# benfred/implicit

Hardware: AMD Instinct MI355X
Metric: ALS user+item updates/sec per iteration (factors=128); top-k recs/sec (higher is better)
Workload: dtype f32; 1 GPU; BASELINE configs[2]: last.fm-360K-shaped synthetic CSR, ALS CG cg_steps=3; users=358868, items=292385, nnz=17308340, factors=128, solver=cg, cg_steps=3

## Files before the change

implicit_amd/csrc/als_cg.hip:

```cpp
#include <type_traits>

#include "common.h"
#include "wave_ops.h"
#include "als_qtile.h"
#include "als_tile.h"

namespace imp {

template <int VPL, bool VEC, bool FIRST>
__device__ __forceinline__ void sparse_pass_simple(const int32_t *__restrict__ indices, const float *__restrict__ data,
                                                   const float *__restrict__ Y, int f, int lane, int begin, int end,
                                                   const float (&vec)[VPL], float (&acc)[VPL]) {
  constexpr int U = 4;
  for (int k0 = begin; k0 < end; k0 += 64) {
    int cnt = min(64, end - k0);
    int my_idx = 0;
    float my_c = 0.f;
    if (lane < cnt) {
      my_idx = indices[k0 + lane];
      my_c = data[k0 + lane];
    }
    for (int j = 0; j < cnt; j += U) {
      float y[U][VPL];
      float d[U];
// ... 387 lines not shown
        acc[v] = ((a8[0][v] + a8[1][v]) + (a8[2][v] + a8[3][v])) + ((a8[4][v] + a8[5][v]) + (a8[6][v] + a8[7][v]));
    }
    float x[VPL], dense[VPL];
    if (PHASE == 1 && xvec) load_row<VPL, VEC>(xvec + (size_t)li * LD, VEC ? LD : f, lane, x);
    else load_xrow<VPL, VEC>(xrow, f, lane, x);
#pragma unroll
    for (int v = 0; v < VPL; ++v) dense[v] = 0.f;
    if (PHASE == 0) {
      gram_matvec<VPL, VEC>(Amat, lda, lane, x, dense, 0, f);
      float r[VPL];
#pragma unroll
      for (int v = 0; v < VPL; ++v) r[v] = acc[v] - dense[v];
      float rsold = wave_allsum(dot_local<VPL>(r, r));
#pragma unroll
      for (int v = 0; v < VPL; ++v) {
        int e = elem<VPL, VEC>(lane, v);
        rvec[(size_t)li * LD + e] = r[v];
        pvec[(size_t)li * LD + e] = r[v];
        if (xvec) xvec[(size_t)li * LD + e] = x[v];
      }
      if (lane == 0) {
        scal[2 * li] = rsold;
        scal[2 * li + 1] = rsold < 1e-20f ? 1.f : 0.f;
      }
    } else {
      float p[VPL], r[VPL];
      load_row<VPL, VEC>(pvec + (size_t)li * LD, vld, lane, p);
      load_row<VPL, VEC>(rvec + (size_t)li * LD, vld, lane, r);
      gram_matvec<VPL, VEC>(Amat, lda, lane, p, dense, 0, f);
      float Ap[VPL];
#pragma unroll
      for (int v = 0; v < VPL; ++v) Ap[v] = dense[v] + acc[v];
      float rsold = scal[2 * li];
      float alpha = rsold / wave_allsum(dot_local<VPL>(p, Ap));
#pragma unroll
      for (int v = 0; v < VPL; ++v) {
        x[v] = fmaf(alpha, p[v], x[v]);
        r[v] = fmaf(-alpha, Ap[v], r[v]);
      }
      float rsnew = wave_allsum(dot_local<VPL>(r, r));
      float beta = rsnew / rsold;
#pragma unroll
      for (int v = 0; v < VPL; ++v) {
        int e = elem<VPL, VEC>(lane, v);
        if (e < f) store_x(xrow + e, x[v]);
        if (xvec) xvec[(size_t)li * LD + e] = x[v];
        rvec[(size_t)li * LD + e] = r[v];
        pvec[(size_t)li * LD + e] = fmaf(beta, p[v], r[v]);
      }
      if (lane == 0) {
        scal[2 * li] = rsnew;
        if (rsnew < 1e-20f) scal[2 * li + 1] = 1.f;
      }
    }
  }
}

template <typename T>
__global__ void zero_rows_kernel(const int32_t *__restrict__ order, int first, int count, T *__restrict__ X, int f) {
  size_t total = (size_t)count * f;
  for (size_t i = blockIdx.x * (size_t)blockDim.x + threadIdx.x; i < total; i += (size_t)gridDim.x * blockDim.x) {
    size_t r = i / f, c = i - r * f;
    store1(X + (size_t)order[first + r] * f + c, 0.f);
  }
}

template <typename T> static void zero_rows_t(const int32_t *order, int first, int count, T *X, int f) {
  if (count <= 0) return;
  IMP_PROF("zero_rows");
  size_t total = (size_t)count * f;
  int grid = (int)std::min<size_t>((total + 255) / 256, (size_t)ctx().num_cus * 8);
  zero_rows_kernel<T><<<grid, 256, 0, stream()>>>(order, first, count, X, f);
  IMP_CHECK_HIP(hipGetLastError());
}
void zero_rows(const int32_t *order, int first, int count, float *X, int f) { zero_rows_t<float>(order, first, count, X, f); }

template <int VPL, bool A_LDS>
static void launch_fused(const imp_csr *C, int first, int count, float *X, const float *Y, const float *A0, int f,
                         int cg_steps, const char *name) {
  if (count <= 0) return;
  constexpr int BLOCK = 512;
  constexpr int LD = 64 * VPL;
  size_t lds = (A_LDS ? (size_t)f * LD : 0) * sizeof(float);
  auto kern = als_cg_kernel<VPL, BLOCK, A_LDS>;
  allow_dynamic_lds(kern, std::max<size_t>(lds, 16));
  int blocks_per_cu = (int)std::max<size_t>(1, std::min<size_t>(2048 / BLOCK, (160 * 1024) / std::max<size_t>(lds, 1)));
  int grid = std::min((count + BLOCK / 64 - 1) / (BLOCK / 64), ctx().num_cus * blocks_per_cu * ctx().oversub);
  IMP_PROF(name);
  kern<<<grid, BLOCK, lds, stream()>>>(C->order.data(), first, count, C->indptr.data(), C->indices.data(), C->data.data(), X, Y,
                                       A0, f, cg_steps);
  IMP_CHECK_HIP(hipGetLastError());
}

template <int VPL, bool VEC, bool A_LDS, typename T>
static void launch_long(const imp_csr *C, const LongPlan &lp, T *X, const T *Y, const float *A0, int f, int cg_steps) {
  const int n_long = lp.n_long, n_seg = lp.n_seg;
  if (n_long <= 0) return;
  constexpr int BLOCK = 512;
  constexpr int LD = 64 * VPL;
  constexpr bool kHalf = !std::is_same<T, float>::value;
  size_t need = ((size_t)n_seg + (kHalf ? 3 : 2) * (size_t)n_long) * LD + 2 * (size_t)n_long;
  float *partial = ctx().long_ws.reserve(need);
  float *rvec = partial + (size_t)n_seg * LD;
  float *pvec = rvec + (size_t)n_long * LD;
  float *scal = pvec + (size_t)n_long * LD;
  float *xvec = kHalf ? scal + 2 * (size_t)n_long : nullptr;
  LongPlanDev plan = lp.dev(C->order.data());

  const bool rowblock = n_long <= ctx().num_cus * 2;
  size_t lds = ((A_LDS ? (size_t)f * LD : 0) + (rowblock ? (size_t)(BLOCK / 64) * LD : 0)) * sizeof(float);
  auto comb0 = rowblock ? cg_long_combine_kernel<VPL, VEC, BLOCK, A_LDS, 0, true, T> : cg_long_combine_kernel<VPL, VEC, BLOCK, A_LDS, 0, false, T>;
  auto comb1 = rowblock ? cg_long_combine_kernel<VPL, VEC, BLOCK, A_LDS, 1, true, T> : cg_long_combine_kernel<VPL, VEC, BLOCK, A_LDS, 1, false, T>;
  allow_dynamic_lds(comb0, std::max<size_t>(lds, 16));
  allow_dynamic_lds(comb1, std::max<size_t>(lds, 16));
  int grid_part = std::min(((n_seg + 3) / 4 + 7) / 8 * 8, ctx().num_cus * 8);
  int grid_comb = rowblock ? n_long : std::min((n_long + BLOCK / 64 - 1) / (BLOCK / 64), ctx().num_cus * 2);
  {
    IMP_PROF("als_cg_long_partial");
    if constexpr (VEC && (VPL == 1 || VPL == 2))
      cg_long_partial_q_kernel<64 * VPL, true, T>
          <<<grid_part, 256, 0, stream()>>>(plan, C->indices.data(), C->data.data(), X, Y, partial, pvec, scal);
    else if constexpr (std::is_same<T, float>::value)
      cg_long_partial_kernel<VPL, VEC, true>
          <<<grid_part, 256, 0, stream()>>>(plan, C->indices.data(), C->data.data(), X, Y, f, partial, pvec, scal);
    IMP_CHECK_HIP(hipGetLastError());
  }
  {
    IMP_PROF("als_cg_long_combine");
    comb0<<<grid_comb, BLOCK, lds, stream()>>>(plan, X, A0, f, partial, rvec, pvec, scal, xvec);
    IMP_CHECK_HIP(hipGetLastError());
  }
  for (int it = 0; it < cg_steps; ++it) {
    {
      IMP_PROF("als_cg_long_partial");
      if constexpr (VEC && (VPL == 1 || VPL == 2))
        cg_long_partial_q_kernel<64 * VPL, false, T>
            <<<grid_part, 256, 0, stream()>>>(plan, C->indices.data(), C->data.data(), X, Y, partial, pvec, scal);
      else if constexpr (std::is_same<T, float>::value)
        cg_long_partial_kernel<VPL, VEC, false>
            <<<grid_part, 256, 0, stream()>>>(plan, C->indices.data(), C->data.data(), X, Y, f, partial, pvec, scal);
      IMP_CHECK_HIP(hipGetLastError());
    }
    {
      IMP_PROF("als_cg_long_combine");
      comb1<<<grid_comb, BLOCK, lds, stream()>>>(plan, X, A0, f, partial, rvec, pvec, scal, xvec);
      IMP_CHECK_HIP(hipGetLastError());
    }
  }
}

template <int VPL, typename T>
static void cg_f64_f128(const imp_csr *C, T *X, const T *Y, size_t y_rows, const float *A0, int cg_steps) {
  constexpr int f = 64 * VPL;
  if (solver_switches().nm) least_squares_cg_nm<T>(C, X, Y, y_rows, A0, f, cg_steps);
  else launch_long<VPL, true, true, T>(C, C->plan_all, X, Y, A0, f, cg_steps);
  least_squares_cg_q<T>(C, X, Y, A0, f, cg_steps);
  zero_rows_t<T>(C->order.data(), C->first_empty(), C->n_empty(), X, f);
}

static void cg_f256(const imp_csr *C, float *X, const float *Y, const float *A0, int cg_steps) {
  constexpr int f = 256;
  const int32_t *b = C->bin_start;
  launch_long<4, true, false, float>(C, C->plan_all, X, Y, A0, f, cg_steps);
  if (solver_switches().w256) {
    launch_f256(C, b[1], b[2] - b[1], X, Y, A0, cg_steps, "als_cg_mid_rows");
    least_squares_cg_w256(C, X, Y, A0, cg_steps);
  } else {
    launch_f256(C, b[1], b[7] - b[1], X, Y, A0, cg_steps, "als_cg_mid_rows");
  }
  zero_rows_t<float>(C->order.data(), C->first_empty(), C->n_empty(), X, f);
}

template <int VPL, bool A_LDS>
static void cg_generic(const imp_csr *C, float *X, const float *Y, const float *A0, int f, int cg_steps) {
  const int32_t *b = C->bin_start;
  launch_long<VPL, false, A_LDS, float>(C, C->plan_all, X, Y, A0, f, cg_steps);
  launch_fused<VPL, A_LDS>(C, b[1], b[7] - b[1], X, Y, A0, f, cg_steps, "als_cg_mid_rows");
  zero_rows_t<float>(C->order.data(), C->first_empty(), C->n_empty(), X, f);
}

bool cg_native_half(int f) { return f == 64 || f == 128; }

static void least_squares_cg_padded(const imp_csr *C, imp_matrix *X, const imp_matrix *YtY, const imp_matrix *Y, int cg_steps, int F) {
  const size_t rx = (size_t)C->rows;
  const PaddedViews p = pad_in(X, Y, YtY, rx, F, true);
  if (F == 64) cg_f64_f128<1, float>(C, p.X.f32(), p.Y.f32(), p.Y.rows, p.YtY.f32(), cg_steps);
  else if (F == 128) cg_f64_f128<2, float>(C, p.X.f32(), p.Y.f32(), p.Y.rows, p.YtY.f32(), cg_steps);
  else cg_f256(C, p.X.f32(), p.Y.f32(), p.YtY.f32(), cg_steps);
  pad_out(X, rx, F);
}

void least_squares_cg(const imp_csr *C, imp_matrix *X, const imp_matrix *YtY, const imp_matrix *Y, int cg_steps) {
  note_device_write(X->data, (size_t)C->rows * X->cols * X->itemsize);
  IMP_PROF("als_cg_half_sweep");
  const int f = (int)X->cols;
  const float *a0 = YtY->f32();
  if (X->itemsize == 2) {
    if (!cg_native_half(f)) throw std::invalid_argument("least_squares: fp16 factors with this factor count are converted by the caller");
    __half *x = reinterpret_cast<__half *>(X->data);
    const __half *y = reinterpret_cast<const __half *>(Y->data);
    if (f == 64) cg_f64_f128<1, __half>(C, x, y, Y->rows, a0, cg_steps);
    else cg_f64_f128<2, __half>(C, x, y, Y->rows, a0, cg_steps);
    return;
  }
  float *x = X->f32();
  const float *y = Y->f32();
  if (solver_switches().cg_pad && f < 256 && f != 64 && f != 128 && f >= 1) {
    least_squares_cg_padded(C, X, YtY, Y, cg_steps, f < 64 ? 64 : (f < 128 ? 128 : 256));
    return;
  }
  if (f == 64) cg_f64_f128<1, float>(C, x, y, Y->rows, a0, cg_steps);
  else if (f == 128) cg_f64_f128<2, float>(C, x, y, Y->rows, a0, cg_steps);
  else if (f == 256) cg_f256(C, x, y, a0, cg_steps);
  else if (f < 64) cg_generic<1, true>(C, x, y, a0, f, cg_steps);
  else if (f < 128) cg_generic<2, true>(C, x, y, a0, f, cg_steps);
  else if (f < 192) cg_generic<3, true>(C, x, y, a0, f, cg_steps);
  else if (f < 256) cg_generic<4, false>(C, x, y, a0, f, cg_steps);
  else if (f <= 384) cg_generic<6, false>(C, x, y, a0, f, cg_steps);
  else if (f <= 512) cg_generic<8, false>(C, x, y, a0, f, cg_steps);
  else if (f <= 768) cg_generic<12, false>(C, x, y, a0, f, cg_steps);
  else if (f <= 1024) cg_generic<16, false>(C, x, y, a0, f, cg_steps);
  else throw std::invalid_argument("least_squares: factors must be <= 1024 (as the reference, implicit/gpu/als.cu:177-182)");
}

}
```

implicit_amd/csrc/als_cg_fixup.hip:

```cpp
#include <type_traits>

#include "als_qtile.h"
#include "common.h"

namespace imp {

template <int F, typename ST>
__global__ __launch_bounds__(256) void als_cg_fault_fixup_kernel(const unsigned *__restrict__ fault_count,
                                                                 const unsigned *__restrict__ fault_rows, int capacity,
                                                                 const int32_t *__restrict__ indptr,
                                                                 const int32_t *__restrict__ indices,
                                                                 const float *__restrict__ data, ST *__restrict__ X,
                                                                 const ST *__restrict__ Y, const float *__restrict__ A0, int cg_steps,
                                                                 unsigned long long *total) {
  constexpr int FC = F / 64, WAVES = 4, U = 4;
  __shared__ float vecs[WAVES][F];
  const int n = min((int)fault_count[0], capacity);
  if (n == 0) return;
  if (blockIdx.x == 0 && threadIdx.x == 0) __hip_atomic_fetch_add(total, (unsigned long long)n, __ATOMIC_RELAXED, __HIP_MEMORY_SCOPE_SYSTEM);
  const int lane = threadIdx.x & 63, wave = threadIdx.x >> 6;
  float *vec = vecs[wave];
  auto load_vec = [&](const ST *row, float (&v)[FC]) {
#pragma unroll
    for (int c = 0; c < FC; ++c) v[c] = load1(row + FC * lane + c);
  };
  auto apply = [&](bool first, int rb, int re, const float (&v)[FC], float (&acc)[FC]) {
#pragma unroll
    for (int c = 0; c < FC; ++c) vec[FC * lane + c] = v[c];
#pragma unroll
    for (int c = 0; c < FC; ++c) acc[c] = 0.f;
    for (int j = 0; j < F; ++j) {
      const float vj = vec[j];
#pragma unroll
      for (int c = 0; c < FC; ++c) acc[c] = fmaf(A0[(size_t)j * F + FC * lane + c], vj, acc[c]);
    }
    if (first) {
#pragma unroll
      for (int c = 0; c < FC; ++c) acc[c] = -acc[c];
    }
    for (int k0 = rb; k0 < re; k0 += U) {
      float conf[U], y[U][FC];
#pragma unroll
      for (int q = 0; q < U; ++q) {
        const int k = min(k0 + q, re - 1);
        conf[q] = data[k];
        load_vec(Y + (size_t)indices[k] * F, y[q]);
      }
#pragma unroll
      for (int q = 0; q < U; ++q) {
        if (k0 + q < re) {
          const float d = wave_allsum(dot_local<FC>(y[q], v));
          const float cm1 = fabsf(conf[q]) - 1.f;
          const float w = first ? fmaxf(conf[q], 0.f) - cm1 * d : cm1 * d;
#pragma unroll
          for (int c = 0; c < FC; ++c) acc[c] = fmaf(w, y[q][c], acc[c]);
        }
      }
    }
  };
  for (int i = blockIdx.x * WAVES + wave; i < n; i += gridDim.x * WAVES) {
    const int u = (int)fault_rows[i];
    const int rb = indptr[u], re = indptr[u + 1];
    ST *xrow = X + (size_t)u * F;
    float x[FC], r[FC], p[FC], Ap[FC];
    load_vec(xrow, x);
    apply(true, rb, re, x, r);
#pragma unroll
    for (int c = 0; c < FC; ++c) p[c] = r[c];
    float rsold = wave_allsum(dot_local<FC>(r, r));
    if (rsold < 1e-20f) continue;
    for (int it = 0; it < cg_steps; ++it) {
      apply(false, rb, re, p, Ap);
      const float alpha = rsold / wave_allsum(dot_local<FC>(p, Ap));
#pragma unroll
      for (int c = 0; c < FC; ++c) {
        x[c] = fmaf(alpha, p[c], x[c]);
        r[c] = fmaf(-alpha, Ap[c], r[c]);
      }
      const float rsnew = wave_allsum(dot_local<FC>(r, r));
      if (rsnew < 1e-20f) break;
      const float beta = rsnew / rsold;
#pragma unroll
      for (int c = 0; c < FC; ++c) p[c] = fmaf(beta, p[c], r[c]);
      rsold = rsnew;
    }
#pragma unroll
    for (int c = 0; c < FC; ++c) store1(xrow + FC * lane + c, x[c]);
  }
}

unsigned long long *fixup_total() {
  auto &c = ctx();
  if (!c.fixup_total) {
    IMP_CHECK_HIP(hipHostMalloc(reinterpret_cast<void **>(&c.fixup_total), sizeof(unsigned long long), hipHostMallocMapped));
    *c.fixup_total = 0ull;
  }
  return c.fixup_total;
}

template <int F, typename T>
void launch_cg_fixup(const unsigned *count, const unsigned *rows, int capacity, const imp_csr *C, T *X, const T *Y, const float *A0,
                     int cg_steps) {
  if (capacity <= 0) return;
  IMP_PROF("als_cg_fixup");
  als_cg_fault_fixup_kernel<F, T><<<std::min((capacity + 3) / 4, ctx().num_cus * 2), 256, 0, stream()>>>(
      count, rows, capacity, C->indptr.data(), C->indices.data(), C->data.data(), X, Y, A0, cg_steps, fixup_total());
  IMP_CHECK_HIP(hipGetLastError());
}
template void launch_cg_fixup<64, float>(const unsigned *, const unsigned *, int, const imp_csr *, float *, const float *, const float *, int);
template void launch_cg_fixup<128, float>(const unsigned *, const unsigned *, int, const imp_csr *, float *, const float *, const float *, int);
template void launch_cg_fixup<64, __half>(const unsigned *, const unsigned *, int, const imp_csr *, __half *, const __half *, const float *, int);
template void launch_cg_fixup<128, __half>(const unsigned *, const unsigned *, int, const imp_csr *, __half *, const __half *, const float *, int);


}
```

implicit_amd/csrc/als_cg_nm.hip:

```cpp
#include "als_qf_common.h"
#include "common.h"
#include "wave_ops.h"

namespace imp {

namespace {

typedef _Float16 half8 __attribute__((ext_vector_type(8)));
typedef _Float16 half2v __attribute__((ext_vector_type(2)));
typedef float f32x16 __attribute__((ext_vector_type(16)));
typedef float f32x4v __attribute__((ext_vector_type(4)));
typedef unsigned u32x4 __attribute__((ext_vector_type(4)));

template <int F> struct NmShape;
template <> struct NmShape<128> {
  static constexpr int M = 32, KG = 2, NACC = 16;
  using acc_t = f32x16;
  __device__ static __forceinline__ acc_t mfma(half8 a, half8 b, acc_t c) { return __builtin_amdgcn_mfma_f32_32x32x16_f16(a, b, c, 0, 0, 0); }
  __device__ static __forceinline__ int row(int lane, int e) { return (e & 3) + 8 * (e >> 2) + 4 * (lane >> 5); }
  __device__ static __forceinline__ int col(int lane) { return lane & 31; }
};
template <> struct NmShape<64> {
  static constexpr int M = 16, KG = 4, NACC = 4;
  using acc_t = f32x4v;
  __device__ static __forceinline__ acc_t mfma(half8 a, half8 b, acc_t c) { return __builtin_amdgcn_mfma_f32_16x16x32_f16(a, b, c, 0, 0, 0); }
  __device__ static __forceinline__ int row(int lane, int e) { return 4 * (lane >> 4) + e; }
  __device__ static __forceinline__ int col(int lane) { return lane & 15; }
};

template <int F> struct NmLayout {
  static constexpr int M = F / 4;
  static constexpr int TS = M + 1;
  static constexpr int IMG = 16 * M * TS;
  static constexpr int KCH = 8 * NmShape<F>::KG;
  static constexpr int ROUND = 4 * KCH;
  static constexpr int kTiles = 10;
  static constexpr int kSlots = 3;
  static constexpr int QUAD = 64 * 4;
  static constexpr int OPS = 4 * 16 * QUAD;
  static constexpr int NP = 256 / F;
  static constexpr int kVec = IMG > OPS ? IMG : OPS;
  static constexpr size_t lds_floats = (size_t)kVec + 2 * F + NP * F + 64 + 4 * F;
  __host__ __device__ static constexpr int at(int I, int J, int m, int n) { return ((I * 4 + J) * M + m) * TS + n; }
};
__device__ constexpr int nm_tile_i(int t) { return t < 1 ? 0 : t < 3 ? 1 : t < 6 ? 2 : 3; }
__device__ constexpr int nm_tile_j(int t) { return t - (nm_tile_i(t) * (nm_tile_i(t) + 1)) / 2; }

__device__ __forceinline__ void split_pair(float x0, float x1, unsigned &hi, unsigned &lo) {
  const f32x2 v = {x0, x1};
  const half2v h = __builtin_convertvector(v, half2v);
  const f32x2 r = v - __builtin_convertvector(h, f32x2);
  const half2v l = __builtin_convertvector(r, half2v);
  hi = __builtin_bit_cast(unsigned, h);
  lo = __builtin_bit_cast(unsigned, l);
}
__device__ __forceinline__ unsigned pack_pair(float x0, float x1) {
  const f32x2 v = {x0, x1};
  return __builtin_bit_cast(unsigned, __builtin_convertvector(v, half2v));
}
__device__ __forceinline__ float comp(const float4 &v, int c) { return c == 0 ? v.x : c == 1 ? v.y : c == 2 ? v.z : v.w; }

template <int F> __global__ void nm_gram_image_kernel(const float *__restrict__ A0, float *__restrict__ img, int *__restrict__ ctl,
                                                      float y_rows, int forced_k, float reg = 0.f) {
  using L = NmLayout<F>;
  if (blockIdx.x == 0 && threadIdx.x < 64) {
    float d = 0.f;
    for (int j = threadIdx.x; j < F; j += 64) d = fmaxf(d, A0[(size_t)j * F + j]);
    d = wave_allmax(d);
    if (threadIdx.x == 0) {
      int k = 0;
      const float rms = sqrtf((d + reg) / fmaxf(y_rows, 1.f));
      if (rms > 0.f && rms < 8.f) k = min((int)floorf(log2f(8.f / rms)), 16);
      ctl[0] = 0;
      ctl[1] = forced_k >= 0 ? forced_k : k;
      ctl[2] = 0;
      ctl[3] = 0;
    }
  }
  for (int e = blockIdx.x * blockDim.x + threadIdx.x; e < L::IMG; e += gridDim.x * blockDim.x) {
    const int n = e % L::TS, m = (e / L::TS) % L::M, t = e / (L::TS * L::M);
    img[e] = n < L::M ? A0[(size_t)(4 * m + t / 4) * F + 4 * n + t % 4] + ((m == n && t / 4 == t % 4) ? reg : 0.f) : 0.f;
  }
}

__device__ __forceinline__ void lds_barrier() { asm volatile("s_waitcnt lgkmcnt(0)\n\ts_barrier" ::: "memory"); }

template <int F, typename T, bool TRIM = false>
__device__ __forceinline__ void nm_build(const int32_t *__restrict__ indices, const float *__restrict__ data, const T *__restrict__ Y,
                                         const float *__restrict__ gram_img, bool whole, int begin, int end, float *smem, float *bvec,
                                         int tid, int ko, int scale_k) {
  using S = NmShape<F>;
  using L = NmLayout<F>;
  constexpr bool kHalf = !std::is_same<T, float>::value;
  const int lane = tid & 63, wave = __builtin_amdgcn_readfirstlane(tid >> 6);
  const int a = lane % S::M, g = lane / S::M;
  const int first = wave < 2 ? 3 * wave : 2 * wave + 2;
  const int n_slots = wave < 2 ? 3 : 2;
  int tI[L::kSlots], tJ[L::kSlots];
#pragma unroll
  for (int k = 0; k < L::kSlots; ++k) {
    const int t = min(first + k, L::kTiles - 1);
    tI[k] = t < 1 ? 0 : t < 3 ? 1 : t < 6 ? 2 : 3;
    tJ[k] = t - tI[k] * (tI[k] + 1) / 2;
  }
  typename S::acc_t acc[L::kSlots];
#pragma unroll
  for (int k = 0; k < L::kSlots; ++k)
#pragma unroll
    for (int e = 0; e < S::NACC; ++e) acc[k][e] = 0.f;
  float b4[4] = {0.f, 0.f, 0.f, 0.f};
  const float scale2 = __uint_as_float((unsigned)(127 + 2 * scale_k) << 23), unscale2 = __uint_as_float((unsigned)(127 - 2 * scale_k) << 23);

  const int n_rounds = (ko & 1) ? 0 : (end - begin + L::ROUND - 1) / L::ROUND;
  struct Entry {
    int col;
    float c;
  };
  auto load_entry = [&](int r) {
    Entry en;
    const int k = begin + r * L::ROUND + wave * L::KCH + (lane % L::KCH);
    const int kk = min(k, end - 1);
    en.col = indices[kk];
    const float c = data[kk];
    en.c = k < end ? c : -1.f;
    return en;
  };
  float4 yb[8];
  auto gather = [&](const Entry &en, float4 (&y)[8]) {
#pragma unroll
    for (int q = 0; q < 8; ++q) {
      const int col = __shfl(en.col, 8 * g + q, 64);
      y[q] = load4(Y + (size_t)col * F + 4 * a);
    }
  };
  float *ops = smem;
  int *negflag = reinterpret_cast<int *>(bvec + 2 * F + L::NP * F + 32);
  Entry e0{0, -1.f}, e1 = e0, e2 = e0;
  if (n_rounds > 0) {
    e0 = load_entry(0), e1 = load_entry(1);
    gather(e0, yb);
  }
  struct Pair {
    half8 h, l;
  };
  const float *lane_ops = ops + 4 * lane;
  int negbits = 0;
  auto ld_u = [&](int st, int I) {
    Pair p;
    const int ku = (negbits >> st) & 1 ? 0 : 2;
    p.h = __builtin_bit_cast(half8, *reinterpret_cast<const u32x4 *>(lane_ops + (st * 16 + ku * 4 + I) * L::QUAD));
    p.l = __builtin_bit_cast(half8, *reinterpret_cast<const u32x4 *>(lane_ops + (st * 16 + (ku + 1) * 4 + I) * L::QUAD));
    return p;
  };
  auto ld_y = [&](int st, int J) {
    Pair p;
    p.h = __builtin_bit_cast(half8, *reinterpret_cast<const u32x4 *>(lane_ops + (st * 16 + 2 * 4 + J) * L::QUAD));
    if constexpr (!kHalf) p.l = __builtin_bit_cast(half8, *reinterpret_cast<const u32x4 *>(lane_ops + (st * 16 + 3 * 4 + J) * L::QUAD));
    else p.l = p.h;
    return p;
  };
  auto products = [&](auto k, const Pair &u, const Pair &y) {
    acc[k.value] = S::mfma(u.h, y.h, acc[k.value]);
    acc[k.value] = S::mfma(u.l, y.h, acc[k.value]);
    if constexpr (!kHalf) acc[k.value] = S::mfma(u.h, y.l, acc[k.value]);
  };
  auto consume = [&](int s0, int s1) {
    negbits = __builtin_amdgcn_readfirstlane(negflag[0] | (negflag[1] << 1) | (negflag[2] << 2) | (negflag[3] << 3));
    if (wave == 0) {
      Pair u0 = ld_u(s0, 0), y0 = ld_y(s0, 0);
#pragma unroll 1
      for (int st = s0; st < s1; ++st) {
        const Pair u1 = ld_u(st, 1);
        products(idx_t<0>{}, u0, y0);
        const Pair y1 = ld_y(st, 1);
        products(idx_t<1>{}, u1, y0);
        u0 = ld_u(min(st + 1, s1 - 1), 0), y0 = ld_y(min(st + 1, s1 - 1), 0);
        products(idx_t<2>{}, u1, y1);
      }
    } else if (wave == 1) {
      Pair u2 = ld_u(s0, 2), y0 = ld_y(s0, 0);
#pragma unroll 1
      for (int st = s0; st < s1; ++st) {
        const Pair y1 = ld_y(st, 1);
        products(idx_t<0>{}, u2, y0);
        const Pair y2 = ld_y(st, 2);
        products(idx_t<1>{}, u2, y1);
        const Pair un = ld_u(min(st + 1, s1 - 1), 2);
        y0 = ld_y(min(st + 1, s1 - 1), 0);
        products(idx_t<2>{}, u2, y2);
        u2 = un;
      }
    } else {
      const int J0 = wave == 2 ? 0 : 2;
      Pair u3 = ld_u(s0, 3), ya = ld_y(s0, J0);
#pragma unroll 1
      for (int st = s0; st < s1; ++st) {
        const Pair yb2 = ld_y(st, J0 + 1);
        products(idx_t<0>{}, u3, ya);
        const Pair un = ld_u(min(st + 1, s1 - 1), 3);
        ya = ld_y(min(st + 1, s1 - 1), J0);
        products(idx_t<1>{}, u3, yb2);
        u3 = un;
      }
    }
  };
  auto produce = [&](int r, float4 (&y)[8]) {
    if (r > 0) e0 = e1, e1 = e2;
    e2 = load_entry(r + 2);
    {
      const float w_mine = (fabsf(e0.c) - 1.f) * scale2;
      const float cp_mine = e0.c > 0.f ? e0.c : 0.f;
      float *mine = ops + (size_t)wave * 16 * L::QUAD + 4 * lane;
      if constexpr (!kHalf) {
        const float sq_mine = __builtin_amdgcn_sqrtf(fabsf(w_mine));
        const unsigned ng_mine = w_mine < 0.f ? 0x8000u : 0u;
        const bool any_neg = __builtin_amdgcn_ballot_w64(ng_mine != 0u) != 0ull;
        if (lane == 0) negflag[wave] = any_neg ? 1 : 0;
        float sq[8];
        unsigned ng[8];
#pragma unroll
        for (int q = 0; q < 8; ++q) {
          sq[q] = __shfl(sq_mine, 8 * g + q, 64);
          ng[q] = (unsigned)__shfl((int)ng_mine, 8 * g + q, 64);
          const float cp = __shfl(cp_mine, 8 * g + q, 64);
          b4[0] = fmaf(cp, y[q].x, b4[0]);
          b4[1] = fmaf(cp, y[q].y, b4[1]);
          b4[2] = fmaf(cp, y[q].z, b4[2]);
          b4[3] = fmaf(cp, y[q].w, b4[3]);
        }
#pragma unroll
        for (int c = 0; c < 4; ++c) {
          u32x4 zh, zl;
#pragma unroll
          for (int q = 0; q < 8; q += 2) {
            unsigned h, l;
            split_pair(sq[q] * comp(y[q], c), sq[q + 1] * comp(y[q + 1], c), h, l);
            zh[q / 2] = h, zl[q / 2] = l;
          }
          *reinterpret_cast<u32x4 *>(mine + (2 * 4 + c) * L::QUAD) = zh;
          *reinterpret_cast<u32x4 *>(mine + (3 * 4 + c) * L::QUAD) = zl;
          if (any_neg) {
            u32x4 uh, ul;
#pragma unroll
            for (int q = 0; q < 8; q += 2) {
              const unsigned m = ng[q] | (ng[q + 1] << 16);
              uh[q / 2] = zh[q / 2] ^ m, ul[q / 2] = zl[q / 2] ^ m;
            }
            *reinterpret_cast<u32x4 *>(mine + (0 * 4 + c) * L::QUAD) = uh;
            *reinterpret_cast<u32x4 *>(mine + (1 * 4 + c) * L::QUAD) = ul;
          }
          __builtin_amdgcn_sched_barrier(0);
        }
      } else {
        unsigned hb = (((__float_as_uint(w_mine) & 0x7f800000u) + (127u << 23)) >> 1) & 0x7f800000u;
        hb = min(max(hb, (127u - 12u) << 23), (127u + 24u) << 23);
        const float sb_mine = __uint_as_float(hb), wa_mine = w_mine * __uint_as_float((254u << 23) - hb);
        if (lane == 0) negflag[wave] = 1;
        float wa[8], sb[8];
#pragma unroll
        for (int q = 0; q < 8; ++q) {
          wa[q] = __shfl(wa_mine, 8 * g + q, 64);
          sb[q] = __shfl(sb_mine, 8 * g + q, 64);
          const float cp = __shfl(cp_mine, 8 * g + q, 64);
          b4[0] = fmaf(cp, y[q].x, b4[0]);
          b4[1] = fmaf(cp, y[q].y, b4[1]);
          b4[2] = fmaf(cp, y[q].z, b4[2]);
          b4[3] = fmaf(cp, y[q].w, b4[3]);
        }
#pragma unroll
        for (int c = 0; c < 4; ++c) {
          u32x4 uh, ul, yh;
#pragma unroll
          for (int q = 0; q < 8; q += 2) {
            const float y0 = comp(y[q], c), y1 = comp(y[q + 1], c);
            unsigned h, l;
            yh[q / 2] = pack_pair(sb[q] * y0, sb[q + 1] * y1);
            split_pair(wa[q] * y0, wa[q + 1] * y1, h, l);
            uh[q / 2] = h, ul[q / 2] = l;
          }
          *reinterpret_cast<u32x4 *>(mine + (0 * 4 + c) * L::QUAD) = uh;
          *reinterpret_cast<u32x4 *>(mine + (1 * 4 + c) * L::QUAD) = ul;
          *reinterpret_cast<u32x4 *>(mine + (2 * 4 + c) * L::QUAD) = yh;
          __builtin_amdgcn_sched_barrier(0);
        }
      }
    }
    gather(e1, y);
  };
#pragma unroll 1
  for (int r = 0; r < n_rounds; ++r) {
    produce(r, yb);
    lds_barrier();
    if constexpr (TRIM) consume(0, min(4, (end - begin - r * L::ROUND + L::KCH - 1) / L::KCH));
    else consume(0, 4);
    lds_barrier();
  }
  if (!(ko & 2)) {
    float *bstage = bvec + 2 * F + L::NP * F + 64;
#pragma unroll
    for (int c = 0; c < 4; ++c) {
      float v = b4[c];
      if constexpr (S::KG == 4) v += __shfl_xor(v, 16, 64);
      v += __shfl_xor(v, 32, 64);
      if (g == 0) bstage[wave * F + c * L::M + a] = v;
    }
    float *img = smem;
    const int n = S::col(lane);
#pragma unroll
    for (int k = 0; k < L::kSlots; ++k) {
      if (k < n_slots) {
        const int I = tI[k], J = tJ[k];
        float gv[S::NACC];
#pragma unroll
        for (int e = 0; e < S::NACC; ++e) gv[e] = 0.f;
        if (whole) {
#pragma unroll
          for (int e = 0; e < S::NACC; ++e) gv[e] = gram_img[L::at(I, J, S::row(lane, e), n)];
        }
#pragma unroll
        for (int e = 0; e < S::NACC; ++e) {
          const int m = S::row(lane, e);
          const float v = fmaf(acc[k][e], unscale2, gv[e]);
          img[L::at(I, J, m, n)] = v;
          if (I != J) img[L::at(J, I, n, m)] = v;
        }
      }
    }
  }
  __syncthreads();
}

template <int F, typename T>
__device__ __forceinline__ bool nm_cg(const float *img, const float *bvec, float *pv, float *parts, float *red, T *xrow, int cg_steps, int tid) {
  using L = NmLayout<F>;
  constexpr int M = L::M, NP = L::NP, JPG = 4 / NP;
  const int r = tid % F, grp = tid / F, lane = tid & 63, wave = tid >> 6;
  const int I = r / M, m = r % M;
  int slot = 0;
  auto matvec = [&]() {
    float s[4] = {0.f, 0.f, 0.f, 0.f};
#pragma unroll
    for (int jj = 0; jj < JPG; ++jj) {
      const int J = grp * JPG + jj;
      const float *row = img + L::at(I, J, m, 0);
#pragma unroll
      for (int n = 0; n < M; n += 4) {
        const float4 p4 = *reinterpret_cast<const float4 *>(pv + J * M + n);
        s[0] = fmaf(row[n], p4.x, s[0]), s[1] = fmaf(row[n + 1], p4.y, s[1]);
        s[2] = fmaf(row[n + 2], p4.z, s[2]), s[3] = fmaf(row[n + 3], p4.w, s[3]);
      }
    }
    parts[grp * F + r] = (s[0] + s[1]) + (s[2] + s[3]);
    __syncthreads();
    float q = parts[r];
#pragma unroll
    for (int gq = 1; gq < NP; ++gq) q += parts[gq * F + r];
    return q;
  };
  auto block_sum = [&](float v) {
    v = wave_allsum(grp == 0 ? v : 0.f);
    if (lane == 0) red[4 * slot + wave] = v;
    __syncthreads();
    const float s = (red[4 * slot] + red[4 * slot + 1]) + (red[4 * slot + 2] + red[4 * slot + 3]);
    slot = (slot + 1) & 7;
    return s;
  };
  auto finite = [](float v) { return fabsf(v) <= 3.0e38f; };
  float x = load1(xrow + 4 * m + I);
  if (grp == 0) pv[r] = x;
  __syncthreads();
  float res = bvec[r] - matvec();
  float p = res;
  float rsold = block_sum(res * res);
  if (!finite(rsold)) return true;
  if (rsold < 1e-20f) return false;
  for (int it = 0; it < cg_steps; ++it) {
    if (grp == 0) pv[r] = p;
    __syncthreads();
    const float Ap = matvec();
    const float pAp = block_sum(p * Ap);
    const float alpha = rsold / pAp;
    x = fmaf(alpha, p, x);
    res = fmaf(-alpha, Ap, res);
    const float rsnew = block_sum(res * res);
    if (!finite(pAp) || !finite(rsnew) || !finite(alpha)) return true;
    if (rsnew < 1e-20f) break;
    p = fmaf(rsnew / rsold, p, res);
    rsold = rsnew;
  }
  if (grp == 0) store1(xrow + 4 * m + I, x);
  return false;
}

#ifdef CHOL_NM_STATS
__device__ unsigned long long g_chol_nm_stats[8];
#define CHOL_TICK(slot)                                                          \
  do {                                                                           \
    __builtin_amdgcn_sched_barrier(0);                                           \
    const unsigned long long now_ = __builtin_amdgcn_s_memtime();                \
    if (threadIdx.x == 0) atomicAdd(&g_chol_nm_stats[slot], now_ - chol_t_last); \
    chol_t_last = now_;                                                          \
    __builtin_amdgcn_sched_barrier(0);                                           \
  } while (0)
__device__ unsigned long long chol_t_last_dummy;
#else
#define CHOL_TICK(slot) ((void)0)
#endif
struct NoGram {
  __device__ __forceinline__ float operator()(int, int, int, int) const { return 0.f; }
};
template <int F, typename GB>
__device__ __forceinline__ bool nm_chol(float *img, float *bvec, float *scr, float *xrow, int tid, const GB &gblocks) {
  static_assert(F == 128, "block ownership and the LDS budget are laid out for f = 128");
#ifdef CHOL_NM_STATS
  unsigned long long chol_t_last = __builtin_amdgcn_s_memtime();
#endif
  using L = NmLayout<F>;
  constexpr int NB = F / 4, NBLK = NB * (NB + 1) / 2, LDL = F + 4, SL = (NBLK + 255) / 256;
  static_assert(F * LDL <= L::kVec, "the row-major factor re-uses the image's space");
  float *pan = scr;
  float *dblk = scr + 2 * F * 4;
  int bm[SL], bn[SL];
  float B[SL][4][4];
#pragma unroll
  for (int s = 0; s < SL; ++s) {
    const int bid = tid + 256 * s;
    bm[s] = bn[s] = -1;
    if (bid < NBLK) {
      int t = (int)((sqrtf(8.f * (float)bid + 1.f) - 1.f) * 0.5f);
      while (t * (t + 1) / 2 > bid) --t;
      while ((t + 1) * (t + 2) / 2 <= bid) ++t;
      bn[s] = NB - 1 - t, bm[s] = bn[s] + (bid - t * (t + 1) / 2);
#pragma unroll
      for (int a = 0; a < 4; ++a)
#pragma unroll
        for (int c = 0; c < 4; ++c) B[s][a][c] = img[L::at(a, c, bm[s], bn[s])] + gblocks(a, c, bm[s], bn[s]);
    }
  }
  float rb[4] = {0.f, 0.f, 0.f, 0.f};
  if (tid < NB) {
#pragma unroll
    for (int c = 0; c < 4; ++c) rb[c] = bvec[c * L::M + tid];
  }
  __syncthreads();
  CHOL_TICK(1);
#pragma unroll
  for (int s = 0; s < SL; ++s) {
    if (bm[s] == 0 && bn[s] == 0) {
#pragma unroll
      for (int a = 0; a < 4; ++a) *reinterpret_cast<float4 *>(dblk + 4 * a) = make_float4(B[s][a][0], B[s][a][1], B[s][a][2], B[s][a][3]);
    }
  }
  __syncthreads();
  bool fail = false;
#pragma unroll 1
  for (int kb = 0; kb < NB; ++kb) {
    const float *D = dblk + (kb & 1) * 16;
    float *P = pan + (size_t)(kb & 1) * F * 4;
    const float4 d0 = *reinterpret_cast<const float4 *>(D), d1 = *reinterpret_cast<const float4 *>(D + 4),
                 d2 = *reinterpret_cast<const float4 *>(D + 8), d3 = *reinterpret_cast<const float4 *>(D + 12);
    auto rsq = [](float d) {
      const float r = __builtin_amdgcn_rsqf(d);
      return r * fmaf(-0.5f * d * r, r, 1.5f);
    };
    const float p0 = d0.x, r0 = rsq(p0);
    const float l10 = d1.x * r0, l20 = d2.x * r0, l30 = d3.x * r0;
    const float p1 = fmaf(-l10, l10, d1.y), r1 = rsq(p1);
    const float l21 = fmaf(-l20, l10, d2.y) * r1, l31 = fmaf(-l30, l10, d3.y) * r1;
    const float p2 = fmaf(-l21, l21, fmaf(-l20, l20, d2.z)), r2 = rsq(p2);
    const float l32 = fmaf(-l31, l21, fmaf(-l30, l20, d3.z)) * r2;
    const float p3 = fmaf(-l32, l32, fmaf(-l31, l31, fmaf(-l30, l30, d3.w))), r3 = rsq(p3);
    if (!(p0 > 0.f && p1 > 0.f && p2 > 0.f && p3 > 0.f && p3 < 3.0e38f)) {
      fail = true;
      break;
    }
    auto solve_row = [&](float (&v)[4]) {
      const float x0 = v[0] * r0;
      const float x1 = fmaf(-x0, l10, v[1]) * r1;
      const float x2 = fmaf(-x1, l21, fmaf(-x0, l20, v[2])) * r2;
      const float x3 = fmaf(-x2, l32, fmaf(-x1, l31, fmaf(-x0, l30, v[3]))) * r3;
      v[0] = x0, v[1] = x1, v[2] = x2, v[3] = x3;
    };
#pragma unroll
    for (int s = 0; s < SL; ++s) {
      if (bn[s] == kb) {
        if (bm[s] > kb) {
#pragma unroll
          for (int a = 0; a < 4; ++a) {
            solve_row(B[s][a]);
            *reinterpret_cast<float4 *>(P + (size_t)(4 * bm[s] + a) * 4) = make_float4(B[s][a][0], B[s][a][1], B[s][a][2], B[s][a][3]);
          }
        } else {
          B[s][0][0] = r0, B[s][1][0] = l10, B[s][1][1] = r1, B[s][2][0] = l20, B[s][2][1] = l21, B[s][2][2] = r2;
          B[s][3][0] = l30, B[s][3][1] = l31, B[s][3][2] = l32, B[s][3][3] = r3;
        }
      }
    }
    if (tid == kb) {
      solve_row(rb);
      *reinterpret_cast<float4 *>(bvec + 4 * kb) = make_float4(rb[0], rb[1], rb[2], rb[3]);
    }
    __syncthreads();
    float *Dn = dblk + ((kb + 1) & 1) * 16;
#pragma unroll
    for (int s = 0; s < SL; ++s) {
      if (bn[s] > kb) {
        float4 pm[4], pn[4];
#pragma unroll
        for (int a = 0; a < 4; ++a) {
          pm[a] = *reinterpret_cast<const float4 *>(P + (size_t)(4 * bm[s] + a) * 4);
          pn[a] = *reinterpret_cast<const float4 *>(P + (size_t)(4 * bn[s] + a) * 4);
        }
#pragma unroll
        for (int a = 0; a < 4; ++a)
#pragma unroll
          for (int c = 0; c < 4; ++c)
            B[s][a][c] = fmaf(-pm[a].w, pn[c].w, fmaf(-pm[a].z, pn[c].z, fmaf(-pm[a].y, pn[c].y, fmaf(-pm[a].x, pn[c].x, B[s][a][c]))));
        if (bn[s] == kb + 1 && bm[s] == kb + 1) {
#pragma unroll
          for (int a = 0; a < 4; ++a) *reinterpret_cast<float4 *>(Dn + 4 * a) = make_float4(B[s][a][0], B[s][a][1], B[s][a][2], B[s][a][3]);
        }
      }
    }
    if (tid < NB && tid > kb) {
      const float4 z4 = *reinterpret_cast<const float4 *>(bvec + 4 * kb);
#pragma unroll
      for (int c = 0; c < 4; ++c) {
        const float4 pc = *reinterpret_cast<const float4 *>(P + (size_t)(4 * tid + c) * 4);
        rb[c] = fmaf(-z4.w, pc.w, fmaf(-z4.z, pc.z, fmaf(-z4.y, pc.y, fmaf(-z4.x, pc.x, rb[c]))));
      }
    }
    __syncthreads();
  }
  CHOL_TICK(2);
  if (fail) return true;
#pragma unroll
  for (int s = 0; s < SL; ++s) {
    if (bm[s] >= 0) {
#pragma unroll
      for (int a = 0; a < 4; ++a)
        *reinterpret_cast<float4 *>(img + (size_t)(4 * bm[s] + a) * LDL + 4 * bn[s]) = make_float4(B[s][a][0], B[s][a][1], B[s][a][2], B[s][a][3]);
    }
  }
  __syncthreads();
// ... 10 lines not shown
    const float x1 = fmaf(-q3.y, x3, fmaf(-q2.y, x2, z.y)) * q1.y;
    const float x0 = fmaf(-q3.x, x3, fmaf(-q2.x, x2, fmaf(-q1.x, x1, z.x))) * q0.x;
    if (tid < 4 * kb) {
      const float *col = img + (size_t)(4 * kb) * LDL + tid;
      bvec[tid] = fmaf(-col[3 * LDL], x3, fmaf(-col[2 * LDL], x2, fmaf(-col[LDL], x1, fmaf(-col[0], x0, bvec[tid]))));
    }
    if (tid == 0) *reinterpret_cast<float4 *>(xs + 4 * kb) = make_float4(x0, x1, x2, x3);
    __syncthreads();
  }
  CHOL_TICK(4);
  if (tid < F) xrow[tid] = xs[tid];
  return false;
}

template <int F, typename T, bool CHOL = false>
__global__ __launch_bounds__(256, 2) void als_cg_nm_kernel(const LongPlanDev plan, const int32_t *__restrict__ indices,
                                                           const float *__restrict__ data, T *__restrict__ X, const T *__restrict__ Y,
                                                           const float *__restrict__ gram_img, int cg_steps, float *__restrict__ partial,
                                                           int *__restrict__ ticket,
                                                           unsigned *__restrict__ fix_rows,
                                                           int ko) {
  using L = NmLayout<F>;
  extern __shared__ __attribute__((aligned(16))) float smem[];
  __shared__ int next_item;
  float *img = smem, *bvec = img + L::kVec, *pv = bvec + F, *parts = pv + F, *red = parts + L::NP * F;
  const int tid = threadIdx.x;
  const int scale_k = __builtin_amdgcn_readfirstlane(ticket[1]);
  for (int s = blockIdx.x; s < plan.n_seg;) {
    const int li = plan.seg_row[s];
    const int begin = plan.seg_begin[s], end = plan.seg_end[s];
    const bool whole = plan.row_seg[li + 1] - plan.row_seg[li] == 1;
    __syncthreads();
    nm_build<F, T>(indices, data, Y, gram_img, whole, begin, end, smem, bvec, tid, ko, scale_k);
    if (tid < F) {
      const float *bstage = bvec + 2 * F + L::NP * F + 64;
      bvec[tid] = (bstage[tid] + bstage[F + tid]) + (bstage[2 * F + tid] + bstage[3 * F + tid]);
    }
    __syncthreads();
    int drawn = 0;
    if (tid == 0) drawn = (int)gridDim.x + atomicAdd(ticket, 1);
    if (!(ko & 4)) {
      if (whole) {
        bool bad = false;
        if constexpr (CHOL) bad = nm_chol<F>(img, bvec, pv, X + (size_t)plan.rows[li] * F, tid, NoGram{});
        else bad = nm_cg<F, T>(img, bvec, pv, parts, red, X + (size_t)plan.rows[li] * F, cg_steps, tid);
        if (bad && tid == 0) fix_rows[atomicAdd(ticket + 2, 1)] = (unsigned)plan.rows[li];
      } else {
        float *out = partial + (size_t)s * (L::IMG + F);
        for (int e = tid; e < L::IMG / 4; e += 256) reinterpret_cast<float4 *>(out)[e] = reinterpret_cast<const float4 *>(img)[e];
        if (tid < F) out[L::IMG + tid] = bvec[tid];
      }
    }
    if (tid == 0) next_item = drawn;
    __syncthreads();
    s = next_item;
  }
}

template <int F>
__global__ __launch_bounds__(256) void als_cg_nm_reduce_kernel(const LongPlanDev plan, int n_multi, const float *__restrict__ gram_img,
                                                               float *__restrict__ partial) {
  using L = NmLayout<F>;
  constexpr int CH = 16, PER = L::IMG / CH / 4;
  static_assert(L::IMG % (CH * 4) == 0, "chunks of whole float4 pieces");
  for (int item = blockIdx.x; item < n_multi * CH; item += gridDim.x) {
    const int li = item / CH, chunk = item % CH;
    const int s0 = plan.row_seg[li], s1 = plan.row_seg[li + 1];
    const size_t stride = (size_t)(L::IMG + F) / 4;
    for (int e = threadIdx.x; e < PER + (chunk == 0 ? F / 4 : 0); e += 256) {
      const size_t off = e < PER ? (size_t)chunk * PER + e : (size_t)L::IMG / 4 + (e - PER);
      float4 *base = reinterpret_cast<float4 *>(partial) + off;
      float4 sum = e < PER ? reinterpret_cast<const float4 *>(gram_img)[off] : make_float4(0.f, 0.f, 0.f, 0.f);
      int s = s0;
      for (; s + 8 <= s1; s += 8) {
        float4 v[8];
#pragma unroll
        for (int q = 0; q < 8; ++q) v[q] = base[(size_t)(s + q) * stride];
#pragma unroll
        for (int q = 0; q < 8; ++q) sum.x += v[q].x, sum.y += v[q].y, sum.z += v[q].z, sum.w += v[q].w;
      }
      for (; s < s1; ++s) {
        const float4 v = base[(size_t)s * stride];
        sum.x += v.x, sum.y += v.y, sum.z += v.z, sum.w += v.w;
      }
      base[(size_t)s0 * stride] = sum;
    }
  }
}

template <int F, typename T, bool CHOL = false>
__global__ __launch_bounds__(256) void als_cg_nm_finish_kernel(const LongPlanDev plan, int n_multi, T *__restrict__ X, int cg_steps,
                                                               const float *__restrict__ partial, int *__restrict__ ctl,
                                                               unsigned *__restrict__ fix_rows) {
  using L = NmLayout<F>;
  extern __shared__ __attribute__((aligned(16))) float smem[];
  float *img = smem, *bvec = img + L::kVec, *pv = bvec + F, *parts = pv + F, *red = parts + L::NP * F;
  const int tid = threadIdx.x;
  for (int li = blockIdx.x; li < n_multi; li += gridDim.x) {
    const float *in = partial + (size_t)plan.row_seg[li] * (L::IMG + F);
    __syncthreads();
    for (int e = tid; e < L::IMG / 4; e += 256) reinterpret_cast<float4 *>(img)[e] = reinterpret_cast<const float4 *>(in)[e];
    if (tid < F) bvec[tid] = in[L::IMG + tid];
    __syncthreads();
    bool bad = false;
    if constexpr (CHOL) bad = nm_chol<F>(img, bvec, pv, X + (size_t)plan.rows[li] * F, tid, NoGram{});
    else bad = nm_cg<F, T>(img, bvec, pv, parts, red, X + (size_t)plan.rows[li] * F, cg_steps, tid);
    if (bad && tid == 0) fix_rows[atomicAdd(ctl + 2, 1)] = (unsigned)plan.rows[li];
  }
}

template <int F>
__global__ __launch_bounds__(256, 2) void als_chol_nm_rows_kernel(const int32_t *__restrict__ order, int first, int count,
                                                                  const int32_t *__restrict__ indptr, const int32_t *__restrict__ indices,
                                                                  const float *__restrict__ data, float *__restrict__ X,
                                                                  const float *__restrict__ Y, const float *__restrict__ gram_img,
                                                                  int *__restrict__ ctl, unsigned *__restrict__ fix_rows) {
  using L = NmLayout<F>;
  extern __shared__ __attribute__((aligned(16))) float smem[];
  __shared__ int next_item;
  float *img = smem, *bvec = img + L::kVec, *pv = bvec + F;
  const int tid = threadIdx.x;
  const int scale_k = __builtin_amdgcn_readfirstlane(ctl[1]);
  struct GramBlocks {
    const float *img;
    __device__ __forceinline__ float operator()(int a, int c, int m, int n) const { return img[L::at(a, c, m, n)]; }
  } gb{gram_img};
  for (int i = blockIdx.x; i < count;) {
    const int u = order[first + i];
    const int begin = indptr[u], end = indptr[u + 1];
    __syncthreads();
#ifdef CHOL_NM_STATS
    unsigned long long chol_t_last = __builtin_amdgcn_s_memtime();
#endif
    nm_build<F, float, true>(indices, data, Y, gram_img, false, begin, end, smem, bvec, tid, 0, scale_k);
    if (tid < F) {
      const float *bstage = bvec + 2 * F + L::NP * F + 64;
      bvec[tid] = (bstage[tid] + bstage[F + tid]) + (bstage[2 * F + tid] + bstage[3 * F + tid]);
    }
    __syncthreads();
    CHOL_TICK(0);
#ifdef CHOL_NM_STATS
    if (tid == 0) atomicAdd(&g_chol_nm_stats[5], 1ull);
#endif
    int drawn = 0;
    if (tid == 0) drawn = (int)gridDim.x + atomicAdd(ctl + 3, 1);
    const bool bad = nm_chol<F>(img, bvec, pv, X + (size_t)u * F, tid, gb);
    if (bad && tid == 0) fix_rows[atomicAdd(ctl + 2, 1)] = (unsigned)u;
    if (tid == 0) next_item = drawn;
    __syncthreads();
    i = next_item;
  }
}

template <int F, typename T> void launch_nm(const imp_csr *C, T *X, const T *Y, size_t y_rows, const float *A0, int cg_steps) {
  const LongPlan &lp = C->plan_nm;
  if (lp.n_seg <= 0) return;
  using L = NmLayout<F>;
  static_assert(L::IMG % 4 == 0, "the image is copied in 16-byte pieces");
  const size_t lds = L::lds_floats * sizeof(float);
  const int n_multi = C->nm_multi_rows, n_multi_seg = C->nm_multi_segs;
  const size_t need = (size_t)L::IMG + (size_t)n_multi_seg * (L::IMG + F);
  float *gram_img = ctx().long_ws.reserve(need), *partial = gram_img + L::IMG;
  auto &tk = ctx().nm_ticket;
  tk.reserve(4, true);
  auto &fix = ctx().nm_fix_rows;
  fix.reserve((size_t)lp.n_long);
  LongPlanDev plan = lp.dev(C->order.data());
  auto kern = als_cg_nm_kernel<F, T>;
  auto fin = als_cg_nm_finish_kernel<F, T>;
  allow_dynamic_lds(kern, lds);
  allow_dynamic_lds(fin, lds);
  {
    IMP_PROF("als_cg_nm_rows");
    constexpr int forced_k = -1;
    nm_gram_image_kernel<F><<<(L::IMG + 255) / 256, 256, 0, stream()>>>(A0, gram_img, tk.data(), (float)y_rows, std::min(forced_k, 16));
    const int grid = std::min(lp.n_seg, ctx().num_cus * 2);
    constexpr int ko = 0;
    kern<<<grid, 256, lds, stream()>>>(plan, C->indices.data(), C->data.data(), X, Y, gram_img, cg_steps, partial, tk.data(), fix.data(), ko);
    IMP_CHECK_HIP(hipGetLastError());
  }
  if (n_multi > 0) {
    IMP_PROF("als_cg_nm_finish");
    als_cg_nm_reduce_kernel<F><<<std::min(n_multi * 16, ctx().num_cus * 16), 256, 0, stream()>>>(plan, n_multi, gram_img, partial);
    fin<<<std::min(n_multi, ctx().num_cus * 2), 256, lds, stream()>>>(plan, n_multi, X, cg_steps, partial, tk.data(), fix.data());
    IMP_CHECK_HIP(hipGetLastError());
  }
  launch_cg_fixup<F, T>(reinterpret_cast<const unsigned *>(tk.data() + 2), fix.data(), lp.n_long, C, X, Y, A0, cg_steps);
}

}

CholNmList least_squares_cholesky_nm(const imp_csr *C, float *X, const float *Y, size_t y_rows, const float *YtY, float reg) {
  constexpr int F = 128;
  using L = NmLayout<F>;
  const LongPlan &lp = C->plan_nm;
  const int32_t *b = C->bin_start;
  const size_t lds = (L::lds_floats + 128) * sizeof(float);
  const int n_multi = C->nm_multi_rows, n_multi_seg = C->nm_multi_segs;
  const size_t need = (size_t)L::IMG + (size_t)n_multi_seg * (L::IMG + F);
  float *gram_img = ctx().long_ws.reserve(need), *partial = gram_img + L::IMG;
  auto &tk = ctx().nm_ticket;
  tk.reserve(4, true);
  auto &fix = ctx().nm_fix_rows;
  const int capacity = C->nonempty();
  fix.reserve((size_t)std::max(capacity, 1));
  constexpr int forced_k = -1;
  {
    IMP_PROF("als_cholesky_nm_long");
    nm_gram_image_kernel<F><<<(L::IMG + 255) / 256, 256, 0, stream()>>>(YtY, gram_img, tk.data(), (float)y_rows, std::min(forced_k, 16), reg);
    if (lp.n_seg > 0) {
      LongPlanDev plan = lp.dev(C->order.data());
      auto kern = als_cg_nm_kernel<F, float, true>;
      auto fin = als_cg_nm_finish_kernel<F, float, true>;
      allow_dynamic_lds(kern, lds);
      allow_dynamic_lds(fin, lds);
      kern<<<std::min(lp.n_seg, ctx().num_cus * 2), 256, lds, stream()>>>(plan, C->indices.data(), C->data.data(), X, Y, gram_img, -1, partial,
                                                                          tk.data(), fix.data(), 0);
      if (n_multi > 0) {
        als_cg_nm_reduce_kernel<F><<<std::min(n_multi * 16, ctx().num_cus * 16), 256, 0, stream()>>>(plan, n_multi, gram_img, partial);
        fin<<<std::min(n_multi, ctx().num_cus * 2), 256, lds, stream()>>>(plan, n_multi, X, -1, partial, tk.data(), fix.data());
      }
    }
    IMP_CHECK_HIP(hipGetLastError());
  }
  const int count = b[7] - b[1];
  if (count > 0) {
    IMP_PROF("als_cholesky_nm_rows");
    auto rk = als_chol_nm_rows_kernel<F>;
    allow_dynamic_lds(rk, lds);
    rk<<<std::min(count, ctx().num_cus * 2), 256, lds, stream()>>>(C->order.data(), b[1], count, C->indptr.data(), C->indices.data(),
                                                                    C->data.data(), X, Y, gram_img, tk.data(), fix.data());
    IMP_CHECK_HIP(hipGetLastError());
#ifdef CHOL_NM_STATS
    {
      unsigned long long h[8], z[8] = {0, 0, 0, 0, 0, 0, 0, 0};
      IMP_CHECK_HIP(hipStreamSynchronize(stream()));
      IMP_CHECK_HIP(hipMemcpyFromSymbol(h, HIP_SYMBOL(g_chol_nm_stats), sizeof(h)));
      IMP_CHECK_HIP(hipMemcpyToSymbol(HIP_SYMBOL(g_chol_nm_stats), z, sizeof(z)));
      const double n = (double)std::max<unsigned long long>(1, h[5]);
      fprintf(stderr, "[chol-nm-stats] rows=%llu cycles per row: build %.0f  block load %.0f  factorisation %.0f  L store %.0f  back substitution %.0f\n",
              h[5], h[0] / n, h[1] / n, h[2] / n, h[3] / n, h[4] / n);
    }
#endif
  }
  return CholNmList{reinterpret_cast<const unsigned *>(tk.data() + 2), fix.data(), capacity};
}

template <typename T> void least_squares_cg_nm(const imp_csr *C, T *X, const T *Y, size_t y_rows, const float *A0, int f, int cg_steps) {
  if (f == 128) launch_nm<128, T>(C, X, Y, y_rows, A0, cg_steps);
  else if (f == 64) launch_nm<64, T>(C, X, Y, y_rows, A0, cg_steps);
  else throw std::invalid_argument("least_squares_cg_nm: f must be 64 or 128");
}
template void least_squares_cg_nm<float>(const imp_csr *, float *, const float *, size_t, const float *, int, int);
template void least_squares_cg_nm<__half>(const imp_csr *, __half *, const __half *, size_t, const float *, int, int);

}
```

implicit_amd/csrc/als_cg_q.hip:

```cpp
#include <type_traits>

#include "als_qtile.h"
#include "common.h"

namespace imp {

template <typename T>
void launch_team_fused(const imp_csr *C, int f, int width, int first, int count, T *X, const T *Y, const float *A0, int cg_steps,
                       const char *name);
template <typename T>
void launch_group_fused(const imp_csr *C, int f, int first, int count, T *X, const T *Y, const float *A0, int cg_steps, const char *name);
template <typename ST>
void launch_team_tile64(const imp_csr *C, int f, int width, int first, int count, ST *X, const ST *Y, const float *A0, int cg_steps,
                        const char *name);

template <typename T>
void launch_team_chain(const imp_csr *C, int f, const int (&first)[3], const int (&count)[3], T *X, const T *Y, const float *A0, int cg_steps,
                       const char *name);
template <typename T>
void launch_wide_chain(const imp_csr *C, int f, const int (&first)[2], const int (&count)[2], T *X, const T *Y, const float *A0, int cg_steps,
                       const char *name);

template <int F, typename T> static void run_classes_q(const imp_csr *C, T *X, const T *Y, const float *A0, int cg_steps) {
  const int32_t *b = C->bin_start;
  constexpr bool kHalf = std::is_same<T, __half>::value;
  auto team = [&](int width32, int lo, int hi, const char *name) {
    if constexpr (kHalf) launch_team_tile64<T>(C, F, width32 / 2, lo, hi - lo, X, Y, A0, cg_steps, name);
    else launch_team_fused<T>(C, F, width32, lo, hi - lo, X, Y, A0, cg_steps, name);
  };
  if (F == 128 && !kHalf && !prof_unfiltered()) {
    const int first[3] = {b[2], b[3], b[4]}, count[3] = {b[3] - b[2], b[4] - b[3], b[5] - b[4]};
    launch_team_chain<T>(C, F, first, count, X, Y, A0, cg_steps, "als_cg_team_chain_rows");
    const int wide_first[2] = {b[1], b[5]}, wide_count[2] = {b[2] - b[1], b[7] - b[5]};
    launch_wide_chain<T>(C, F, wide_first, wide_count, X, Y, A0, cg_steps, "als_cg_wide_chain_rows");
    return;
  }
  team(16, b[1], b[2], "als_cg_team16_rows");
  team(8, b[2], b[3], "als_cg_team8_rows");
  team(4, b[3], b[4], "als_cg_team4_rows");
  team(2, b[4], b[5], "als_cg_team2_rows");
  if constexpr (F == 64) launch_team_fused<T>(C, F, 1, b[5], b[7] - b[5], X, Y, A0, cg_steps, "als_cg_short_rows");
  else launch_group_fused<T>(C, F, b[5], b[7] - b[5], X, Y, A0, cg_steps, "als_cg_short_rows");
}

template <typename T> void least_squares_cg_q(const imp_csr *C, T *X, const T *Y, const float *A0, int f, int cg_steps) {
  if (f == 128) run_classes_q<128, T>(C, X, Y, A0, cg_steps);
  else if (f == 64) run_classes_q<64, T>(C, X, Y, A0, cg_steps);
  else throw std::invalid_argument("least_squares_cg_q: f must be 64 or 128");
}
template void least_squares_cg_q<float>(const imp_csr *, float *, const float *, const float *, int, int);
template void least_squares_cg_q<__half>(const imp_csr *, __half *, const __half *, const float *, int, int);

}
```

implicit_amd/csrc/als_cg_qf.hip:

```cpp
#include <type_traits>

#include <algorithm>

#include "als_qf_common.h"
#include "common.h"

namespace imp {

template <typename ST> struct Tile32 {
  typedef f32x2 elem;
  static constexpr int T = 32;
  static constexpr bool ROLL = std::is_same<ST, float>::value;
  static __device__ __forceinline__ void fetch(const int32_t *indices, const float *data, int lane, int k0, int end, int &col, float &c) {
    fetch_entries(indices, data, lane, k0, end, col, c);
  }
  template <int H> static __device__ __forceinline__ void gather(elem (&yq)[H], const ST *p) {
#pragma unroll
    for (int h = 0; h < H; h += 2) {
      const float4 v = load4(p + 32 * h);
      yq[h] = f32x2{v.x, v.y}, yq[h + 1] = f32x2{v.z, v.w};
    }
  }
  template <int H> static __device__ __forceinline__ float dot(const elem (&yq)[H], const f32x2 (&ve)[H]) {
    f32x2 s = yq[0] * ve[0];
#pragma unroll
    for (int h = 1; h < H; ++h) s = __builtin_elementwise_fma(yq[h], ve[h], s);
    return s.x + s.y;
  }
  template <int H> static __device__ __forceinline__ void axpy(const elem (&yq)[H], float w, f32x2 (&ae)[H]) {
    const f32x2 w2 = {w, w};
#pragma unroll
    for (int h = 0; h < H; ++h) ae[h] = __builtin_elementwise_fma(w2, yq[h], ae[h]);
  }
};

template <int F, int WPR, int BLOCK, typename ST>
__global__ __launch_bounds__(BLOCK, F == 64 ? 8 : 4) void als_cg_qfteam_kernel(const int32_t *__restrict__ order, int first, int count,
                                                                 const int32_t *__restrict__ indptr,
                                                                 const int32_t *__restrict__ indices,
                                                                 const float *__restrict__ data, ST *__restrict__ X,
                                                                 const ST *__restrict__ Y, const float *__restrict__ A0,
                                                                 int cg_steps) {
  team_rows<Tile32<ST>, F, WPR, BLOCK>(order, first, count, indptr, indices, data, X, Y, A0, cg_steps);
}

template <int F, int WPR, int BLOCK, typename T>
static void launch_qfteam(const imp_csr *C, int first, int count, T *X, const T *Y, const float *A0, int cg_steps,
                          const char *name) {
  if (count <= 0) return;
  constexpr int WAVES = BLOCK / 64, TEAMS = WAVES / WPR;
  size_t lds = team_lds_bytes<F, WPR, BLOCK, Tile32<T>::T>();
  auto kern = als_cg_qfteam_kernel<F, WPR, BLOCK, T>;
  allow_dynamic_lds(kern, lds);
  int per_cu = (int)std::max<size_t>(1, std::min<size_t>(2048 / BLOCK, (160 * 1024) / lds));
  constexpr int kBaseOversub = WPR <= 4 ? 4 : (WPR == 8 ? 2 : (F == 64 ? 2 : 1));
  int grid = std::min((count + TEAMS - 1) / TEAMS, ctx().num_cus * per_cu * std::max(kBaseOversub, ctx().oversub));
  IMP_PROF(name);
  kern<<<grid, BLOCK, lds, stream()>>>(C->order.data(), first, count, C->indptr.data(), C->indices.data(), C->data.data(), X, Y,
                                      A0, cg_steps);
  IMP_CHECK_HIP(hipGetLastError());
}

struct ChainClassArgs {
  int first[ChainTickets::kClasses], count[ChainTickets::kClasses];
  unsigned base[ChainTickets::kClasses][ChainTickets::kQueues];
};
static_assert(ChainTickets::kQueues == kTicketQueues, "queues of a ticketed class");
template <int F> constexpr size_t chain_lds_bytes() {
  return std::max(team_lds_bytes<F, 8, 512, 32>(), std::max(team_lds_bytes<F, 4, 512, 32>(), team_lds_bytes<F, 2, 512, 32>()));
}
template <int F, typename ST>
__global__ __launch_bounds__(512, F == 64 ? 8 : 4) void als_cg_qfteam_chain_kernel(const int32_t *__restrict__ order, ChainClassArgs cls,
                                                                                  unsigned *__restrict__ counters,
                                                                                  const int32_t *__restrict__ indptr,
                                                                                  const int32_t *__restrict__ indices,
                                                                                  const float *__restrict__ data, ST *__restrict__ X,
                                                                                  const ST *__restrict__ Y, const float *__restrict__ A0,
                                                                                  int cg_steps) {
  static_assert(Tile32<ST>::T == 32, "chain_lds_bytes");
  team_stage_gramian<F, 512>(A0);
  bool entered = false;
  static_for<ChainTickets::kClasses>([&](auto Cc) {
    constexpr int C = decltype(Cc)::value, WPR = 8 >> C;
    if (cls.count[C] > 0) {
      if (entered) __syncthreads();
      entered = true;
      team_rows<Tile32<ST>, F, WPR, 512, true, false>(order, cls.first[C], cls.count[C], indptr, indices, data, X, Y, A0, cg_steps,
                                                      counters + (C * kTicketQueues + blockIdx.x % kTicketQueues) * ChainTickets::kCounterStride,
                                                      cls.base[C][blockIdx.x % kTicketQueues]);
    }
  });
}

static int team512_per_cu(size_t lds) { return (int)std::max<size_t>(1, std::min<size_t>(2048 / 512, (160 * 1024) / lds)); }

template <typename T>
void launch_team_chain(const imp_csr *C, int f, const int (&first)[3], const int (&count)[3], T *X, const T *Y, const float *A0, int cg_steps,
                       const char *name) {
  if constexpr (std::is_same<T, float>::value) {
    auto run = [&](auto Fc) {
      constexpr int F = decltype(Fc)::value;
      if (count[0] <= 0 && count[1] <= 0 && count[2] <= 0) return;
      const size_t lds = chain_lds_bytes<F>();
      auto kern = als_cg_qfteam_chain_kernel<F, T>;
      allow_dynamic_lds(kern, lds);
      const int grid = std::max(ctx().num_cus * team512_per_cu(lds), ChainTickets::kQueues);
      ChainClassArgs cls;
      const int teams[3] = {1, 2, 4};
      for (int c = 0; c < 3; ++c) {
        if (count[c] >= ChainTickets::kMaxCount) throw std::invalid_argument("launch_team_chain: too many rows in a class");
        cls.first[c] = first[c], cls.count[c] = std::max(count[c], 0);
      }
      Context &cx = ctx();
      cx.chain_counters.reserve((size_t)ChainTickets::kClasses * ChainTickets::kQueues * ChainTickets::kCounterStride, true);
      ChainTickets after = cx.chain_tickets;
      after.launch(cls.count, grid, teams, cls.base);
      IMP_PROF(name);
      kern<<<grid, 512, lds, stream()>>>(C->order.data(), cls, cx.chain_counters.data(), C->indptr.data(), C->indices.data(),
                                        C->data.data(), X, Y, A0, cg_steps);
      IMP_CHECK_HIP(hipGetLastError());
      cx.chain_tickets = after;
    };
    if (f == 128) run(idx_t<128>{});
    else throw std::invalid_argument("launch_team_chain: f must be 128");
  } else {
    throw std::invalid_argument("launch_team_chain: fp32 storage only (float16 storage runs its classes on the packed tiles)");
  }
}
template void launch_team_chain<float>(const imp_csr *, int, const int (&)[3], const int (&)[3], float *, const float *, const float *, int,
                                       const char *);
template void launch_team_chain<__half>(const imp_csr *, int, const int (&)[3], const int (&)[3], __half *, const __half *, const float *,
                                        int, const char *);

typedef float f32x4 __attribute__((ext_vector_type(4)));
template <int F> struct QFGroupCfg {
  static constexpr int LD = F + 8;
  static constexpr int LDB = F + 8;
  static constexpr int NT = F / 16;
  static constexpr int KH = 16 / NT;
  static constexpr int KB = (F / 16) / KH;
  static constexpr size_t lds_bytes = (size_t)3 * F * LDB * 2 + (size_t)3 * 16 * LDB * 2 +
                                      ((size_t)16 * LD + (size_t)KH * 16 * LD + 16 * 64) * sizeof(float);
};
typedef __bf16 bf16x8 __attribute__((ext_vector_type(8)));
typedef __bf16 bf16x2 __attribute__((ext_vector_type(2)));
__device__ __forceinline__ void split_bf16(float x, __bf16 &hi, __bf16 &mid, __bf16 &lo) {
  hi = (__bf16)x;
  const float r1 = x - (float)hi;
  mid = (__bf16)r1;
  lo = (__bf16)(r1 - (float)mid);
}

template <int F, bool FIRST, bool LAST, bool ROLL, typename ST>
__device__ __forceinline__ float tile_pass(f32x2 (&y)[8][F / 32], float *cw, int cnt, const float *vrow, float (&acc)[F / 64], int lane,
                                          int cnt_nx, int &col_nx, float &c_nx, const ST *__restrict__ Y) {
  using Tile = Tile32<ST>;
  constexpr int FE = F / 16, H = FE / 2;
  static_assert(!(FIRST && LAST) && (LAST || !ROLL), "pass form");
  if constexpr (ROLL) {
    col_nx = opaque(col_nx);
    c_nx = __int_as_float(opaque(__float_as_int(c_nx)));
  }
  f32x2 ve[H], ae[H];
  const float *cwg;
  {
    const int ln = opaque(lane);
    const int g = ln >> 4, m = ln & 15;
#pragma unroll
    for (int e = 0; e < FE; e += 4) {
      const float4 t = *reinterpret_cast<const float4 *>(vrow + 16 * e + 4 * m);
      ve[e / 2] = f32x2{t.x, t.y}, ve[e / 2 + 1] = f32x2{t.z, t.w};
    }
    cwg = cw + g;
    if constexpr (LAST) cwg += 4 * (m >> 3);
  }
#pragma unroll
  for (int h = 0; h < H; ++h) ae[h] = f32x2{0.f, 0.f};
  float s8 = 0.f;
  auto partial = [&](int q) { return Tile::template dot<H>(y[q], ve); };
  auto axpy = [&](int q, float w) { Tile::template axpy<H>(y[q], w, ae); };
  static_for<4>([&](auto Pc) {
    constexpr int P = decltype(Pc)::value;
    if (8 * P < cnt) {
      const float cm1_0 = cwg[8 * P];
      float cm1_1 = 0.f, cp_0 = 0.f, cp_1 = 0.f;
      if constexpr (!LAST) cm1_1 = cwg[8 * P + 4];
      if constexpr (FIRST) cp_0 = cwg[32 + 8 * P], cp_1 = cwg[32 + 8 * P + 4];
      const float u = reduce_pair(partial(2 * P), partial(2 * P + 1));
      if constexpr (LAST) {
        s8 = fmaf(cm1_0 * u, u, s8);
      } else {
        const float w0 = FIRST ? fmaf(-cm1_0, row_bcast_from<0>(u), cp_0) : cm1_0 * row_bcast_from<0>(u);
        const float w1 = FIRST ? fmaf(-cm1_1, row_bcast_from<8>(u), cp_1) : cm1_1 * row_bcast_from<8>(u);
        axpy(2 * P, w0);
        axpy(2 * P + 1, w1);
      }
    }
    if constexpr (ROLL) {
      if (8 * P < cnt_nx) gather_pair<Tile, F, P>(y, cw, col_nx, c_nx, cnt_nx, Y, lane);
    }
  });
  if constexpr (LAST) {
    return 0.125f * s8;
  } else {
    float aes[FE];
#pragma unroll
    for (int h = 0; h < H; ++h) aes[2 * h] = ae[h].x, aes[2 * h + 1] = ae[h].y;
    reduce_expanded<F>(aes, acc);
    return 0.f;
  }
}

template <int F> __device__ __forceinline__ void group_stage_gramian(const float *__restrict__ A0) {
  extern __shared__ __attribute__((aligned(16))) float smem[];
  constexpr int LDB = QFGroupCfg<F>::LDB;
  __bf16 *A0b = reinterpret_cast<__bf16 *>(smem);
  for (int e = threadIdx.x; e < F * F; e += 1024) {
    int r = e / F, c = e - r * F;
    __bf16 h, m, l;
    split_bf16(A0[e], h, m, l);
    A0b[r * LDB + c] = h, A0b[(size_t)F * LDB + r * LDB + c] = m, A0b[(size_t)2 * F * LDB + r * LDB + c] = l;
  }
  __syncthreads();
}

template <int F, typename ST, bool TICKETS = false>
__device__ __forceinline__ void group_rows(const int32_t *__restrict__ order, int first, int count, const int32_t *__restrict__ indptr,
                                           const int32_t *__restrict__ indices, const float *__restrict__ data, ST *__restrict__ X,
                                           const ST *__restrict__ Y, int cg_steps, unsigned *counter = nullptr, unsigned base = 0u) {
  using Cfg = QFGroupCfg<F>;
  constexpr int FC = F / 64, FE = F / 16, LD = Cfg::LD;
  constexpr bool ROLL = Tile32<ST>::ROLL;
  extern __shared__ __attribute__((aligned(16))) float smem[];
  constexpr int LDB = Cfg::LDB;
  __bf16 *A0b = reinterpret_cast<__bf16 *>(smem);
  __bf16 *Pb = A0b + (size_t)3 * F * LDB;
  float *Ps = reinterpret_cast<float *>(Pb + (size_t)3 * 16 * LDB);
  float *Outs = Ps + 16 * LD;
  float *cws = Outs + (size_t)Cfg::KH * 16 * LD;
  const int lane = threadIdx.x & 63;
  const int wave = __builtin_amdgcn_readfirstlane(threadIdx.x >> 6);
  float *prow = Ps + (size_t)wave * LD;
  float *cw = cws + (size_t)wave * 64;
  const unsigned cf = (unsigned)QL<F>::cfactor(lane, 0);

  auto publish = [&](const float (&vec)[FC], bool valid) {
    if constexpr (FC == 2) *reinterpret_cast<float2 *>(prow + cf) = valid ? make_float2(vec[0], vec[1]) : make_float2(0.f, 0.f);
    else prow[cf] = valid ? vec[0] : 0.f;
    bf16x2 t[3];
#pragma unroll
    for (int c = 0; c < 2; ++c) {
      __bf16 h, m, l;
      split_bf16(valid ? vec[c] : 0.f, h, m, l);
      t[0][c] = h, t[1][c] = m, t[2][c] = l;
    }
#pragma unroll
    for (int k = 0; k < 3; ++k) *reinterpret_cast<bf16x2 *>(Pb + (size_t)k * 16 * LDB + (size_t)wave * LDB + cf) = t[k];
    __syncthreads();
  };
  auto product = [&]() {
    const int ti = wave % Cfg::NT, kh = wave / Cfg::NT;
    const int ln = opaque(lane);
    const int i = ln & 15, kq = ln >> 4;
    f32x4 acc = {0.f, 0.f, 0.f, 0.f};
    static_assert(Cfg::KB * 16 == 64, "three-term product: 64 k per wave");
#pragma unroll
    for (int b = 0; b < 2; ++b) {
      const int k0 = kh * 64 + 32 * b + 8 * kq;
      const __bf16 *ar = A0b + (size_t)(16 * ti + i) * LDB + k0, *pr = Pb + (size_t)i * LDB + k0;
      const bf16x8 ah = *reinterpret_cast<const bf16x8 *>(ar), am = *reinterpret_cast<const bf16x8 *>(ar + (size_t)F * LDB),
                   al = *reinterpret_cast<const bf16x8 *>(ar + (size_t)2 * F * LDB);
      const bf16x8 ph = *reinterpret_cast<const bf16x8 *>(pr), pm = *reinterpret_cast<const bf16x8 *>(pr + (size_t)16 * LDB),
                   pl = *reinterpret_cast<const bf16x8 *>(pr + (size_t)2 * 16 * LDB);
      acc = __builtin_amdgcn_mfma_f32_16x16x32_bf16(al, ph, acc, 0, 0, 0);
      acc = __builtin_amdgcn_mfma_f32_16x16x32_bf16(ah, pl, acc, 0, 0, 0);
      acc = __builtin_amdgcn_mfma_f32_16x16x32_bf16(am, pm, acc, 0, 0, 0);
      acc = __builtin_amdgcn_mfma_f32_16x16x32_bf16(am, ph, acc, 0, 0, 0);
      acc = __builtin_amdgcn_mfma_f32_16x16x32_bf16(ah, pm, acc, 0, 0, 0);
      acc = __builtin_amdgcn_mfma_f32_16x16x32_bf16(ah, ph, acc, 0, 0, 0);
    }
    *reinterpret_cast<float4 *>(Outs + (kh * 16 + i) * LD + 16 * ti + 4 * kq) = make_float4(acc[0], acc[1], acc[2], acc[3]);
  };
  auto collect = [&](float (&out)[FC]) {
#pragma unroll
    for (int c = 0; c < FC; ++c) out[c] = 0.f;
// ... 31 lines not shown
  };
  int id0 = row_id(g_first), id1 = row_id(t1), id2 = row_id(t2), id3 = row_id(t3);
  int b0 = indptr[id0], e0 = indptr[id0 + 1], b1 = indptr[id1], e1 = indptr[id1 + 1], b2 = indptr[id2], e2 = indptr[id2 + 1];
  int ent_col, ent_cnt = row_valid(g_first) ? e0 - b0 : 0;
  float ent_c;
  fetch_entries(indices, data, opaque(lane), b0, max(e0, b0 + 1), ent_col, ent_c);
  bool tile_ready = false;
  int cnt = 0;
  f32x2 y[8][FE / 2];
  float x[FC];
  auto kill = [](float (&v)[FC]) {
#pragma unroll
    for (int cc = 0; cc < FC; ++cc) v[cc] = 0.f;
  };
  kill(x);
  for (int g = g_first; g < groups;) {
    const bool valid = row_valid(g);
    int t_new = t3 + g_step;
    ST *xrow = X + (size_t)id0 * F;
    if (!tile_ready) {
      cnt = ent_cnt;
      ent_col = opaque(ent_col);
      ent_c = __int_as_float(opaque(__float_as_int(ent_c)));
      static_for<4>([&](auto Pc) {
        constexpr int P = decltype(Pc)::value;
        if (8 * P < cnt) gather_pair<Tile32<ST>, F, P>(y, cw, ent_col, ent_c, cnt, Y, lane);
      });
      ent_cnt = row_valid(t1) ? e1 - b1 : 0;
      fetch_entries(indices, data, opaque(lane), b1, max(e1, b1 + 1), ent_col, ent_c);
      load_compact<F>(xrow, opaque(lane), x);
    }
    float xc[FC], r[FC], p[FC], Ap[FC], sp[FC];
#pragma unroll
    for (int cc = 0; cc < FC; ++cc) xc[cc] = x[cc];
    publish(xc, valid);
    const bool drawing = TICKETS && t3 < groups;
    if constexpr (TICKETS) {
      if (drawing && wave == 0) draw();
    }
    if (!product_first) tile_pass<F, true, false, false, ST>(y, cw, cnt, prow, sp, lane, 0, ent_col, ent_c, Y);
    product();
    if (product_first) tile_pass<F, true, false, false, ST>(y, cw, cnt, prow, sp, lane, 0, ent_col, ent_c, Y);
    if constexpr (TICKETS) {
      if (drawing && wave == 0) take_draw();
    }
    __syncthreads();
    if constexpr (TICKETS) {
      t_new = drawing ? (int)__builtin_amdgcn_readfirstlane(*reinterpret_cast<volatile unsigned *>(ticket_word)) : groups;
    }
    collect(Ap);
#pragma unroll
    for (int cc = 0; cc < FC; ++cc) p[cc] = r[cc] = sp[cc] - Ap[cc];
    float rsold = dot_compact<F>(r, r);
    bool active = valid && rsold >= 1e-20f;
    const bool store = active;
    for (int it = 0; it + 1 < cg_steps; ++it) {
      publish(p, active);
      if (active && !product_first) tile_pass<F, false, false, false, ST>(y, cw, cnt, prow, sp, lane, 0, ent_col, ent_c, Y);
      product();
      if (active && product_first) tile_pass<F, false, false, false, ST>(y, cw, cnt, prow, sp, lane, 0, ent_col, ent_c, Y);
      __syncthreads();
      collect(Ap);
      if (active) {
#pragma unroll
        for (int cc = 0; cc < FC; ++cc) Ap[cc] += sp[cc];
        const float alpha = rsold * __builtin_amdgcn_rcpf(dot_compact<F>(p, Ap));
#pragma unroll
        for (int cc = 0; cc < FC; ++cc) {
          xc[cc] = fmaf(alpha, p[cc], xc[cc]);
          r[cc] = fmaf(-alpha, Ap[cc], r[cc]);
        }
        const float rsnew = dot_compact<F>(r, r);
        if (rsnew < 1e-20f) {
          active = false;
        } else {
          const float beta = rsnew * __builtin_amdgcn_rcpf(rsold);
#pragma unroll
          for (int cc = 0; cc < FC; ++cc) p[cc] = fmaf(beta, p[cc], r[cc]);
          rsold = rsnew;
        }
      }
    }
    bool rolled = false;
    if (cg_steps > 0) {
      publish(p, active);
      float tile_pAp = 0.f;
      auto last_tiles = [&]() {
        if constexpr (ROLL) tile_pAp = tile_pass<F, false, true, true, ST>(y, cw, cnt, prow, sp, lane, ent_cnt, ent_col, ent_c, Y);
        else tile_pAp = tile_pass<F, false, true, false, ST>(y, cw, cnt, prow, sp, lane, 0, ent_col, ent_c, Y);
      };
      if (active && !product_first) last_tiles();
      product();
      if (active && product_first) last_tiles();
      __syncthreads();
      collect(Ap);
      if (active) {
        if constexpr (ROLL) {
          cnt = ent_cnt;
          ent_cnt = row_valid(t2) ? e2 - b2 : 0;
          fetch_entries(indices, data, opaque(lane), b2, max(e2, b2 + 1), ent_col, ent_c);
          load_compact<F>(X + (size_t)id1 * F, opaque(lane), x);
          rolled = true;
        } else {
          kill(x);
        }
        const float alpha = rsold * __builtin_amdgcn_rcpf(wave_allsum(dot_local<FC>(p, Ap) + tile_pAp));
#pragma unroll
        for (int cc = 0; cc < FC; ++cc) xc[cc] = fmaf(alpha, p[cc], xc[cc]);
      } else {
        kill(x);
      }
    } else {
      kill(x);
    }
    if (store) store_compact<F>(xrow, opaque(lane), xc);
    tile_ready = rolled;
    g = t1, t1 = t2, t2 = t3, t3 = t_new;
    id0 = id1, id1 = id2, id2 = id3, id3 = row_id(t3);
    b0 = b1, e0 = e1, b1 = b2, e1 = e2, b2 = indptr[id2], e2 = indptr[id2 + 1];
  }
}

template <int F, typename ST>
__global__ __launch_bounds__(1024) void als_cg_qfgroup_kernel(const int32_t *__restrict__ order, int first, int count,
                                                              const int32_t *__restrict__ indptr,
                                                              const int32_t *__restrict__ indices,
                                                              const float *__restrict__ data, ST *__restrict__ X,
                                                              const ST *__restrict__ Y, const float *__restrict__ A0, int cg_steps) {
  group_stage_gramian<F>(A0);
  group_rows<F, ST>(order, first, count, indptr, indices, data, X, Y, cg_steps);
}

template <typename T>
static void launch_qfgroup(const imp_csr *C, int first, int count, T *X, const T *Y, const float *A0, int cg_steps, const char *name) {
  if (count <= 0) return;
  constexpr int F = 128;
  const size_t lds = QFGroupCfg<F>::lds_bytes;
  auto kern = als_cg_qfgroup_kernel<F, T>;
  allow_dynamic_lds(kern, lds);
  int grid = std::min((count + 15) / 16, ctx().num_cus * std::max(2, ctx().oversub));
  IMP_PROF(name);
  kern<<<grid, 1024, lds, stream()>>>(C->order.data(), first, count, C->indptr.data(), C->indices.data(), C->data.data(), X, Y, A0,
                                      cg_steps);
  IMP_CHECK_HIP(hipGetLastError());
}

#ifndef IMP_WIDE_FORM
#define IMP_WIDE_FORM 0
#endif
struct WideClassArgs {
  int first[WideTickets::kClasses], count[WideTickets::kClasses];
  unsigned base[WideTickets::kClasses][WideTickets::kQueues];
};
static_assert(WideTickets::kQueues == kTicketQueues && WideTickets::kGroupRows == 16, "queues and groups of the ticketed classes");
template <int F> constexpr size_t wide_chain_lds_bytes() {
  return std::max(team_lds_bytes<F, 16, 1024, 32>(), QFGroupCfg<F>::lds_bytes + 16);
}
template <int F, typename ST, bool SHORT_TICKETS>
__global__ __launch_bounds__(1024) void als_cg_qfwide_chain_kernel(const int32_t *__restrict__ order, WideClassArgs cls,
                                                                   unsigned *__restrict__ counters,
                                                                   const int32_t *__restrict__ indptr,
                                                                   const int32_t *__restrict__ indices,
                                                                   const float *__restrict__ data, ST *__restrict__ X,
                                                                   const ST *__restrict__ Y, const float *__restrict__ A0,
                                                                   int cg_steps) {
  const unsigned queue = blockIdx.x % kTicketQueues;
  if (cls.count[0] > 0)
    team_rows<Tile32<ST>, F, 16, 1024, true, true>(order, cls.first[0], cls.count[0], indptr, indices, data, X, Y, A0, cg_steps,
                                                   counters + queue * WideTickets::kCounterStride, cls.base[0][queue]);
  if (cls.count[1] > 0) {
    if (cls.count[0] > 0) __syncthreads();
    group_stage_gramian<F>(A0);
    group_rows<F, ST, SHORT_TICKETS>(order, cls.first[1], cls.count[1], indptr, indices, data, X, Y, cg_steps,
                                     counters + (kTicketQueues + queue) * WideTickets::kCounterStride, cls.base[1][queue]);
  }
}

template <typename T>
void launch_wide_chain(const imp_csr *C, int f, const int (&first)[2], const int (&count)[2], T *X, const T *Y, const float *A0, int cg_steps,
                       const char *name) {
  if constexpr (std::is_same<T, float>::value) {
    if (f != 128) throw std::invalid_argument("launch_wide_chain: f must be 128");
    constexpr int F = 128;
    constexpr bool kShortTickets = IMP_WIDE_FORM != 1;
    if (count[0] <= 0 && count[1] <= 0) return;
    const size_t lds = wide_chain_lds_bytes<F>();
    auto kern = als_cg_qfwide_chain_kernel<F, T, kShortTickets>;
    static const int per_cu = [&] {
      int n = 0;
      allow_dynamic_lds(kern, lds);
      IMP_CHECK_HIP(hipOccupancyMaxActiveBlocksPerMultiprocessor(&n, reinterpret_cast<const void *>(kern), 1024, lds));
      if (n < 1) throw std::runtime_error("launch_wide_chain: the kernel does not fit a compute unit");
      return n;
    }();
    allow_dynamic_lds(kern, lds);
    const int grid = std::max(ctx().num_cus * per_cu, WideTickets::kQueues);
    for (int c = 0; c < 2; ++c)
      if (count[c] >= WideTickets::kMaxCount) throw std::invalid_argument("launch_wide_chain: too many rows in a class");
    Context &cx = ctx();
    cx.wide_counters.reserve((size_t)WideTickets::kClasses * WideTickets::kQueues * WideTickets::kCounterStride, true);
    auto run = [&](bool on0, bool on1) {
      WideClassArgs cls;
      const int32_t rows[2] = {on0 ? std::max(count[0], 0) : 0, on1 ? std::max(count[1], 0) : 0};
      if (rows[0] == 0 && rows[1] == 0) return;
      for (int c = 0; c < 2; ++c) cls.first[c] = first[c], cls.count[c] = rows[c];
      WideTickets after = cx.wide_tickets;
      const int32_t ticketed[2] = {rows[0], kShortTickets ? rows[1] : 0};
      after.launch_rows(ticketed, grid, cls.base);
      kern<<<grid, 1024, lds, stream()>>>(C->order.data(), cls, cx.wide_counters.data(), C->indptr.data(), C->indices.data(),
                                         C->data.data(), X, Y, A0, cg_steps);
      IMP_CHECK_HIP(hipGetLastError());
      cx.wide_tickets = after;
    };
    IMP_PROF(name);
    if (IMP_WIDE_FORM == 2) run(true, false), run(false, true);
    else run(true, true);
  } else {
    throw std::invalid_argument("launch_wide_chain: fp32 storage only");
  }
}
template void launch_wide_chain<float>(const imp_csr *, int, const int (&)[2], const int (&)[2], float *, const float *, const float *, int,
                                       const char *);
template void launch_wide_chain<__half>(const imp_csr *, int, const int (&)[2], const int (&)[2], __half *, const __half *, const float *,
                                        int, const char *);

template <typename T>
void launch_group_fused(const imp_csr *C, int f, int first, int count, T *X, const T *Y, const float *A0, int cg_steps, const char *name) {
  if (f == 128) launch_qfgroup<T>(C, first, count, X, Y, A0, cg_steps, name);
  else throw std::invalid_argument("launch_group_fused: f must be 128 (f = 64 short rows run on independent wavefronts)");
}
template void launch_group_fused<float>(const imp_csr *, int, int, int, float *, const float *, const float *, int, const char *);
template void launch_group_fused<__half>(const imp_csr *, int, int, int, __half *, const __half *, const float *, int, const char *);

template <typename T>
void launch_team_fused(const imp_csr *C, int f, int width, int first, int count, T *X, const T *Y, const float *A0, int cg_steps,
                       const char *name) {
  if constexpr (std::is_same<T, __half>::value) {
    if (f != 64 || width != 1) throw std::invalid_argument("launch_team_fused: float16 storage takes the f = 64 short rows only");
    launch_qfteam<64, 1, 512, T>(C, first, count, X, Y, A0, cg_steps, name);
  } else {
    auto run = [&](auto Fc) {
      constexpr int F = decltype(Fc)::value;
      switch (width) {
        case 16: launch_qfteam<F, 16, 1024, T>(C, first, count, X, Y, A0, cg_steps, name); break;
        case 8: launch_qfteam<F, 8, 512, T>(C, first, count, X, Y, A0, cg_steps, name); break;
        case 4: launch_qfteam<F, 4, 512, T>(C, first, count, X, Y, A0, cg_steps, name); break;
        case 2: launch_qfteam<F, 2, 512, T>(C, first, count, X, Y, A0, cg_steps, name); break;
        case 1:
          if constexpr (F == 64) launch_qfteam<F, 1, 512, T>(C, first, count, X, Y, A0, cg_steps, name);
          else throw std::invalid_argument("launch_team_fused: one wave per row needs f = 64");
          break;
        default: throw std::invalid_argument("launch_team_fused: team width");
      }
    };
    if (f == 128) run(idx_t<128>{});
    else if (f == 64) run(idx_t<64>{});
    else throw std::invalid_argument("launch_team_fused: f must be 64 or 128");
  }
}
template void launch_team_fused<float>(const imp_csr *, int, int, int, int, float *, const float *, const float *, int, const char *);
template void launch_team_fused<__half>(const imp_csr *, int, int, int, int, __half *, const __half *, const float *, int,
                                        const char *);

}
```

implicit_amd/csrc/common.h:

```cpp
#ifndef IMPLICIT_AMD_CSRC_COMMON_H_
#define IMPLICIT_AMD_CSRC_COMMON_H_

#include <hip/hip_runtime.h>

#include <climits>
#include <cstdint>
#include <cstdio>
#include <memory>
#include <mutex>
#include <optional>
#include <stdexcept>
#include <string>
#include <vector>

#include "../../include/implicit_hip.h"
#include "csr_schedule.h"
#include "team_tickets.h"

namespace imp {

struct out_of_range_error : std::runtime_error {
  using std::runtime_error::runtime_error;
};

// ... 139 lines not shown
  bool deferred = false;
  hipStream_t occupy_stream = nullptr;
  std::recursive_mutex mutex;
  std::mutex small_mutex;
  std::vector<void *> small_free[24];
  void *pin_stage = nullptr;
  size_t pin_stage_bytes = 0;
  hipEvent_t pin_stage_ev = nullptr;
  DeviceArray<float> gram_ws;
  DeviceArray<float> long_ws;
  PaddedSystem pad;
  DeviceArray<double> loss_buf;
  DeviceArray<unsigned long long> fail_word;
  DeviceArray<float> barrier_word;
  unsigned long long *fixup_total = nullptr;
  DeviceArray<float> w256_ws;
  DeviceArray<unsigned> nm_fix_rows;
  DeviceArray<unsigned> chain_counters;
  ChainTickets chain_tickets;
  DeviceArray<unsigned> wide_counters;
  WideTickets wide_tickets;
  DeviceArray<int> nm_ticket;
  DeviceArray<unsigned long long> pair_stats;
  DeviceArray<float> lmf_ws;
  DeviceArray<double> knn_acc;
  DeviceArray<int32_t> knn_touched;
  int knn_cols = -1;
  DeviceArray<float> subspace_pred;
  DeviceArray<float> subspace_ws;
};
inline hipStream_t stream() { return ctx().stream; }

template <typename K> void allow_dynamic_lds(K *kernel, size_t bytes) {
  IMP_CHECK_HIP(hipFuncSetAttribute(reinterpret_cast<const void *>(kernel), hipFuncAttributeMaxDynamicSharedMemorySize, (int)bytes));
}
template <auto Kernel> void allow_dynamic_lds_once(size_t bytes) {
  static bool done[64] = {};
  const int dev = ctx().device;
  if (dev >= 0 && dev < 64 && done[dev]) return;
  allow_dynamic_lds(Kernel, bytes);
  if (dev >= 0 && dev < 64) done[dev] = true;
}

constexpr unsigned long long kNoFailure = ~0ULL;
unsigned long long *reset_fail_word();
int64_t read_fail_word(const unsigned long long *w);

imp_matrix *new_matrix(size_t rows, size_t cols, size_t itemsize, bool zero);
std::unique_ptr<imp_matrix> astype(const imp_matrix *src, size_t itemsize);
template <typename T> void pad_rows(int grid, const T *src, float *dst, size_t rows, int f, int F, const int *skip = nullptr);
void zero_rows(const int32_t *order, int first, int count, float *X, int f);
void note_device_write(const void *dst, size_t bytes);
struct DerivedCache {
  const void *src = nullptr;
  size_t bytes = 0;
};
void register_derived_cache(DerivedCache *c);
void unregister_derived_cache(DerivedCache *c);

}

struct imp_matrix {
  size_t rows = 0, cols = 0, itemsize = 4;
  void *data = nullptr;
  std::shared_ptr<imp::Storage> storage;
  size_t bytes() const { return rows * cols * itemsize; }
  float *f32() const {
    if (itemsize != 4) throw std::runtime_error("can't cast Matrix to float*");
    return reinterpret_cast<float *>(data);
  }
};

struct imp_intvector {
  imp::DeviceArray<int32_t> v;
  size_t size = 0;
};

struct LongPlanDev {
  int n_long, n_seg;
  const int32_t *rows;
  const int32_t *row_seg;
  const int32_t *seg_row;
  const int32_t *seg_begin;
  const int32_t *seg_end;
  const int32_t *seg_exec;
  int xcd_start[9];
};

struct LongPlan {
  int32_t n_long = 0, n_seg = 0;
  imp::DeviceArray<int32_t> row_seg, seg_row, seg_begin, seg_end, seg_exec;
  int32_t xcd_start[9] = {0, 0, 0, 0, 0, 0, 0, 0, 0};
  void upload(const imp::HostPlan &p) {
    n_long = p.n_long, n_seg = p.n_seg;
    seg_exec.upload(p.seg_exec.data(), p.seg_exec.size());
    row_seg.upload(p.row_seg.data(), p.row_seg.size());
    seg_row.upload(p.seg_row.data(), p.seg_row.size());
    seg_begin.upload(p.seg_begin.data(), p.seg_begin.size());
    seg_end.upload(p.seg_end.data(), p.seg_end.size());
    for (int x = 0; x < 9; ++x) xcd_start[x] = p.xcd_start[x];
  }
  LongPlanDev dev(const int32_t *rows) const {
    LongPlanDev d{n_long, n_seg, rows, row_seg.data(), seg_row.data(), seg_begin.data(), seg_end.data(), seg_exec.data(), {0}};
    for (int x = 0; x < 9; ++x) d.xcd_start[x] = xcd_start[x];
    return d;
  }
};

struct imp_csr : imp::CsrClasses {
  int32_t rows = 0, cols = 0;
  int64_t nnz = 0;
  imp::DeviceArray<int32_t> indptr, indices;
  imp::DeviceArray<float> data;
  imp::DeviceArray<int32_t> order;
  int32_t bin_start[kBins + 1] = {0, 0, 0, 0, 0, 0, 0, 0, 0};
  LongPlan plan_all;
  LongPlan plan_chol;
  int32_t n_chol_long = 0;
  LongPlan plan_nm;
  int32_t nm_segment = 2048, nm_multi_rows = 0, nm_multi_segs = 0;
  std::vector<std::unique_ptr<imp_csr>> parts;
  std::vector<int32_t> part_row0;
  int32_t nonempty() const { return bin_start[kBins - 1]; }
  int32_t first_empty() const { return bin_start[kBins - 1]; }
  int32_t n_empty() const { return bin_start[kBins] - bin_start[kBins - 1]; }
};

struct imp_coo {
  int32_t rows = 0, cols = 0;
  int64_t nnz = 0;
  imp::DeviceArray<int32_t> row, col;
  imp::DeviceArray<float> data;
};

namespace imp {
struct PaddedViews {
  imp_matrix X, Y, YtY;
};
PaddedViews pad_in(const imp_matrix *X, const imp_matrix *Y, const imp_matrix *YtY, size_t rows_of_X, int F, bool reuse_y);
void pad_out(imp_matrix *X, size_t rows_of_X, int F);
struct CholNmList {
  const unsigned *count, *rows;
  int capacity;
};
CholNmList least_squares_cholesky_nm(const imp_csr *C, float *X, const float *Y, size_t y_rows, const float *YtY, float reg);
template <int F, typename T>
void launch_cg_fixup(const unsigned *count, const unsigned *rows, int capacity, const imp_csr *C, T *X, const T *Y, const float *A0,
                     int cg_steps);

void gramian(const float *Y, long n_rows, int f, float reg, float *out);
void gramian_half(const void *Y, long n_rows, int f, float reg, float *out);
bool cg_native_half(int f);
void least_squares_cg(const imp_csr *C, imp_matrix *X, const imp_matrix *YtY, const imp_matrix *Y, int cg_steps);
template <typename T> void least_squares_cg_q(const imp_csr *C, T *X, const T *Y, const float *A0, int f, int cg_steps);
void least_squares_cg_w256(const imp_csr *C, float *X, const float *Y, const float *A0, int cg_steps);
template <typename T>
void least_squares_cg_nm(const imp_csr *C, T *X, const T *Y, size_t y_rows, const float *A0, int f, int cg_steps);
int64_t least_squares_cholesky(const imp_csr *C, imp_matrix *X, const imp_matrix *YtY, const imp_matrix *Y, double reg);
int64_t least_squares_subspace(const imp_csr *C, imp_matrix *X, const imp_matrix *YtY, const imp_matrix *Y, double reg, int block_size,
                               int sweeps);
size_t knn_temp_budget(const imp_knn *k);
}

#endif
```

implicit_amd/csrc/containers.hip:

```cpp
#include <hip/hip_fp16.h>

#include <algorithm>
#include <cstring>
#include <map>
#include <mutex>
#include <thread>

#include "common.h"

namespace imp {

static thread_local std::string g_last_error;
void set_last_error(const std::string &msg) { g_last_error = msg; }

static std::mutex g_ctx_mutex;
static auto &g_contexts = *new std::map<int, std::unique_ptr<Context>>;

Context &ctx() {
  int dev = 0;
  IMP_CHECK_HIP(hipGetDevice(&dev));
  std::lock_guard<std::mutex> lock(g_ctx_mutex);
  auto it = g_contexts.find(dev);
  if (it == g_contexts.end()) {
    auto c = std::make_unique<Context>();
    c->device = dev;
    IMP_CHECK_HIP(hipStreamCreateWithFlags(&c->stream, hipStreamNonBlocking));
    hipDeviceProp_t prop;
    IMP_CHECK_HIP(hipGetDeviceProperties(&prop, dev));
    c->num_cus = prop.multiProcessorCount;
    if (const char *e = getenv("IMP_OVERSUB")) c->oversub = std::max(1, atoi(e));
    it = g_contexts.emplace(dev, std::move(c)).first;
  }
  return *it->second;
}

static auto &g_derived = *new std::vector<DerivedCache *>;
void register_derived_cache(DerivedCache *c) {
  std::lock_guard<std::mutex> lock(g_ctx_mutex);
  g_derived.push_back(c);
}
void unregister_derived_cache(DerivedCache *c) {
  std::lock_guard<std::mutex> lock(g_ctx_mutex);
  g_derived.erase(std::remove(g_derived.begin(), g_derived.end(), c), g_derived.end());
}

void note_device_write(const void *dst, size_t bytes) {
  const char *a = static_cast<const char *>(dst);
  std::lock_guard<std::mutex> lock(g_ctx_mutex);
  for (DerivedCache *d : g_derived) {
    const char *b = static_cast<const char *>(d->src);
    if (b && a < b + d->bytes && b < a + bytes) d->src = nullptr;
  }
  for (auto &kv : g_contexts) {
    PaddedSystem &pad = kv.second->pad;
    if (pad.y_made_from(dst, bytes)) pad.forget_y();
  }
}

std::unique_lock<std::recursive_mutex> lock_device() {
  try {
    return std::unique_lock<std::recursive_mutex>(ctx().mutex);
  } catch (...) {
    return std::unique_lock<std::recursive_mutex>();
  }
}

static bool env_unless_zero(const char *name) {
  const char *e = getenv(name);
  return !(e && atoi(e) == 0);
}
const SolverSwitches &solver_switches() {
  static const SolverSwitches s = [] {
    SolverSwitches v;
    v.nm = env_unless_zero("IMP_NM");
    v.w256 = getenv("IMP_F256_OLD") == nullptr;
    v.cg_pad = getenv("IMP_NO_PAD") == nullptr;
    v.chol_nm = env_unless_zero("IMP_CHOL_NM");
    v.chol_pad = v.chol_nm && env_unless_zero("IMP_CHOL_PAD");
    return v;
  }();
  return s;
}

void sync() { IMP_CHECK_HIP(hipStreamSynchronize(stream())); }
void sync_call() {
  if (!ctx().deferred) sync();
}

unsigned long long *reset_fail_word() {
  unsigned long long *w = ctx().fail_word.reserve(1);
  IMP_CHECK_HIP(hipMemsetAsync(w, 0xFF, sizeof(unsigned long long), stream()));
  return w;
}
int64_t read_fail_word(const unsigned long long *w) {
  unsigned long long failed = 0;
  IMP_CHECK_HIP(hipMemcpyAsync(&failed, w, sizeof(failed), hipMemcpyDeviceToHost, stream()));
  sync();
  return failed == kNoFailure ? -1 : (int64_t)failed;
}

struct ProfEntry {
  double total_ms = 0;
  int64_t launches = 0;
};
struct ProfPending {
  const char *name;
  hipEvent_t start, stop;
};
static std::recursive_mutex g_prof_mutex;
static bool g_prof_on = false;
static std::string g_prof_filter;
static std::map<std::string, ProfEntry> g_prof;
static std::vector<ProfPending> g_prof_pending;
static std::vector<hipEvent_t> g_event_pool;

bool prof_enabled() { return g_prof_on; }
bool prof_unfiltered() {
  std::lock_guard<std::recursive_mutex> plock(g_prof_mutex);
  return g_prof_on && g_prof_filter.empty();
}

static hipEvent_t get_event() {
  if (!g_event_pool.empty()) {
    hipEvent_t e = g_event_pool.back();
    g_event_pool.pop_back();
    return e;
  }
  hipEvent_t e;
  IMP_CHECK_HIP(hipEventCreate(&e));
  return e;
}

static void prof_account(const ProfPending &p) {
  float ms = 0;
  if (hipEventElapsedTime(&ms, p.start, p.stop) == hipSuccess) {
    auto &e = g_prof[p.name];
    e.total_ms += ms;
    e.launches += 1;
  }
  g_event_pool.push_back(p.start);
  g_event_pool.push_back(p.stop);
}

static void prof_collect_finished() {
  size_t done = 0;
  while (done < g_prof_pending.size() && hipEventQuery(g_prof_pending[done].stop) == hipSuccess) prof_account(g_prof_pending[done++]);
  if (done) g_prof_pending.erase(g_prof_pending.begin(), g_prof_pending.begin() + (long)done);
}

ProfScope::ProfScope(const char *n) : name(n) {
  if (!g_prof_on) return;
  std::lock_guard<std::recursive_mutex> plock(g_prof_mutex);
  if (!g_prof_filter.empty() && !strstr(n, g_prof_filter.c_str())) return;
  if (g_event_pool.size() < 2 && g_prof_pending.size() >= 32) prof_collect_finished();
  start = get_event();
  stop = get_event();
  IMP_CHECK_HIP(hipEventRecord(start, stream()));
}

ProfScope::~ProfScope() {
  if (!start) return;
// ... 313 lines not shown
    if (indptr[0] != 0 || indptr[rows] != nnz) throw std::invalid_argument("host_csr_transpose: indptr does not span the nonzeros");
    int T = std::max(1, std::min(threads > 0 ? threads : (int)std::thread::hardware_concurrency() / 2, 32));
    while (T > 1 && (size_t)T * (size_t)cols > ((size_t)64 << 20)) --T;
    if (nnz < (1 << 16)) T = 1;
    std::vector<int32_t> cut(T + 1, rows);
    cut[0] = 0;
    for (int t = 1; t < T; ++t) {
      const int64_t target = nnz * t / T;
      cut[t] = (int32_t)(std::lower_bound(indptr, indptr + rows + 1, (int32_t)target) - indptr);
      cut[t] = std::min(rows, std::max(cut[t], cut[t - 1]));
    }
    for (int32_t r = 0; r < rows; ++r)
      if (indptr[r + 1] < indptr[r]) throw std::invalid_argument("host_csr_transpose: indptr must be non-decreasing (row " + std::to_string(r) + ")");
    std::vector<std::vector<int32_t>> hist(T);
    for (auto &h : hist) h.assign((size_t)cols, 0);
    std::string error;
    std::mutex error_mutex;
    auto parallel = [&](auto &&fn) {
      auto fenced = [&](int t) {
        try {
          fn(t);
        } catch (const std::exception &e) {
          std::lock_guard<std::mutex> g(error_mutex);
          if (error.empty()) error = std::string("host_csr_transpose: ") + e.what();
        } catch (...) {
          std::lock_guard<std::mutex> g(error_mutex);
          if (error.empty()) error = "host_csr_transpose: unknown failure in a worker thread";
        }
      };
      std::vector<std::thread> pool;
      pool.reserve((size_t)T);
      int started = 1;
      try {
        for (; started < T; ++started) pool.emplace_back(fenced, started);
      } catch (...) {
      }
      fenced(0);
      for (int t = started; t < T; ++t) fenced(t);
      for (auto &th : pool) th.join();
      if (!error.empty()) throw std::invalid_argument(error);
    };
    parallel([&](int t) {
      auto &h = hist[t];
      for (int64_t k = indptr[cut[t]]; k < indptr[cut[t + 1]]; ++k) {
        const int32_t c = indices[k];
        if (c < 0 || c >= cols) throw std::invalid_argument("column index out of range");
        ++h[c];
      }
    });
    parallel([&](int t) {
      const int32_t c0 = (int32_t)((int64_t)cols * t / T), c1 = (int32_t)((int64_t)cols * (t + 1) / T);
      for (int32_t c = c0; c < c1; ++c) {
        int32_t sum = 0;
        for (int u = 0; u < T; ++u) sum += hist[u][c];
        t_indptr[c + 1] = sum;
      }
    });
    t_indptr[0] = 0;
    for (int32_t c = 0; c < cols; ++c) t_indptr[c + 1] += t_indptr[c];
    parallel([&](int t) {
      const int32_t c0 = (int32_t)((int64_t)cols * t / T), c1 = (int32_t)((int64_t)cols * (t + 1) / T);
      for (int32_t c = c0; c < c1; ++c) {
        int32_t at = t_indptr[c];
        for (int u = 0; u < T; ++u) {
          const int32_t n = hist[u][c];
          hist[u][c] = at;
          at += n;
        }
      }
    });
    parallel([&](int t) {
      auto &pos = hist[t];
      for (int32_t r = cut[t]; r < cut[t + 1]; ++r)
        for (int32_t k = indptr[r]; k < indptr[r + 1]; ++k) {
          const int32_t at = pos[indices[k]]++;
          t_indices[at] = r;
          t_data[at] = data[k];
        }
    });
  });
}

int imp_host_csr_plan(int32_t rows, int32_t cols, const int32_t *indptr, const int32_t *indices, int32_t segment, int32_t stripe,
                      int32_t nm_segment, int32_t num_cus, int which, int32_t *order, int32_t *bin_start, int32_t *row_seg,
                      int64_t seg_capacity, int32_t *seg_row, int32_t *seg_begin, int32_t *seg_end, int32_t *seg_exec,
                      int32_t *xcd_start, int32_t *info) {
  return guarded_host([&] {
    if (which < 0 || which > 2) throw std::invalid_argument("host_csr_plan: which must be 0 (all), 1 (chol) or 2 (nm)");
    if (nm_segment < 0) throw std::invalid_argument("host_csr_plan: nm_segment must be positive, or 0 for the automatic length");
    if (rows < 0) throw std::invalid_argument("negative dimension for CSRMatrix");
    validate_csr(rows, cols, rows ? (int64_t)indptr[rows] : 0, indptr, indices);
    PlanKnobs knobs;
    knobs.segment = segment, knobs.stripe = stripe, knobs.nm_segment = nm_segment, knobs.num_cus = num_cus;
    const HostSchedule s = plan_csr(rows, cols, indptr, indices, knobs);
    const HostPlan &p = which == 0 ? s.plan_all : which == 1 ? s.plan_chol : s.plan_nm;
    if (p.n_seg > seg_capacity) throw std::invalid_argument("host_csr_plan: the plan has more segments than seg_capacity");
    std::copy(s.order.begin(), s.order.end(), order);
    std::copy(s.bin_start, s.bin_start + imp_csr::kBins + 1, bin_start);
    std::copy(p.row_seg.begin(), p.row_seg.end(), row_seg);
    std::copy(p.seg_row.begin(), p.seg_row.end(), seg_row);
    std::copy(p.seg_begin.begin(), p.seg_begin.end(), seg_begin);
    std::copy(p.seg_end.begin(), p.seg_end.end(), seg_end);
    std::copy(p.seg_exec.begin(), p.seg_exec.end(), seg_exec);
    std::copy(p.xcd_start, p.xcd_start + 9, xcd_start);
    const int32_t fields[8] = {p.n_long, p.n_seg, p.striped, s.n_chol_long, s.nm_segment, s.nm_multi_rows, s.nm_multi_segs, 0};
    std::copy(fields, fields + 8, info);
  });
}

int imp_host_chain_tickets(uint32_t *next, const int32_t *count, int32_t workgroups, const int32_t *teams_per_workgroup, uint32_t *base,
                           uint32_t *draws) {
  return guarded_host([&] {
    constexpr int NC = ChainTickets::kClasses, NQ = ChainTickets::kQueues;
    ChainTickets t;
    int32_t c[NC], n[NC];
    uint32_t b[NC][NQ];
    if (workgroups <= 0) throw std::invalid_argument("host_chain_tickets: the grid holds at least one workgroup");
    for (int k = 0; k < NC; ++k) {
      if (count[k] < 0 || count[k] >= ChainTickets::kMaxCount || teams_per_workgroup[k] <= 0)
        throw std::invalid_argument("host_chain_tickets: a class holds 0 .. 2^30 - 1 rows and a workgroup at least one team");
      c[k] = count[k], n[k] = teams_per_workgroup[k];
      for (int q = 0; q < NQ; ++q) t.next[k][q] = next[k * NQ + q];
    }
    t.launch(c, workgroups, n, b);
    for (int k = 0; k < NC; ++k)
      for (int q = 0; q < NQ; ++q) {
        draws[k * NQ + q] = t.next[k][q] - next[k * NQ + q];
        next[k * NQ + q] = t.next[k][q], base[k * NQ + q] = b[k][q];
      }
  });
}

int imp_host_wide_tickets(uint32_t *next, const int32_t *rows, int32_t workgroups, uint32_t *base, uint32_t *draws) {
  return guarded_host([&] {
    constexpr int NC = WideTickets::kClasses, NQ = WideTickets::kQueues;
    WideTickets t;
    uint32_t b[NC][NQ];
    if (workgroups <= 0) throw std::invalid_argument("host_wide_tickets: the grid holds at least one workgroup");
    for (int k = 0; k < NC; ++k) {
      if (rows[k] < 0 || rows[k] >= WideTickets::kMaxCount)
        throw std::invalid_argument("host_wide_tickets: a class holds 0 .. 2^30 - 1 rows");
      for (int q = 0; q < NQ; ++q) t.next[k][q] = next[k * NQ + q];
    }
    const int32_t r[NC] = {rows[0], rows[1]};
    t.launch_rows(r, workgroups, b);
    for (int k = 0; k < NC; ++k)
      for (int q = 0; q < NQ; ++q) {
        draws[k * NQ + q] = t.next[k][q] - next[k * NQ + q];
        next[k * NQ + q] = t.next[k][q], base[k * NQ + q] = b[k][q];
      }
  });
}

int imp_matrix_create(size_t rows, size_t cols, const void *host_data, size_t itemsize, imp_matrix **out) {
  return guarded([&] {
    imp_matrix *m = new_matrix(rows, cols, itemsize, host_data == nullptr);
    std::unique_ptr<imp_matrix> guard(m);
    if (host_data && m->bytes()) {
      IMP_CHECK_HIP(hipMemcpyAsync(m->data, host_data, m->bytes(), hipMemcpyHostToDevice, stream()));
    }
    sync();
    *out = guard.release();
  });
}

int imp_matrix_wrap_device(size_t rows, size_t cols, void *device_ptr, size_t itemsize, imp_matrix **out) {
  return guarded([&] {
    if (itemsize != 4 && itemsize != 2) throw std::invalid_argument("invalid itemsize for Matrix (must be 2 or 4)");
    auto m = std::make_unique<imp_matrix>();
    m->rows = rows;
    m->cols = cols;
    m->itemsize = itemsize;
    m->storage = std::make_shared<Storage>(device_ptr);
    m->data = device_ptr;
    *out = m.release();
  });
}

int imp_matrix_row(const imp_matrix *src, size_t rowid, imp_matrix **out) {
  return guarded([&] {
    if (rowid >= src->rows) throw std::invalid_argument("row index out of bounds for matrix");
    auto m = std::make_unique<imp_matrix>(*src);
    m->rows = 1;
    m->data = reinterpret_cast<char *>(src->data) + rowid * src->cols * src->itemsize;
    *out = m.release();
  });
}

int imp_matrix_slice(const imp_matrix *src, size_t start, size_t end, imp_matrix **out) {
  return guarded([&] {
    if (end < start) throw std::invalid_argument("end_rowid < start_rowid for matrix slice");
    if (end > src->rows) throw std::invalid_argument("row index out of bounds for matrix");
    auto m = std::make_unique<imp_matrix>(*src);
    m->rows = end - start;
    m->data = reinterpret_cast<char *>(src->data) + start * src->cols * src->itemsize;
    *out = m.release();
  });
}

int imp_matrix_gather(const imp_matrix *src, const imp_intvector *rowids, imp_matrix **out) {
  return guarded([&] {
    std::unique_ptr<imp_matrix> m(new_matrix(rowids->size, src->cols, src->itemsize, false));
    size_t total = m->rows * m->cols;
    if (total) {
      IMP_PROF("gather_rows");
      if (src->itemsize == 4)
        gather_rows_kernel<float><<<grid_for(total), 256, 0, stream()>>>(
            (const float *)src->data, rowids->v.data(), (float *)m->data, m->rows, m->cols);
      else
        gather_rows_kernel<__half><<<grid_for(total), 256, 0, stream()>>>(
            (const __half *)src->data, rowids->v.data(), (__half *)m->data, m->rows, m->cols);
      IMP_CHECK_HIP(hipGetLastError());
    }
    sync();
    *out = m.release();
  });
}

int imp_matrix_resize(imp_matrix *m, size_t rows, size_t cols) {
  return guarded([&] {
    if (cols != m->cols) throw std::logic_error("changing number of columns in Matrix::resize is not implemented yet");
    if (rows < m->rows) throw std::logic_error("reducing number of rows in Matrix::resize is not implemented yet");
    auto storage = std::make_shared<Storage>(rows * cols * m->itemsize, true);
    if (m->bytes()) IMP_CHECK_HIP(hipMemcpyAsync(storage->ptr, m->data, m->bytes(), hipMemcpyDeviceToDevice, stream()));
    sync();
    m->storage = storage;
    m->data = storage->ptr;
    m->rows = rows;
  });
}

int imp_matrix_assign_rows(imp_matrix *m, const imp_intvector *rowids, const imp_matrix *other) {
  return guarded([&] {
    if (other->cols != m->cols) throw std::invalid_argument("column dimension mismatch for Matrix::assign_rows");
    if (other->rows != rowids->size) throw std::invalid_argument("row dimension mismatch for Matrix::assign_rows");
    if (other->itemsize != m->itemsize) throw std::invalid_argument("dtype mismatch for Matrix::assign_rows");
    size_t total = other->rows * other->cols;
    note_device_write(m->data, m->bytes());
    if (total) {
      IMP_PROF("scatter_rows");
      if (m->itemsize == 4)
        scatter_rows_kernel<float><<<grid_for(total), 256, 0, stream()>>>(m->f32(), rowids->v.data(), other->f32(), other->rows,
                                                                          other->cols);
      else
        scatter_rows_kernel<__half><<<grid_for(total), 256, 0, stream()>>>((__half *)m->data, rowids->v.data(),
                                                                           (const __half *)other->data, other->rows, other->cols);
      IMP_CHECK_HIP(hipGetLastError());
    }
    sync();
  });
}

int imp_matrix_astype(const imp_matrix *src, size_t itemsize, imp_matrix **out) {
  return guarded([&] { *out = astype(src, itemsize).release(); });
}

int imp_matrix_calculate_norms(const imp_matrix *src, imp_matrix **out) {
  return guarded([&] {
    std::unique_ptr<imp_matrix> m(new_matrix(1, src->rows, 4, false));
    if (src->rows) {
      IMP_PROF("row_norms");
      int grid = grid_for(src->rows * 64);
      if (src->itemsize == 4)
        row_norms_kernel<float><<<grid, 256, 0, stream()>>>((const float *)src->data, (float *)m->data, src->rows, src->cols);
      else
        row_norms_kernel<__half><<<grid, 256, 0, stream()>>>((const __half *)src->data, (float *)m->data, src->rows, src->cols);
      IMP_CHECK_HIP(hipGetLastError());
    }
    sync();
    *out = m.release();
  });
}

int imp_matrix_to_host(const imp_matrix *m, void *host_out) {
  return guarded([&] {
    if (m->bytes()) IMP_CHECK_HIP(hipMemcpyAsync(host_out, m->data, m->bytes(), hipMemcpyDeviceToHost, stream()));
    sync();
  });
}

int imp_matrix_from_host(imp_matrix *m, const void *host_in) {
  return guarded([&] {
    note_device_write(m->data, m->bytes());
    if (m->bytes()) IMP_CHECK_HIP(hipMemcpyAsync(m->data, host_in, m->bytes(), hipMemcpyHostToDevice, stream()));
    sync();
  });
}

int imp_matrix_copy_rows(imp_matrix *dst, size_t dst_row, const imp_matrix *src, size_t src_row, size_t rows) {
  return guarded([&] {
    if (dst->cols != src->cols || dst->itemsize != src->itemsize)
      throw std::invalid_argument("copy_rows: the two matrices must have rows of the same width and itemsize");
    if (dst_row + rows > dst->rows || src_row + rows > src->rows) throw imp::out_of_range_error("copy_rows: row range out of bounds");
    const size_t row_bytes = dst->cols * dst->itemsize;
    note_device_write(static_cast<char *>(dst->data) + dst_row * row_bytes, rows * row_bytes);
    if (rows && row_bytes)
      IMP_CHECK_HIP(hipMemcpyAsync(static_cast<char *>(dst->data) + dst_row * row_bytes,
                                   static_cast<const char *>(src->data) + src_row * row_bytes, rows * row_bytes,
                                   hipMemcpyDeviceToDevice, stream()));
    sync_call();
  });
}

int imp_matrix_shape(const imp_matrix *m, size_t *rows, size_t *cols, size_t *itemsize) {
  return guarded([&] {
    if (rows) *rows = m->rows;
// ... 237 lines not shown
```

implicit_amd/gpu/_hip.py:

```python
import ctypes
import os

_HERE = os.path.dirname(os.path.abspath(__file__))
from .. import _libpath

LIB_PATH = _libpath.OVERRIDE or os.path.join(os.path.dirname(_HERE), "libimplicit_hip.so")

c_void_pp = ctypes.POINTER(ctypes.c_void_p)
c_i32_p = ctypes.POINTER(ctypes.c_int32)
c_f32_p = ctypes.POINTER(ctypes.c_float)

IMP_OK, IMP_INVALID_ARGUMENT, IMP_OUT_OF_RANGE, IMP_RUNTIME_ERROR = 0, 1, 2, 3

_SIGNATURES = {
    "imp_get_device_count": [ctypes.POINTER(ctypes.c_int)],
    "imp_set_device": [ctypes.c_int],
    "imp_get_device": [ctypes.POINTER(ctypes.c_int)],
    "imp_set_oversubscribe": [ctypes.c_int],
    "imp_get_oversubscribe": [ctypes.POINTER(ctypes.c_int)],
    "imp_set_deferred_sync": [ctypes.c_int],
    "imp_debug_occupy": [ctypes.c_int, ctypes.c_int],
    "imp_debug_core_clock": [ctypes.c_int, ctypes.POINTER(ctypes.c_double)],
    "imp_device_synchronize": [],
    "imp_solver_fixup_rows": [ctypes.POINTER(ctypes.c_ulonglong), ctypes.c_int],
    "imp_mem_get_info": [ctypes.POINTER(ctypes.c_size_t), ctypes.POINTER(ctypes.c_size_t)],
    "imp_release_workspaces": [],
    "imp_host_csr_transpose": [ctypes.c_int32, ctypes.c_int32, ctypes.c_int64, ctypes.c_void_p, ctypes.c_void_p, ctypes.c_void_p,
                               ctypes.c_void_p, ctypes.c_void_p, ctypes.c_void_p, ctypes.c_int],
    "imp_host_csr_plan": [ctypes.c_int32, ctypes.c_int32, ctypes.c_void_p, ctypes.c_void_p, ctypes.c_int32, ctypes.c_int32,
                          ctypes.c_int32, ctypes.c_int32, ctypes.c_int, ctypes.c_void_p, ctypes.c_void_p, ctypes.c_void_p,
                          ctypes.c_int64, ctypes.c_void_p, ctypes.c_void_p, ctypes.c_void_p, ctypes.c_void_p, ctypes.c_void_p,
                          ctypes.c_void_p],
    "imp_host_chain_tickets": [ctypes.c_void_p, ctypes.c_void_p, ctypes.c_int32, ctypes.c_void_p, ctypes.c_void_p, ctypes.c_void_p],
    "imp_host_wide_tickets": [ctypes.c_void_p, ctypes.c_void_p, ctypes.c_int32, ctypes.c_void_p, ctypes.c_void_p],
    "imp_matrix_create": [ctypes.c_size_t, ctypes.c_size_t, ctypes.c_void_p, ctypes.c_size_t, c_void_pp],
    "imp_matrix_wrap_device": [ctypes.c_size_t, ctypes.c_size_t, ctypes.c_void_p, ctypes.c_size_t, c_void_pp],
    "imp_matrix_row": [ctypes.c_void_p, ctypes.c_size_t, c_void_pp],
    "imp_matrix_slice": [ctypes.c_void_p, ctypes.c_size_t, ctypes.c_size_t, c_void_pp],
    "imp_matrix_gather": [ctypes.c_void_p, ctypes.c_void_p, c_void_pp],
    "imp_matrix_resize": [ctypes.c_void_p, ctypes.c_size_t, ctypes.c_size_t],
    "imp_matrix_assign_rows": [ctypes.c_void_p, ctypes.c_void_p, ctypes.c_void_p],
    "imp_matrix_astype": [ctypes.c_void_p, ctypes.c_size_t, c_void_pp],
    "imp_matrix_calculate_norms": [ctypes.c_void_p, c_void_pp],
    "imp_matrix_to_host": [ctypes.c_void_p, ctypes.c_void_p],
    "imp_matrix_from_host": [ctypes.c_void_p, ctypes.c_void_p],
    "imp_matrix_copy_rows": [ctypes.c_void_p, ctypes.c_size_t, ctypes.c_void_p, ctypes.c_size_t, ctypes.c_size_t],
    "imp_matrix_shape": [ctypes.c_void_p, ctypes.POINTER(ctypes.c_size_t), ctypes.POINTER(ctypes.c_size_t),
                         ctypes.POINTER(ctypes.c_size_t)],
    "imp_matrix_device_ptr": [ctypes.c_void_p, c_void_pp],
    "imp_matrix_destroy": [ctypes.c_void_p],
    "imp_intvector_create": [ctypes.c_void_p, ctypes.c_size_t, c_void_pp],
    "imp_intvector_destroy": [ctypes.c_void_p],
    "imp_csr_create": [ctypes.c_int32, ctypes.c_int32, ctypes.c_int64, ctypes.c_void_p, ctypes.c_void_p,
                       ctypes.c_void_p, c_void_pp],
    "imp_csr_create64": [ctypes.c_int32, ctypes.c_int32, ctypes.c_int64, ctypes.c_void_p, ctypes.c_void_p,
                         ctypes.c_void_p, c_void_pp],
    "imp_csr_shape": [ctypes.c_void_p, c_i32_p, c_i32_p, ctypes.POINTER(ctypes.c_int64)],
    "imp_csr_destroy": [ctypes.c_void_p],
    "imp_coo_create": [ctypes.c_int32, ctypes.c_int32, ctypes.c_int64, ctypes.c_void_p, ctypes.c_void_p,
                       ctypes.c_void_p, c_void_pp],
    "imp_coo_create_from_csr_pattern": [ctypes.c_int32, ctypes.c_int32, ctypes.c_void_p, ctypes.c_int, ctypes.c_void_p,
                                        ctypes.POINTER(ctypes.c_void_p)],
    "imp_coo_destroy": [ctypes.c_void_p],
    "imp_solver_create": [c_void_pp],
    "imp_solver_destroy": [ctypes.c_void_p],
    "imp_solver_calculate_yty": [ctypes.c_void_p, ctypes.c_void_p, ctypes.c_void_p, ctypes.c_float],
    "imp_solver_least_squares": [ctypes.c_void_p, ctypes.c_void_p, ctypes.c_void_p, ctypes.c_void_p,
                                 ctypes.c_void_p, ctypes.c_int],
    "imp_solver_least_squares_cholesky": [ctypes.c_void_p, ctypes.c_void_p, ctypes.c_void_p, ctypes.c_void_p,
                                          ctypes.c_void_p, ctypes.c_double, ctypes.POINTER(ctypes.c_int64)],
    "imp_solver_least_squares_subspace": [ctypes.c_void_p, ctypes.c_void_p, ctypes.c_void_p, ctypes.c_void_p,
                                          ctypes.c_void_p, ctypes.c_double, ctypes.c_int, ctypes.c_int,
                                          ctypes.POINTER(ctypes.c_int64)],
    "imp_solver_calculate_loss": [ctypes.c_void_p, ctypes.c_void_p, ctypes.c_void_p, ctypes.c_void_p,
                                  ctypes.c_float, c_f32_p],
    "imp_solver_explain_factor": [ctypes.c_void_p, ctypes.c_void_p, ctypes.c_void_p, ctypes.c_void_p, ctypes.c_double,
                                  ctypes.c_void_p, ctypes.POINTER(ctypes.c_int64)],
    "imp_solver_explain": [ctypes.c_void_p, ctypes.c_void_p, ctypes.c_void_p, ctypes.c_void_p, ctypes.c_void_p, ctypes.c_int,
                           ctypes.c_int, ctypes.c_void_p, ctypes.c_void_p, ctypes.c_void_p],
    "imp_knn_create": [ctypes.c_size_t, c_void_pp],
    "imp_knn_destroy": [ctypes.c_void_p],
    "imp_knn_topk": [ctypes.c_void_p, ctypes.c_void_p, ctypes.c_void_p, ctypes.c_int, ctypes.c_void_p,
                     ctypes.c_void_p, ctypes.c_void_p, ctypes.c_void_p, ctypes.c_void_p],
    "imp_knn_rank": [ctypes.c_void_p, ctypes.c_void_p, ctypes.c_void_p, ctypes.c_void_p, ctypes.c_void_p, ctypes.c_int,
                     ctypes.c_void_p, ctypes.c_void_p, ctypes.c_void_p, ctypes.c_void_p],
    "imp_random_create": [ctypes.c_int64, c_void_pp],
    "imp_random_destroy": [ctypes.c_void_p],
    "imp_random_uniform": [ctypes.c_void_p, ctypes.c_size_t, ctypes.c_size_t, ctypes.c_float, ctypes.c_float,
                           c_void_pp],
    "imp_random_randn": [ctypes.c_void_p, ctypes.c_size_t, ctypes.c_size_t, ctypes.c_float, ctypes.c_float,
                         c_void_pp],
    "imp_bpr_update": [ctypes.c_void_p, ctypes.c_void_p, ctypes.c_void_p, ctypes.c_void_p, ctypes.c_void_p, ctypes.c_float,
                       ctypes.c_float, ctypes.c_int64, ctypes.c_int, ctypes.c_int64, ctypes.POINTER(ctypes.c_int64),
                       ctypes.POINTER(ctypes.c_int64)],
    "imp_warp_update": [ctypes.c_void_p, ctypes.c_void_p, ctypes.c_void_p, ctypes.c_void_p, ctypes.c_void_p, ctypes.c_float,
                        ctypes.c_float, ctypes.c_int64, ctypes.c_int, ctypes.c_int64, ctypes.POINTER(ctypes.c_int64),
                        ctypes.POINTER(ctypes.c_int64)],
    "imp_lmf_update": [ctypes.c_void_p, ctypes.c_void_p, ctypes.c_void_p, ctypes.c_void_p, ctypes.c_float, ctypes.c_float,
                       ctypes.c_int, ctypes.c_int64, ctypes.c_int],
    "imp_spmat_create": [ctypes.c_int32, ctypes.c_int32, ctypes.c_int64, ctypes.c_void_p, ctypes.c_void_p, ctypes.c_void_p,
                         c_void_pp],
    "imp_spmat_destroy": [ctypes.c_void_p],
    "imp_sparse_topk_product": [ctypes.c_void_p, ctypes.c_void_p, ctypes.c_int, ctypes.c_int, ctypes.c_void_p, ctypes.c_void_p,
                                ctypes.c_void_p],
    "imp_eval_create": [ctypes.c_int32, ctypes.c_int32, ctypes.c_void_p, ctypes.c_int, ctypes.c_void_p, ctypes.c_int,
                        ctypes.c_void_p, ctypes.c_void_p, c_void_pp],
    "imp_eval_add": [ctypes.c_void_p, ctypes.c_void_p, ctypes.c_void_p, ctypes.c_void_p],
    "imp_eval_result": [ctypes.c_void_p, ctypes.c_void_p],
    "imp_eval_reset": [ctypes.c_void_p],
    "imp_eval_destroy": [ctypes.c_void_p],
    "imp_host_ranking_metrics": [ctypes.c_int32, ctypes.c_int32, ctypes.c_void_p, ctypes.c_int, ctypes.c_void_p, ctypes.c_int,
                                 ctypes.c_void_p, ctypes.c_void_p, ctypes.c_void_p, ctypes.c_void_p, ctypes.c_int64,
                                 ctypes.c_void_p, ctypes.c_void_p],
    "imp_ivf_build": [ctypes.c_void_p, ctypes.c_int, ctypes.c_int, ctypes.c_void_p, c_void_pp],
    "imp_ivf_shape": [ctypes.c_void_p, ctypes.POINTER(ctypes.c_size_t), ctypes.POINTER(ctypes.c_size_t),
                      ctypes.POINTER(ctypes.c_int)],
    "imp_ivf_set_temp_memory": [ctypes.c_void_p, ctypes.c_size_t],
    "imp_ivf_lists": [ctypes.c_void_p, ctypes.c_void_p, ctypes.c_void_p, ctypes.c_void_p],
    "imp_ivf_search": [ctypes.c_void_p, ctypes.c_void_p, ctypes.c_int, ctypes.c_int, ctypes.c_void_p, ctypes.c_void_p,
                       ctypes.c_void_p],
    "imp_ivf_destroy": [ctypes.c_void_p],
    "imp_ease_gram": [ctypes.c_void_p, ctypes.c_void_p, ctypes.c_float, ctypes.c_void_p],
    "imp_spd_inverse": [ctypes.c_void_p, ctypes.POINTER(ctypes.c_int64)],
    "imp_ease_weights": [ctypes.c_void_p],
    "imp_ease_topk": [ctypes.c_void_p, ctypes.c_void_p, ctypes.c_int32, ctypes.c_void_p, ctypes.c_void_p, ctypes.c_void_p,
                      ctypes.c_int, ctypes.c_int, ctypes.c_void_p, ctypes.c_void_p, ctypes.c_void_p],
    "imp_csr_spmm": [ctypes.c_void_p, ctypes.c_void_p, ctypes.c_void_p],
    "imp_matrix_multiply_small": [ctypes.c_void_p, ctypes.c_void_p, ctypes.c_void_p],
    "imp_comm_unique_id": [ctypes.c_void_p],
    "imp_comm_init_rank": [ctypes.c_void_p, ctypes.c_int, ctypes.c_int, c_void_pp],
    "imp_comm_destroy": [ctypes.c_void_p],
    "imp_comm_allreduce_sum": [ctypes.c_void_p, ctypes.c_void_p],
    "imp_comm_allgather_rows": [ctypes.c_void_p, ctypes.c_void_p, ctypes.POINTER(ctypes.c_int64)],
    "imp_comm_allgather_rows_begin": [ctypes.c_void_p, ctypes.c_void_p, ctypes.POINTER(ctypes.c_int64),
                                      ctypes.POINTER(ctypes.c_int64)],
    "imp_comm_allgather_rows_end": [ctypes.c_void_p],
    "imp_comm_alltoall_rows": [ctypes.c_void_p, ctypes.c_void_p, ctypes.POINTER(ctypes.c_int64), ctypes.POINTER(ctypes.c_int64),
                               ctypes.c_void_p, ctypes.POINTER(ctypes.c_int64), ctypes.POINTER(ctypes.c_int64)],
    "imp_comm_barrier": [ctypes.c_void_p],
    "imp_comm_ranks_seen": [ctypes.c_void_p, ctypes.POINTER(ctypes.c_int)],
    "imp_prof_enable": [ctypes.c_int],
    "imp_prof_filter": [ctypes.c_char_p],
    "imp_prof_reset": [],
    "imp_prof_get": [ctypes.c_char_p, ctypes.POINTER(ctypes.c_double), ctypes.POINTER(ctypes.c_int64)],
    "imp_prof_names": [ctypes.c_char_p, ctypes.c_size_t],
}
_RESTYPES = {"imp_last_error": ctypes.c_char_p, "imp_version": ctypes.c_char_p}

EXPORTED_SYMBOLS = sorted(list(_SIGNATURES) + list(_RESTYPES))

_lib = None


def lib():
    global _lib
    if _lib is None:
        if not os.path.exists(LIB_PATH):
            raise ImportError(
                f"{LIB_PATH} is missing: build it with `python -m implicit_amd._build` "
                "(hipcc --offload-arch=gfx950). There is no CPU fallback.")
        L = ctypes.CDLL(LIB_PATH)
        for name, argtypes in _SIGNATURES.items():
            fn = getattr(L, name)
            fn.argtypes = argtypes
            fn.restype = ctypes.c_int
        for name, restype in _RESTYPES.items():
            fn = getattr(L, name)
            fn.argtypes = []
            fn.restype = restype
        _lib = L
    return _lib


def check(status):
    if status == IMP_OK:
        return
    msg = (lib().imp_last_error() or b"").decode("utf-8", "replace")
    if status == IMP_INVALID_ARGUMENT:
        raise ValueError(msg)
    if status == IMP_OUT_OF_RANGE:
        raise IndexError(msg)
    raise RuntimeError(msg)
```

implicit_amd/utils.py:

```python
import time
import warnings

import numpy as np
import scipy.sparse


class ParameterWarning(Warning):
    """Raised (as a warning) when an input had to be converted (implicit/utils.py:155-156)."""


def check_csr(user_items):
    if isinstance(user_items, scipy.sparse.csr_matrix):
        return user_items
    kind = type(user_items).__name__
    t0 = time.time()
    converted = user_items.tocsr()
    warnings.warn(
        f"Method expects CSR input, and was passed {kind} instead. "
        f"Converting to CSR took {time.time() - t0} seconds",
        ParameterWarning,
    )
    return converted


# ... 6 lines not shown
def nonzeros(m, row):
    for k in range(m.indptr[row], m.indptr[row + 1]):
        yield m.indices[k], m.data[k]


def _id_array(a, what):
    a = np.asarray(a)
    if a.size and a.dtype.kind not in "iu":
        raise ValueError(f"{what} must hold integer item ids, got dtype {a.dtype}")
    return a if a.dtype.kind in "iu" else a.astype(np.int32)


def candidate_form(selected_items):
    if isinstance(selected_items, np.ndarray) and selected_items.dtype != object:
        if selected_items.ndim == 1:
            return "shared"
        if selected_items.ndim == 2:
            return "padded"
        raise ValueError(f"selected_items must be 1- or 2-dimensional, got {selected_items.ndim} dimensions")
    if np.isscalar(selected_items) or not hasattr(selected_items, "__len__"):
        raise ValueError("selected_items must be an array of item ids or a sequence of such arrays")
    if all(np.isscalar(x) for x in selected_items):
        return "shared"
    return "ragged"


def candidate_lists(selected_items, batch):
    form = candidate_form(selected_items)
    if form == "shared":
        ids = _id_array(selected_items, "selected_items")
        lengths = np.full(batch, len(ids), dtype=np.int64)
        flat = np.tile(ids, batch)
    elif form == "padded":
        ids = _id_array(selected_items, "selected_items")
        if ids.shape[0] != batch:
            raise ValueError("selected_items must contain 1 row for every user in userids")
        keep = ids >= 0
        lengths = keep.sum(axis=1).astype(np.int64)
        flat = ids.reshape(-1) if keep.all() else ids[keep]
    else:
        if len(selected_items) != batch:
            raise ValueError("selected_items must contain 1 list for every user in userids")
        rows = [_id_array(x, "every list of selected_items") for x in selected_items]
        if any(x.ndim != 1 for x in rows):
            raise ValueError("every list of selected_items must be 1-dimensional")
        lengths = np.array([len(x) for x in rows], dtype=np.int64)
        flat = np.concatenate(rows) if rows else np.zeros(0, dtype=np.int32)
    if flat.size and flat.dtype != np.int32 and (flat.max() > np.iinfo(np.int32).max or flat.min() < np.iinfo(np.int32).min):
        raise IndexError("Some itemids are not in the model")
    offsets = np.zeros(batch + 1, dtype=np.int64)
    np.cumsum(lengths, out=offsets[1:])
    return offsets, np.ascontiguousarray(flat, dtype=np.int32)


def random_factors(rng, rows, cols, scale=0.01, workers=None):
    import os
    from concurrent.futures import ThreadPoolExecutor

    n = rows * cols
    bg = rng.bit_generator
    state = bg.state if type(bg).__name__ == "PCG64" else None
    if state is None or n % 2 or n < (1 << 20) or state.get("has_uint32", 0):
        return rng.random((rows, cols), dtype=np.float32) * scale
    if workers is None:
        workers = max(1, min(16, (os.cpu_count() or 2) // 2))
    out = np.empty(n, dtype=np.float32)
    chunk = ((n // workers + 1) // 2) * 2
    scale32 = np.float32(scale)

    def fill(start):
        stop = min(n, start + chunk)
        g = np.random.PCG64()
        g.state = state
        g.advance(start // 2)
        np.random.Generator(g).random(stop - start, dtype=np.float32, out=out[start:stop])
        out[start:stop] *= scale32

    with ThreadPoolExecutor(max_workers=workers) as ex:
        list(ex.map(fill, range(0, n, chunk)))
    bg.advance(n // 2)
    return out.reshape(rows, cols)


def transpose_csr(m, threads=0):
    ok = (isinstance(m, scipy.sparse.csr_matrix) and m.dtype == np.float32 and m.indptr.dtype == np.int32
          and m.indices.dtype == np.int32 and m.nnz < 2**31 - 1 and m.has_canonical_format)
    if ok:
        try:
            from .gpu._hip import check, lib

            fn = lib().imp_host_csr_transpose
        except (ImportError, OSError, AttributeError):
            ok = False
    if not ok:
        return m.T.tocsr()
    rows, cols = m.shape
    indptr, indices, data = (np.ascontiguousarray(a) for a in (m.indptr, m.indices, m.data))
    t_indptr = np.empty(cols + 1, dtype=np.int32)
    t_indices = np.empty(m.nnz, dtype=np.int32)
    t_data = np.empty(m.nnz, dtype=np.float32)
    check(fn(rows, cols, m.nnz, indptr.ctypes.data, indices.ctypes.data, data.ctypes.data, t_indptr.ctypes.data,
             t_indices.ctypes.data, t_data.ctypes.data, int(threads)))
    out = scipy.sparse.csr_matrix((t_data, t_indices, t_indptr), shape=(cols, rows), copy=False)
    out.has_sorted_indices = True
    out.has_canonical_format = True
    return out


def csr_schedule(m, which=0, segment=512, stripe=-1, nm_segment=0, num_cus=256):
    from .gpu._hip import check, lib

    rows, cols = m.shape
    indptr = np.ascontiguousarray(m.indptr, dtype=np.int32)
    indices = np.ascontiguousarray(m.indices, dtype=np.int32)
    capacity = max(int(indptr[-1]), 0) if rows else 0
    out = {"order": np.empty(rows, np.int32), "bin_start": np.empty(9, np.int32), "row_seg": np.empty(rows + 1, np.int32)}
    segs = {k: np.empty(capacity, np.int32) for k in ("seg_row", "seg_begin", "seg_end", "seg_exec")}
    out["xcd_start"] = np.empty(9, np.int32)
    info = np.zeros(8, np.int32)
    check(lib().imp_host_csr_plan(rows, cols, indptr.ctypes.data, indices.ctypes.data, segment, stripe, nm_segment, num_cus, which,
                                  out["order"].ctypes.data, out["bin_start"].ctypes.data, out["row_seg"].ctypes.data, capacity,
                                  *(segs[k].ctypes.data for k in ("seg_row", "seg_begin", "seg_end", "seg_exec")),
                                  out["xcd_start"].ctypes.data, info.ctypes.data))
    names = ("n_long", "n_seg", "striped", "n_chol_long", "nm_segment", "nm_multi_rows", "nm_multi_segs")
    out.update({k: int(v) for k, v in zip(names, info)})
    out["striped"] = bool(out["striped"])
    out["row_seg"] = out["row_seg"][:out["n_long"] + 1]
    out.update({k: v[:out["n_seg"]] for k, v in segs.items()})
    return out


def chain_tickets(state, counts, workgroups, teams_per_workgroup=(1, 2, 4)):
    from .gpu._hip import check, lib

    assert state.dtype == np.uint32 and state.shape == (3, 8) and state.flags.c_contiguous
    counts = np.ascontiguousarray(counts, dtype=np.int32)
    teams = np.ascontiguousarray(teams_per_workgroup, dtype=np.int32)
    assert counts.shape == teams.shape == (3,)
    base, draws = np.empty((3, 8), np.uint32), np.empty((3, 8), np.uint32)
    check(lib().imp_host_chain_tickets(state.ctypes.data, counts.ctypes.data, int(workgroups), teams.ctypes.data, base.ctypes.data,
                                       draws.ctypes.data))
    return base, draws


def wide_tickets(state, rows, workgroups):
    from .gpu._hip import check, lib

    assert state.dtype == np.uint32 and state.shape == (2, 8) and state.flags.c_contiguous
    rows = np.ascontiguousarray(rows, dtype=np.int32)
    assert rows.shape == (2,)
    base, draws = np.empty((2, 8), np.uint32), np.empty((2, 8), np.uint32)
    check(lib().imp_host_wide_tickets(state.ctypes.data, rows.ctypes.data, int(workgroups), base.ctypes.data, draws.ctypes.data))
    return base, draws
```

include/implicit_hip.h:

```cpp
#ifndef IMPLICIT_HIP_H_
#define IMPLICIT_HIP_H_

#include <stddef.h>
#include <stdint.h>

#ifdef __cplusplus
extern "C" {
#endif

typedef enum {
  IMP_OK = 0,
  IMP_INVALID_ARGUMENT = 1,
  IMP_OUT_OF_RANGE = 2,
  IMP_RUNTIME_ERROR = 3
} imp_status;

typedef struct imp_matrix imp_matrix;
typedef struct imp_intvector imp_intvector;
typedef struct imp_csr imp_csr;
typedef struct imp_coo imp_coo;
typedef struct imp_solver imp_solver;
typedef struct imp_knn imp_knn;
typedef struct imp_random imp_random;
typedef struct imp_comm imp_comm;

const char *imp_last_error(void);
int imp_get_device_count(int *count);
int imp_set_device(int device);
int imp_get_device(int *device);
int imp_set_oversubscribe(int factor);
int imp_get_oversubscribe(int *factor);
int imp_set_deferred_sync(int on);
int imp_debug_occupy(int workgroups, int microseconds);
int imp_debug_core_clock(int microseconds, double *mhz);
int imp_device_synchronize(void);
int imp_solver_fixup_rows(unsigned long long *count, int reset);
int imp_mem_get_info(size_t *free_bytes, size_t *total_bytes);
int imp_release_workspaces(void);
const char *imp_version(void);

int imp_host_csr_transpose(int32_t rows, int32_t cols, int64_t nonzeros, const int32_t *indptr, const int32_t *indices,
                           const float *data, int32_t *t_indptr, int32_t *t_indices, float *t_data, int threads);

int imp_host_csr_plan(int32_t rows, int32_t cols, const int32_t *indptr, const int32_t *indices, int32_t segment, int32_t stripe,
                      int32_t nm_segment, int32_t num_cus, int which, int32_t *order, int32_t *bin_start, int32_t *row_seg,
                      int64_t seg_capacity, int32_t *seg_row, int32_t *seg_begin, int32_t *seg_end, int32_t *seg_exec,
                      int32_t *xcd_start, int32_t *info);

int imp_host_chain_tickets(uint32_t *next, const int32_t *count, int32_t workgroups, const int32_t *teams_per_workgroup, uint32_t *base,
                           uint32_t *draws);

int imp_host_wide_tickets(uint32_t *next, const int32_t *rows, int32_t workgroups, uint32_t *base, uint32_t *draws);

int imp_matrix_create(size_t rows, size_t cols, const void *host_data, size_t itemsize, imp_matrix **out);
int imp_matrix_wrap_device(size_t rows, size_t cols, void *device_ptr, size_t itemsize, imp_matrix **out);
int imp_matrix_row(const imp_matrix *m, size_t rowid, imp_matrix **out);
int imp_matrix_slice(const imp_matrix *m, size_t start, size_t end, imp_matrix **out);
int imp_matrix_gather(const imp_matrix *m, const imp_intvector *rowids, imp_matrix **out);
int imp_matrix_resize(imp_matrix *m, size_t rows, size_t cols);
int imp_matrix_assign_rows(imp_matrix *m, const imp_intvector *rowids, const imp_matrix *other);
int imp_matrix_astype(const imp_matrix *m, size_t itemsize, imp_matrix **out);
int imp_matrix_calculate_norms(const imp_matrix *m, imp_matrix **out);
int imp_matrix_to_host(const imp_matrix *m, void *host_out);
int imp_matrix_from_host(imp_matrix *m, const void *host_in);
int imp_matrix_copy_rows(imp_matrix *dst, size_t dst_row, const imp_matrix *src, size_t src_row, size_t rows);
int imp_matrix_shape(const imp_matrix *m, size_t *rows, size_t *cols, size_t *itemsize);
int imp_matrix_device_ptr(const imp_matrix *m, void **ptr);
int imp_matrix_destroy(imp_matrix *m);

int imp_intvector_create(const int32_t *host_data, size_t size, imp_intvector **out);
int imp_intvector_destroy(imp_intvector *v);
int imp_csr_create(int32_t rows, int32_t cols, int64_t nonzeros, const int32_t *indptr,
                   const int32_t *indices, const float *data, imp_csr **out);
int imp_csr_create64(int32_t rows, int32_t cols, int64_t nonzeros, const int64_t *indptr,
                     const int32_t *indices, const float *data, imp_csr **out);
int imp_csr_shape(const imp_csr *m, int32_t *rows, int32_t *cols, int64_t *nonzeros);
int imp_csr_destroy(imp_csr *m);
int imp_coo_create(int32_t rows, int32_t cols, int64_t nonzeros, const int32_t *row,
                   const int32_t *col, const float *data, imp_coo **out);
int imp_coo_create_from_csr_pattern(int32_t rows, int32_t cols, const void *indptr, int indptr_is_64,
                                    const int32_t *indices, imp_coo **out);
int imp_coo_destroy(imp_coo *m);

int imp_solver_create(imp_solver **out);
int imp_solver_destroy(imp_solver *s);
int imp_solver_calculate_yty(imp_solver *s, const imp_matrix *Y, imp_matrix *YtY, float regularization);
int imp_solver_least_squares(imp_solver *s, const imp_csr *cui, imp_matrix *X, const imp_matrix *YtY,
                             const imp_matrix *Y, int cg_steps);
int imp_solver_least_squares_cholesky(imp_solver *s, const imp_csr *cui, imp_matrix *X,
                                      const imp_matrix *YtY, const imp_matrix *Y,
                                      double regularization, int64_t *failed_row);
int imp_solver_least_squares_subspace(imp_solver *s, const imp_csr *cui, imp_matrix *X, const imp_matrix *YtY,
                                      const imp_matrix *Y, double regularization, int block_size, int sweeps,
                                      int64_t *failed_row);
int imp_solver_calculate_loss(imp_solver *s, const imp_csr *cui, const imp_matrix *X,
                              const imp_matrix *Y, float regularization, float *loss_out);
int imp_solver_explain_factor(imp_solver *s, const imp_csr *cui, const imp_matrix *YtY, const imp_matrix *Y,
                              double regularization, imp_matrix *weights, int64_t *failed_row);
int imp_solver_explain(imp_solver *s, const imp_csr *cui, const imp_matrix *Y, const imp_matrix *weights,
                       const imp_intvector *itemids, int items_per_row, int n, float *total, int32_t *ids, float *scores);

int imp_knn_create(size_t max_temp_memory, imp_knn **out);
int imp_knn_destroy(imp_knn *k);
int imp_knn_topk(imp_knn *k, const imp_matrix *items, const imp_matrix *query, int topk,
                 int32_t *indices, float *distances, const imp_matrix *item_norms,
                 const imp_coo *query_filter, const imp_intvector *item_filter);
int imp_knn_rank(imp_knn *k, const imp_matrix *items, const imp_matrix *query, const int64_t *offsets,
                 const int32_t *candidates, int n, const int64_t *liked_indptr, const int32_t *liked_indices,
                 int32_t *indices, float *scores);

int imp_random_create(int64_t seed, imp_random **out);
int imp_random_destroy(imp_random *r);
int imp_random_uniform(imp_random *r, size_t rows, size_t cols, float low, float high, imp_matrix **out);
int imp_random_randn(imp_random *r, size_t rows, size_t cols, float mean, float stddev, imp_matrix **out);

int imp_bpr_update(const imp_intvector *userids, const imp_intvector *itemids, const imp_intvector *indptr, imp_matrix *X,
                   imp_matrix *Y, float learning_rate, float regularization, int64_t seed, int verify_negative, int64_t samples,
                   int64_t *correct, int64_t *skipped);

int imp_warp_update(const imp_intvector *userids, const imp_intvector *itemids, const imp_intvector *indptr, imp_matrix *X,
                    imp_matrix *Y, float learning_rate, float regularization, int64_t seed, int max_sampled, int64_t samples,
                    int64_t *satisfied, int64_t *trials);

int imp_lmf_update(const imp_csr *cui, imp_matrix *X, const imp_matrix *Y, imp_matrix *deriv_sum_sq, float learning_rate,
                   float regularization, int neg_prop, int64_t seed, int one_col);

typedef struct imp_spmat imp_spmat;
int imp_spmat_create(int32_t rows, int32_t cols, int64_t nnz, const int64_t *indptr, const int32_t *indices,
                     const double *data, imp_spmat **out);
int imp_spmat_destroy(imp_spmat *m);
int imp_sparse_topk_product(const imp_spmat *A, const imp_spmat *B, int k, int zero_own_columns, int32_t *ids,
                            double *scores, int32_t *counts);

typedef struct imp_eval imp_eval;
int imp_eval_create(int32_t rows, int32_t cols, const void *indptr, int indptr_is_64, const int32_t *indices, int k,
                    const double *cg, const double *cg_sum, imp_eval **out);
int imp_eval_add(imp_eval *e, const imp_matrix *ids, const imp_intvector *userids, double *per_row);
int imp_eval_result(imp_eval *e, double *out);
int imp_eval_reset(imp_eval *e);
int imp_eval_destroy(imp_eval *e);
int imp_host_ranking_metrics(int32_t rows, int32_t cols, const void *indptr, int indptr_is_64, const int32_t *indices, int k,
                             const double *cg, const double *cg_sum, const int32_t *ids, const int32_t *userids, int64_t n,
                             double *sums, double *per_row);

typedef struct imp_ivf imp_ivf;
int imp_ivf_build(const imp_matrix *vectors, int nlist, int iterations, const int32_t *init_rows, imp_ivf **out);
int imp_ivf_shape(const imp_ivf *ix, size_t *rows, size_t *cols, int *nlist);
int imp_ivf_set_temp_memory(imp_ivf *ix, size_t max_temp_memory);
int imp_ivf_lists(const imp_ivf *ix, float *centroids, int64_t *list_offsets, int32_t *list_ids);
int imp_ivf_search(imp_ivf *ix, const imp_matrix *query, int k, int nprobe, int32_t *indices, float *distances, int32_t *probes);
int imp_ivf_destroy(imp_ivf *ix);

int imp_ease_gram(const imp_csr *item_users, const imp_csr *user_items, float regularization, imp_matrix *G);
int imp_spd_inverse(imp_matrix *A, int64_t *failed_pivot);
int imp_ease_weights(imp_matrix *P);
int imp_ease_topk(imp_knn *k, const imp_matrix *B, int32_t rows, const int64_t *indptr, const int32_t *indices,
                  const float *data, int topk, int filter_liked, const imp_intvector *item_filter, int32_t *ids,
                  float *scores);

int imp_csr_spmm(const imp_csr *A, const imp_matrix *D, imp_matrix *out);
int imp_matrix_multiply_small(const imp_matrix *Y, const imp_matrix *W, imp_matrix *out);

#define IMP_COMM_UNIQUE_ID_BYTES 128
int imp_comm_unique_id(void *id_out);
int imp_comm_init_rank(const void *id, int nranks, int rank, imp_comm **out);
int imp_comm_destroy(imp_comm *c);
int imp_comm_allreduce_sum(imp_comm *c, imp_matrix *m);
int imp_comm_allgather_rows(imp_comm *c, imp_matrix *full, const int64_t *row_offsets);
int imp_comm_allgather_rows_begin(imp_comm *c, imp_matrix *full, const int64_t *row_lo, const int64_t *row_hi);
int imp_comm_allgather_rows_end(imp_comm *c);
int imp_comm_alltoall_rows(imp_comm *c, const imp_matrix *send, const int64_t *send_lo, const int64_t *send_hi,
                           imp_matrix *recv, const int64_t *recv_lo, const int64_t *recv_hi);
int imp_comm_barrier(imp_comm *c);
int imp_comm_ranks_seen(imp_comm *c, int *out);

int imp_prof_enable(int on);
int imp_prof_filter(const char *substr);
int imp_prof_reset(void);
int imp_prof_get(const char *kernel, double *total_ms, int64_t *launches);
int imp_prof_names(char *buf, size_t buflen);

#ifdef __cplusplus
}
#endif
#endif
```

Baseline: 178.2 million updates/s.

## Fold NM multi-segment finish and fault fixup into the team-chain long-tail schedule

The NM solver no longer launches its reduce/finish and fault-fixup kernels right after the main NM kernel. It returns an NmTail descriptor, and the q-tile CG stage routes that work through a long_tail_route decision: inside the team chain, behind it, or inside the wide chain. The CG fixup body is moved into a shared device function so the chained kernels can call it. The aim is to cut separate kernel launches and tail idle time by overlapping the long-row finish with other row classes, at the cost of more complex cross-kernel ordering.

```diff
diff --git a/implicit_amd/csrc/als_cg.hip b/implicit_amd/csrc/als_cg.hip
--- a/implicit_amd/csrc/als_cg.hip
+++ b/implicit_amd/csrc/als_cg.hip
@@ -563,9 +563,10 @@
 template <int VPL, typename T>
 static void cg_f64_f128(const imp_csr *C, T *X, const T *Y, size_t y_rows, const float *A0, int cg_steps) {
   constexpr int f = 64 * VPL;
-  if (solver_switches().nm) least_squares_cg_nm<T>(C, X, Y, y_rows, A0, f, cg_steps);
+  NmTail tail;
+  if (solver_switches().nm) tail = least_squares_cg_nm<T>(C, X, Y, y_rows, A0, f, cg_steps);
   else launch_long<VPL, true, true, T>(C, C->plan_all, X, Y, A0, f, cg_steps);
-  least_squares_cg_q<T>(C, X, Y, A0, f, cg_steps);
+  least_squares_cg_q<T>(C, X, Y, A0, f, cg_steps, tail);
   zero_rows_t<T>(C->order.data(), C->first_empty(), C->n_empty(), X, f);
 }
 
diff --git a/implicit_amd/csrc/als_cg_fixup.h b/implicit_amd/csrc/als_cg_fixup.h
--- /dev/null
+++ b/implicit_amd/csrc/als_cg_fixup.h
@@ -0,0 +1,83 @@
+#ifndef IMPLICIT_AMD_CSRC_ALS_CG_FIXUP_H_
+#define IMPLICIT_AMD_CSRC_ALS_CG_FIXUP_H_
+
+#include "als_qtile.h"
+#include "common.h"
+#include "wave_ops.h"
+
+namespace imp {
+
+template <int F, typename ST>
+__device__ __forceinline__ void cg_fixup_row(float *vec, int lane, int u, const int32_t *__restrict__ indptr,
+                                             const int32_t *__restrict__ indices, const float *__restrict__ data, ST *__restrict__ X,
+                                             const ST *__restrict__ Y, const float *__restrict__ A0, int cg_steps) {
+  constexpr int FC = F / 64, U = 4;
+  auto load_vec = [&](const ST *row, float (&v)[FC]) {
+#pragma unroll
+    for (int c = 0; c < FC; ++c) v[c] = load1(row + FC * lane + c);
+  };
+  auto apply = [&](bool first, int rb, int re, const float (&v)[FC], float (&acc)[FC]) {
+#pragma unroll
+    for (int c = 0; c < FC; ++c) vec[FC * lane + c] = v[c];
+#pragma unroll
+    for (int c = 0; c < FC; ++c) acc[c] = 0.f;
+    for (int j = 0; j < F; ++j) {
+      const float vj = vec[j];
+#pragma unroll
+      for (int c = 0; c < FC; ++c) acc[c] = fmaf(A0[(size_t)j * F + FC * lane + c], vj, acc[c]);
+    }
+    if (first) {
+#pragma unroll
+      for (int c = 0; c < FC; ++c) acc[c] = -acc[c];
+    }
+    for (int k0 = rb; k0 < re; k0 += U) {
+      float conf[U], y[U][FC];
+#pragma unroll
+      for (int q = 0; q < U; ++q) {
+        const int k = min(k0 + q, re - 1);
+        conf[q] = data[k];
+        load_vec(Y + (size_t)indices[k] * F, y[q]);
+      }
+#pragma unroll
+      for (int q = 0; q < U; ++q) {
+        if (k0 + q < re) {
+          const float d = wave_allsum(dot_local<FC>(y[q], v));
+          const float cm1 = fabsf(conf[q]) - 1.f;
+          const float w = first ? fmaxf(conf[q], 0.f) - cm1 * d : cm1 * d;
+#pragma unroll
+          for (int c = 0; c < FC; ++c) acc[c] = fmaf(w, y[q][c], acc[c]);
+        }
+      }
+    }
+  };
+  const int rb = indptr[u], re = indptr[u + 1];
+  ST *xrow = X + (size_t)u * F;
+  float x[FC], r[FC], p[FC], Ap[FC];
+  load_vec(xrow, x);
+  apply(true, rb, re, x, r);
+#pragma unroll
+  for (int c = 0; c < FC; ++c) p[c] = r[c];
+  float rsold = wave_allsum(dot_local<FC>(r, r));
+  if (rsold < 1e-20f) return;
+  for (int it = 0; it < cg_steps; ++it) {
+    apply(false, rb, re, p, Ap);
+    const float alpha = rsold / wave_allsum(dot_local<FC>(p, Ap));
+#pragma unroll
+    for (int c = 0; c < FC; ++c) {
+      x[c] = fmaf(alpha, p[c], x[c]);
+      r[c] = fmaf(-alpha, Ap[c], r[c]);
+    }
+    const float rsnew = wave_allsum(dot_local<FC>(r, r));
+    if (rsnew < 1e-20f) break;
+    const float beta = rsnew / rsold;
+#pragma unroll
+    for (int c = 0; c < FC; ++c) p[c] = fmaf(beta, p[c], r[c]);
+    rsold = rsnew;
+  }
+#pragma unroll
+  for (int c = 0; c < FC; ++c) store1(xrow + FC * lane + c, x[c]);
+}
+
+}
+
+#endif
diff --git a/implicit_amd/csrc/als_cg_fixup.hip b/implicit_amd/csrc/als_cg_fixup.hip
--- a/implicit_amd/csrc/als_cg_fixup.hip
+++ b/implicit_amd/csrc/als_cg_fixup.hip
@@ -1,5 +1,6 @@
 #include <type_traits>
 
+#include "als_cg_fixup.h"
 #include "als_qtile.h"
 #include "common.h"
 
@@ -13,80 +14,14 @@
                                                                  const float *__restrict__ data, ST *__restrict__ X,
                                                                  const ST *__restrict__ Y, const float *__restrict__ A0, int cg_steps,
                                                                  unsigned long long *total) {
-  constexpr int FC = F / 64, WAVES = 4, U = 4;
+  constexpr int WAVES = 4;
   __shared__ float vecs[WAVES][F];
   const int n = min((int)fault_count[0], capacity);
   if (n == 0) return;
   if (blockIdx.x == 0 && threadIdx.x == 0) __hip_atomic_fetch_add(total, (unsigned long long)n, __ATOMIC_RELAXED, __HIP_MEMORY_SCOPE_SYSTEM);
   const int lane = threadIdx.x & 63, wave = threadIdx.x >> 6;
-  float *vec = vecs[wave];
-  auto load_vec = [&](const ST *row, float (&v)[FC]) {
-#pragma unroll
-    for (int c = 0; c < FC; ++c) v[c] = load1(row + FC * lane + c);
-  };
-  auto apply = [&](bool first, int rb, int re, const float (&v)[FC], float (&acc)[FC]) {
-#pragma unroll
-    for (int c = 0; c < FC; ++c) vec[FC * lane + c] = v[c];
-#pragma unroll
-    for (int c = 0; c < FC; ++c) acc[c] = 0.f;
-    for (int j = 0; j < F; ++j) {
-      const float vj = vec[j];
-#pragma unroll
-      for (int c = 0; c < FC; ++c) acc[c] = fmaf(A0[(size_t)j * F + FC * lane + c], vj, acc[c]);
-    }
-    if (first) {
-#pragma unroll
-      for (int c = 0; c < FC; ++c) acc[c] = -acc[c];
-    }
-    for (int k0 = rb; k0 < re; k0 += U) {
-      float conf[U], y[U][FC];
-#pragma unroll
-      for (int q = 0; q < U; ++q) {
-        const int k = min(k0 + q, re - 1);
-        conf[q] = data[k];
-        load_vec(Y + (size_t)indices[k] * F, y[q]);
-      }
-#pragma unroll
-      for (int q = 0; q < U; ++q) {
-        if (k0 + q < re) {
-          const float d = wave_allsum(dot_local<FC>(y[q], v));
-          const float cm1 = fabsf(conf[q]) - 1.f;
-          const float w = first ? fmaxf(conf[q], 0.f) - cm1 * d : cm1 * d;
-#pragma unroll
-          for (int c = 0; c < FC; ++c) acc[c] = fmaf(w, y[q][c], acc[c]);
-        }
-      }
-    }
-  };
-  for (int i = blockIdx.x * WAVES + wave; i < n; i += gridDim.x * WAVES) {
-    const int u = (int)fault_rows[i];
-    const int rb = indptr[u], re = indptr[u + 1];
-    ST *xrow = X + (size_t)u * F;
-    float x[FC], r[FC], p[FC], Ap[FC];
-    load_vec(xrow, x);
-    apply(true, rb, re, x, r);
-#pragma unroll
-    for (int c = 0; c < FC; ++c) p[c] = r[c];
-    float rsold = wave_allsum(dot_local<FC>(r, r));
-    if (rsold < 1e-20f) continue;
-    for (int it = 0; it < cg_steps; ++it) {
-      apply(false, rb, re, p, Ap);
-      const float alpha = rsold / wave_allsum(dot_local<FC>(p, Ap));
-#pragma unroll
-      for (int c = 0; c < FC; ++c) {
-        x[c] = fmaf(alpha, p[c], x[c]);
-        r[c] = fmaf(-alpha, Ap[c], r[c]);
-      }
-      const float rsnew = wave_allsum(dot_local<FC>(r, r));
-      if (rsnew < 1e-20f) break;
-      const float beta = rsnew / rsold;
-#pragma unroll
-      for (int c = 0; c < FC; ++c) p[c] = fmaf(beta, p[c], r[c]);
-      rsold = rsnew;
-    }
-#pragma unroll
-    for (int c = 0; c < FC; ++c) store1(xrow + FC * lane + c, x[c]);
-  }
+  for (int i = blockIdx.x * WAVES + wave; i < n; i += gridDim.x * WAVES)
+    cg_fixup_row<F, ST>(vecs[wave], lane, (int)fault_rows[i], indptr, indices, data, X, Y, A0, cg_steps);
 }
 
 unsigned long long *fixup_total() {
diff --git a/implicit_amd/csrc/als_cg_nm.hip b/implicit_amd/csrc/als_cg_nm.hip
--- a/implicit_amd/csrc/als_cg_nm.hip
+++ b/implicit_amd/csrc/als_cg_nm.hip
@@ -1,3 +1,4 @@
+#include "als_nm_image.h"
 #include "als_qf_common.h"
 #include "common.h"
 #include "wave_ops.h"
@@ -6,43 +7,6 @@
 
 namespace {
 
-typedef _Float16 half8 __attribute__((ext_vector_type(8)));
-typedef _Float16 half2v __attribute__((ext_vector_type(2)));
-typedef float f32x16 __attribute__((ext_vector_type(16)));
-typedef float f32x4v __attribute__((ext_vector_type(4)));
-typedef unsigned u32x4 __attribute__((ext_vector_type(4)));
-
-template <int F> struct NmShape;
-template <> struct NmShape<128> {
-  static constexpr int M = 32, KG = 2, NACC = 16;
-  using acc_t = f32x16;
-  __device__ static __forceinline__ acc_t mfma(half8 a, half8 b, acc_t c) { return __builtin_amdgcn_mfma_f32_32x32x16_f16(a, b, c, 0, 0, 0); }
-  __device__ static __forceinline__ int row(int lane, int e) { return (e & 3) + 8 * (e >> 2) + 4 * (lane >> 5); }
-  __device__ static __forceinline__ int col(int lane) { return lane & 31; }
-};
-template <> struct NmShape<64> {
-  static constexpr int M = 16, KG = 4, NACC = 4;
-  using acc_t = f32x4v;
-  __device__ static __forceinline__ acc_t mfma(half8 a, half8 b, acc_t c) { return __builtin_amdgcn_mfma_f32_16x16x32_f16(a, b, c, 0, 0, 0); }
-  __device__ static __forceinline__ int row(int lane, int e) { return 4 * (lane >> 4) + e; }
-  __device__ static __forceinline__ int col(int lane) { return lane & 15; }
-};
-
-template <int F> struct NmLayout {
-  static constexpr int M = F / 4;
-  static constexpr int TS = M + 1;
-  static constexpr int IMG = 16 * M * TS;
-  static constexpr int KCH = 8 * NmShape<F>::KG;
-  static constexpr int ROUND = 4 * KCH;
-  static constexpr int kTiles = 10;
-  static constexpr int kSlots = 3;
-  static constexpr int QUAD = 64 * 4;
-  static constexpr int OPS = 4 * 16 * QUAD;
-  static constexpr int NP = 256 / F;
-  static constexpr int kVec = IMG > OPS ? IMG : OPS;
-  static constexpr size_t lds_floats = (size_t)kVec + 2 * F + NP * F + 64 + 4 * F;
-  __host__ __device__ static constexpr int at(int I, int J, int m, int n) { return ((I * 4 + J) * M + m) * TS + n; }
-};
 __device__ constexpr int nm_tile_i(int t) { return t < 1 ? 0 : t < 3 ? 1 : t < 6 ? 2 : 3; }
 __device__ constexpr int nm_tile_j(int t) { return t - (nm_tile_i(t) * (nm_tile_i(t) + 1)) / 2; }
 
@@ -328,68 +292,6 @@
     }
   }
   __syncthreads();
-}
-
-template <int F, typename T>
-__device__ __forceinline__ bool nm_cg(const float *img, const float *bvec, float *pv, float *parts, float *red, T *xrow, int cg_steps, int tid) {
-  using L = NmLayout<F>;
-  constexpr int M = L::M, NP = L::NP, JPG = 4 / NP;
-  const int r = tid % F, grp = tid / F, lane = tid & 63, wave = tid >> 6;
-  const int I = r / M, m = r % M;
-  int slot = 0;
-  auto matvec = [&]() {
-    float s[4] = {0.f, 0.f, 0.f, 0.f};
-#pragma unroll
-    for (int jj = 0; jj < JPG; ++jj) {
-      const int J = grp * JPG + jj;
-      const float *row = img + L::at(I, J, m, 0);
-#pragma unroll
-      for (int n = 0; n < M; n += 4) {
-        const float4 p4 = *reinterpret_cast<const float4 *>(pv + J * M + n);
-        s[0] = fmaf(row[n], p4.x, s[0]), s[1] = fmaf(row[n + 1], p4.y, s[1]);
-        s[2] = fmaf(row[n + 2], p4.z, s[2]), s[3] = fmaf(row[n + 3], p4.w, s[3]);
-      }
-    }
-    parts[grp * F + r] = (s[0] + s[1]) + (s[2] + s[3]);
-    __syncthreads();
-    float q = parts[r];
-#pragma unroll
-    for (int gq = 1; gq < NP; ++gq) q += parts[gq * F + r];
-    return q;
-  };
-  auto block_sum = [&](float v) {
-    v = wave_allsum(grp == 0 ? v : 0.f);
-    if (lane == 0) red[4 * slot + wave] = v;
-    __syncthreads();
-    const float s = (red[4 * slot] + red[4 * slot + 1]) + (red[4 * slot + 2] + red[4 * slot + 3]);
-    slot = (slot + 1) & 7;
-    return s;
-  };
-  auto finite = [](float v) { return fabsf(v) <= 3.0e38f; };
-  float x = load1(xrow + 4 * m + I);
-  if (grp == 0) pv[r] = x;
-  __syncthreads();
-  float res = bvec[r] - matvec();
-  float p = res;
-  float rsold = block_sum(res * res);
-  if (!finite(rsold)) return true;
-  if (rsold < 1e-20f) return false;
-  for (int it = 0; it < cg_steps; ++it) {
-    if (grp == 0) pv[r] = p;
-    __syncthreads();
-    const float Ap = matvec();
-    const float pAp = block_sum(p * Ap);
-    const float alpha = rsold / pAp;
-    x = fmaf(alpha, p, x);
-    res = fmaf(-alpha, Ap, res);
-    const float rsnew = block_sum(res * res);
-    if (!finite(pAp) || !finite(rsnew) || !finite(alpha)) return true;
-    if (rsnew < 1e-20f) break;
-    p = fmaf(rsnew / rsold, p, res);
-    rsold = rsnew;
-  }
-  if (grp == 0) store1(xrow + 4 * m + I, x);
-  return false;
 }
 
 #ifdef CHOL_NM_STATS
@@ -706,11 +608,10 @@
   }
 }
 
-template <int F, typename T> void launch_nm(const imp_csr *C, T *X, const T *Y, size_t y_rows, const float *A0, int cg_steps) {
+template <int F, typename T> NmTail launch_nm(const imp_csr *C, T *X, const T *Y, size_t y_rows, const float *A0, int cg_steps) {
   const LongPlan &lp = C->plan_nm;
-  if (lp.n_seg <= 0) return;
-  using L = NmLayout<F>;
-  static_assert(L::IMG % 4 == 0, "the image is copied in 16-byte pieces");
+  if (lp.n_seg <= 0) return NmTail{};
+  using L = NmLayout<F>;
   const size_t lds = L::lds_floats * sizeof(float);
   const int n_multi = C->nm_multi_rows, n_multi_seg = C->nm_multi_segs;
   const size_t need = (size_t)L::IMG + (size_t)n_multi_seg * (L::IMG + F);
@@ -721,9 +622,7 @@
   fix.reserve((size_t)lp.n_long);
   LongPlanDev plan = lp.dev(C->order.data());
   auto kern = als_cg_nm_kernel<F, T>;
-  auto fin = als_cg_nm_finish_kernel<F, T>;
   allow_dynamic_lds(kern, lds);
-  allow_dynamic_lds(fin, lds);
   {
     IMP_PROF("als_cg_nm_rows");
     constexpr int forced_k = -1;
@@ -733,13 +632,25 @@
     kern<<<grid, 256, lds, stream()>>>(plan, C->indices.data(), C->data.data(), X, Y, gram_img, cg_steps, partial, tk.data(), fix.data(), ko);
     IMP_CHECK_HIP(hipGetLastError());
   }
-  if (n_multi > 0) {
-    IMP_PROF("als_cg_nm_finish");
-    als_cg_nm_reduce_kernel<F><<<std::min(n_multi * 16, ctx().num_cus * 16), 256, 0, stream()>>>(plan, n_multi, gram_img, partial);
-    fin<<<std::min(n_multi, ctx().num_cus * 2), 256, lds, stream()>>>(plan, n_multi, X, cg_steps, partial, tk.data(), fix.data());
-    IMP_CHECK_HIP(hipGetLastError());
-  }
-  launch_cg_fixup<F, T>(reinterpret_cast<const unsigned *>(tk.data() + 2), fix.data(), lp.n_long, C, X, Y, A0, cg_steps);
+  NmTail tail;
+  tail.plan = plan, tail.n_multi = n_multi, tail.gram_img = gram_img, tail.partial = partial;
+  tail.ctl = tk.data(), tail.fix_rows = fix.data(), tail.capacity = lp.n_long;
+  return tail;
+}
+
+template <int F, typename T> void launch_nm_finish(const NmTail &tail, T *X, int cg_steps) {
+  if (tail.n_multi <= 0) return;
+  using L = NmLayout<F>;
+  static_assert(L::IMG % 4 == 0, "the image is copied in 16-byte pieces");
+  const size_t lds = L::lds_floats * sizeof(float);
+  auto fin = als_cg_nm_finish_kernel<F, T>;
+  allow_dynamic_lds(fin, lds);
+  IMP_PROF("als_cg_nm_finish");
+  als_cg_nm_reduce_kernel<F><<<std::min(tail.n_multi * 16, ctx().num_cus * 16), 256, 0, stream()>>>(tail.plan, tail.n_multi, tail.gram_img,
+                                                                                                  tail.partial);
+  fin<<<std::min(tail.n_multi, ctx().num_cus * 2), 256, lds, stream()>>>(tail.plan, tail.n_multi, X, cg_steps, tail.partial, tail.ctl,
+                                                                         tail.fix_rows);
+  IMP_CHECK_HIP(hipGetLastError());
 }
 
 }
@@ -800,12 +711,20 @@
   return CholNmList{reinterpret_cast<const unsigned *>(tk.data() + 2), fix.data(), capacity};
 }
 
-template <typename T> void least_squares_cg_nm(const imp_csr *C, T *X, const T *Y, size_t y_rows, const float *A0, int f, int cg_steps) {
-  if (f == 128) launch_nm<128, T>(C, X, Y, y_rows, A0, cg_steps);
-  else if (f == 64) launch_nm<64, T>(C, X, Y, y_rows, A0, cg_steps);
-  else throw std::invalid_argument("least_squares_cg_nm: f must be 64 or 128");
-}
-template void least_squares_cg_nm<float>(const imp_csr *, float *, const float *, size_t, const float *, int, int);
-template void least_squares_cg_nm<__half>(const imp_csr *, __half *, const __half *, size_t, const float *, int, int);
-
-}
+template <typename T> NmTail least_squares_cg_nm(const imp_csr *C, T *X, const T *Y, size_t y_rows, const float *A0, int f, int cg_steps) {
+  if (f == 128) return launch_nm<128, T>(C, X, Y, y_rows, A0, cg_steps);
+  if (f == 64) return launch_nm<64, T>(C, X, Y, y_rows, A0, cg_steps);
+  throw std::invalid_argument("least_squares_cg_nm: f must be 64 or 128");
+}
+template NmTail least_squares_cg_nm<float>(const imp_csr *, float *, const float *, size_t, const float *, int, int);
+template NmTail least_squares_cg_nm<__half>(const imp_csr *, __half *, const __half *, size_t, const float *, int, int);
+
+template <typename T> void cg_nm_finish(const NmTail &tail, T *X, int f, int cg_steps) {
+  if (f == 128) launch_nm_finish<128, T>(tail, X, cg_steps);
+  else if (f == 64) launch_nm_finish<64, T>(tail, X, cg_steps);
+  else throw std::invalid_argument("cg_nm_finish: f must be 64 or 128");
+}
+template void cg_nm_finish<float>(const NmTail &, float *, int, int);
+template void cg_nm_finish<__half>(const NmTail &, __half *, int, int);
+
+}
diff --git a/implicit_amd/csrc/als_cg_q.hip b/implicit_amd/csrc/als_cg_q.hip
--- a/implicit_amd/csrc/als_cg_q.hip
+++ b/implicit_amd/csrc/als_cg_q.hip
@@ -2,6 +2,7 @@
 
 #include "als_qtile.h"
 #include "common.h"
+#include "long_tail_route.h"
 
 namespace imp {
 
@@ -16,23 +17,33 @@
 
 template <typename T>
 void launch_team_chain(const imp_csr *C, int f, const int (&first)[3], const int (&count)[3], T *X, const T *Y, const float *A0, int cg_steps,
-                       const char *name);
+                       const char *name, const NmTail *finish);
 template <typename T>
 void launch_wide_chain(const imp_csr *C, int f, const int (&first)[2], const int (&count)[2], T *X, const T *Y, const float *A0, int cg_steps,
-                       const char *name);
+                       const char *name, const NmTail *fixup);
 
-template <int F, typename T> static void run_classes_q(const imp_csr *C, T *X, const T *Y, const float *A0, int cg_steps) {
+template <int F, typename T> static void run_classes_q(const imp_csr *C, T *X, const T *Y, const float *A0, int cg_steps, const NmTail &tail) {
   const int32_t *b = C->bin_start;
   constexpr bool kHalf = std::is_same<T, __half>::value;
+  auto fixup_alone = [&]() {
+    launch_cg_fixup<F, T>(reinterpret_cast<const unsigned *>(tail.ctl + 2), tail.fix_rows, tail.capacity, C, X, Y, A0, cg_steps);
+  };
   auto team = [&](int width32, int lo, int hi, const char *name) {
     if constexpr (kHalf) launch_team_tile64<T>(C, F, width32 / 2, lo, hi - lo, X, Y, A0, cg_steps, name);
     else launch_team_fused<T>(C, F, width32, lo, hi - lo, X, Y, A0, cg_steps, name);
   };
-  if (F == 128 && !kHalf && !prof_unfiltered()) {
-    const int first[3] = {b[2], b[3], b[4]}, count[3] = {b[3] - b[2], b[4] - b[3], b[5] - b[4]};
-    launch_team_chain<T>(C, F, first, count, X, Y, A0, cg_steps, "als_cg_team_chain_rows");
-    const int wide_first[2] = {b[1], b[5]}, wide_count[2] = {b[2] - b[1], b[7] - b[5]};
-    launch_wide_chain<T>(C, F, wide_first, wide_count, X, Y, A0, cg_steps, "als_cg_wide_chain_rows");
+  const bool chained = F == 128 && !kHalf && !prof_unfiltered();
+  const int first[3] = {b[2], b[3], b[4]}, count[3] = {b[3] - b[2], b[4] - b[3], b[5] - b[4]};
+  const int wide_first[2] = {b[1], b[5]}, wide_count[2] = {b[2] - b[1], b[7] - b[5]};
+  const LongTailRoute route = long_tail_route(count, wide_count, tail.n_multi, tail.capacity, chained);
+  if (route.finish == LongTailRoute::kFinishAlone) cg_nm_finish<T>(tail, X, F, cg_steps);
+  if (route.fixup == LongTailRoute::kFixupAheadOfClasses) fixup_alone();
+  if (chained) {
+    launch_team_chain<T>(C, F, first, count, X, Y, A0, cg_steps, "als_cg_team_chain_rows",
+                         route.finish == LongTailRoute::kFinishInTeamChain ? &tail : nullptr);
+    if (route.fixup == LongTailRoute::kFixupBehindTeamChain) fixup_alone();
+    launch_wide_chain<T>(C, F, wide_first, wide_count, X, Y, A0, cg_steps, "als_cg_wide_chain_rows",
+                         route.fixup == LongTailRoute::kFixupInWideChain ? &tail : nullptr);
     return;
   }
   team(16, b[1], b[2], "als_cg_team16_rows");
@@ -43,12 +54,12 @@
   else launch_group_fused<T>(C, F, b[5], b[7] - b[5], X, Y, A0, cg_steps, "als_cg_short_rows");
 }
 
-template <typename T> void least_squares_cg_q(const imp_csr *C, T *X, const T *Y, const float *A0, int f, int cg_steps) {
-  if (f == 128) run_classes_q<128, T>(C, X, Y, A0, cg_steps);
-  else if (f == 64) run_classes_q<64, T>(C, X, Y, A0, cg_steps);
+template <typename T> void least_squares_cg_q(const imp_csr *C, T *X, const T *Y, const float *A0, int f, int cg_steps, const NmTail &tail) {
+  if (f == 128) run_classes_q<128, T>(C, X, Y, A0, cg_steps, tail);
+  else if (f == 64) run_classes_q<64, T>(C, X, Y, A0, cg_steps, tail);
   else throw std::invalid_argument("least_squares_cg_q: f must be 64 or 128");
 }
-template void least_squares_cg_q<float>(const imp_csr *, float *, const float *, const float *, int, int);
-template void least_squares_cg_q<__half>(const imp_csr *, __half *, const __half *, const float *, int, int);
+template void least_squares_cg_q<float>(const imp_csr *, float *, const float *, const float *, int, int, const NmTail &);
+template void least_squares_cg_q<__half>(const imp_csr *, __half *, const __half *, const float *, int, int, const NmTail &);
 
 }
diff --git a/implicit_amd/csrc/als_cg_qf.hip b/implicit_amd/csrc/als_cg_qf.hip
--- a/implicit_amd/csrc/als_cg_qf.hip
+++ b/implicit_amd/csrc/als_cg_qf.hip
@@ -2,6 +2,8 @@
 
 #include <algorithm>
 
+#include "als_cg_fixup.h"
+#include "als_nm_image.h"
 #include "als_qf_common.h"
 #include "common.h"
 
@@ -76,8 +78,13 @@
                                                                                   const int32_t *__restrict__ indices,
                                                                                   const float *__restrict__ data, ST *__restrict__ X,
                                                                                   const ST *__restrict__ Y, const float *__restrict__ A0,
-                                                                                  int cg_steps) {
+                                                                                  int cg_steps, NmFinishArgs finish) {
   static_assert(Tile32<ST>::T == 32, "chain_lds_bytes");
+  static_assert(NmLayout<F>::lds_floats * sizeof(float) <= chain_lds_bytes<F>(), "the finish items work in the chain's own LDS");
+  if (finish.n_multi > 0) {
+    extern __shared__ __attribute__((aligned(16))) float smem[];
+    nm_finish_items<F, ST, 512>(finish, X, cg_steps, smem);
+  }
   team_stage_gramian<F, 512>(A0);
   bool entered = false;
   static_for<ChainTickets::kClasses>([&](auto Cc) {
@@ -96,11 +103,17 @@
 
 template <typename T>
 void launch_team_chain(const imp_csr *C, int f, const int (&first)[3], const int (&count)[3], T *X, const T *Y, const float *A0, int cg_steps,
-                       const char *name) {
+                       const char *name, const NmTail *finish) {
   if constexpr (std::is_same<T, float>::value) {
     auto run = [&](auto Fc) {
       constexpr int F = decltype(Fc)::value;
-      if (count[0] <= 0 && count[1] <= 0 && count[2] <= 0) return;
+      if (count[0] <= 0 && count[1] <= 0 && count[2] <= 0) {
+        if (finish) throw std::logic_error("launch_team_chain: finish items without a launch to carry them");
+        return;
+      }
+      NmFinishArgs fin;
+      if (finish)
+        fin = NmFinishArgs{finish->n_multi, finish->plan.rows, finish->plan.row_seg, finish->gram_img, finish->partial, finish->ctl, finish->fix_rows};
       const size_t lds = chain_lds_bytes<F>();
       auto kern = als_cg_qfteam_chain_kernel<F, T>;
       allow_dynamic_lds(kern, lds);
@@ -117,7 +130,7 @@
       after.launch(cls.count, grid, teams, cls.base);
       IMP_PROF(name);
       kern<<<grid, 512, lds, stream()>>>(C->order.data(), cls, cx.chain_counters.data(), C->indptr.data(), C->indices.data(),
-                                        C->data.data(), X, Y, A0, cg_steps);
+                                        C->data.data(), X, Y, A0, cg_steps, fin);
       IMP_CHECK_HIP(hipGetLastError());
       cx.chain_tickets = after;
     };
@@ -128,9 +141,9 @@
   }
 }
 template void launch_team_chain<float>(const imp_csr *, int, const int (&)[3], const int (&)[3], float *, const float *, const float *, int,
-                                       const char *);
+                                       const char *, const NmTail *);
 template void launch_team_chain<__half>(const imp_csr *, int, const int (&)[3], const int (&)[3], __half *, const __half *, const float *,
-                                        int, const char *);
+                                        int, const char *, const NmTail *);
 
 typedef float f32x4 __attribute__((ext_vector_type(4)));
 template <int F> struct QFGroupCfg {
@@ -468,6 +481,11 @@
   int first[WideTickets::kClasses], count[WideTickets::kClasses];
   unsigned base[WideTickets::kClasses][WideTickets::kQueues];
 };
+struct WideFixupArgs {
+  const unsigned *count = nullptr, *rows = nullptr;
+  int capacity = 0;
+  unsigned long long *total = nullptr;
+};
 static_assert(WideTickets::kQueues == kTicketQueues && WideTickets::kGroupRows == 16, "queues and groups of the ticketed classes");
 template <int F> constexpr size_t wide_chain_lds_bytes() {
   return std::max(team_lds_bytes<F, 16, 1024, 32>(), QFGroupCfg<F>::lds_bytes + 16);
@@ -479,7 +497,19 @@
                                                                    const int32_t *__restrict__ indices,
                                                                    const float *__restrict__ data, ST *__restrict__ X,
                                                                    const ST *__restrict__ Y, const float *__restrict__ A0,
-                                                                   int cg_steps) {
+                                                                   int cg_steps, WideFixupArgs fix) {
+  if (fix.capacity > 0) {
+    const int n = min((int)fix.count[0], fix.capacity);
+    if (n != 0) {
+      extern __shared__ __attribute__((aligned(16))) float smem[];
+      if (blockIdx.x == 0 && threadIdx.x == 0)
+        __hip_atomic_fetch_add(fix.total, (unsigned long long)n, __ATOMIC_RELAXED, __HIP_MEMORY_SCOPE_SYSTEM);
+      const int lane = threadIdx.x & 63, wave = threadIdx.x >> 6;
+      for (int i = blockIdx.x * 16 + wave; i < n; i += gridDim.x * 16)
+        cg_fixup_row<F, ST>(smem + wave * F, lane, (int)fix.rows[i], indptr, indices, data, X, Y, A0, cg_steps);
+      __syncthreads();
+    }
+  }
   const unsigned queue = blockIdx.x % kTicketQueues;
   if (cls.count[0] > 0)
     team_rows<Tile32<ST>, F, 16, 1024, true, true>(order, cls.first[0], cls.count[0], indptr, indices, data, X, Y, A0, cg_steps,
@@ -494,12 +524,19 @@
 
 template <typename T>
 void launch_wide_chain(const imp_csr *C, int f, const int (&first)[2], const int (&count)[2], T *X, const T *Y, const float *A0, int cg_steps,
-                       const char *name) {
+                       const char *name, const NmTail *fixup) {
   if constexpr (std::is_same<T, float>::value) {
     if (f != 128) throw std::invalid_argument("launch_wide_chain: f must be 128");
     constexpr int F = 128;
     constexpr bool kShortTickets = IMP_WIDE_FORM != 1;
-    if (count[0] <= 0 && count[1] <= 0) return;
+    if (count[0] <= 0 && count[1] <= 0) {
+      if (fixup) throw std::logic_error("launch_wide_chain: a fix-up without a launch to carry it");
+      return;
+    }
+    static_assert(16 * F * sizeof(float) <= wide_chain_lds_bytes<F>(), "an operand slot per wavefront of the fix-up");
+    WideFixupArgs fix;
+    if (fixup && fixup->capacity > 0)
+      fix = WideFixupArgs{reinterpret_cast<const unsigned *>(fixup->ctl + 2), fixup->fix_rows, fixup->capacity, fixup_total()};
     const size_t lds = wide_chain_lds_bytes<F>();
     auto kern = als_cg_qfwide_chain_kernel<F, T, kShortTickets>;
     static const int per_cu = [&] {
@@ -524,8 +561,9 @@
       const int32_t ticketed[2] = {rows[0], kShortTickets ? rows[1] : 0};
       after.launch_rows(ticketed, grid, cls.base);
       kern<<<grid, 1024, lds, stream()>>>(C->order.data(), cls, cx.wide_counters.data(), C->indptr.data(), C->indices.data(),
-                                         C->data.data(), X, Y, A0, cg_steps);
+                                         C->data.data(), X, Y, A0, cg_steps, fix);
       IMP_CHECK_HIP(hipGetLastError());
+      fix = WideFixupArgs{};
       cx.wide_tickets = after;
     };
     IMP_PROF(name);
@@ -536,9 +574,9 @@
   }
 }
 template void launch_wide_chain<float>(const imp_csr *, int, const int (&)[2], const int (&)[2], float *, const float *, const float *, int,
-                                       const char *);
+                                       const char *, const NmTail *);
 template void launch_wide_chain<__half>(const imp_csr *, int, const int (&)[2], const int (&)[2], __half *, const __half *, const float *,
-                                        int, const char *);
+                                        int, const char *, const NmTail *);
 
 template <typename T>
 void launch_group_fused(const imp_csr *C, int f, int first, int count, T *X, const T *Y, const float *A0, int cg_steps, const char *name) {
diff --git a/implicit_amd/csrc/als_nm_image.h b/implicit_amd/csrc/als_nm_image.h
--- /dev/null
+++ b/implicit_amd/csrc/als_nm_image.h
@@ -0,0 +1,183 @@
+#ifndef IMPLICIT_AMD_CSRC_ALS_NM_IMAGE_H_
+#define IMPLICIT_AMD_CSRC_ALS_NM_IMAGE_H_
+
+#include "als_qtile.h"
+#include "common.h"
+#include "wave_ops.h"
+
+namespace imp {
+
+typedef _Float16 half8 __attribute__((ext_vector_type(8)));
+typedef _Float16 half2v __attribute__((ext_vector_type(2)));
+typedef float f32x16 __attribute__((ext_vector_type(16)));
+typedef float f32x4v __attribute__((ext_vector_type(4)));
+typedef unsigned u32x4 __attribute__((ext_vector_type(4)));
+
+template <int F> struct NmShape;
+template <> struct NmShape<128> {
+  static constexpr int M = 32, KG = 2, NACC = 16;
+  using acc_t = f32x16;
+  __device__ static __forceinline__ acc_t mfma(half8 a, half8 b, acc_t c) { return __builtin_amdgcn_mfma_f32_32x32x16_f16(a, b, c, 0, 0, 0); }
+  __device__ static __forceinline__ int row(int lane, int e) { return (e & 3) + 8 * (e >> 2) + 4 * (lane >> 5); }
+  __device__ static __forceinline__ int col(int lane) { return lane & 31; }
+};
+template <> struct NmShape<64> {
+  static constexpr int M = 16, KG = 4, NACC = 4;
+  using acc_t = f32x4v;
+  __device__ static __forceinline__ acc_t mfma(half8 a, half8 b, acc_t c) { return __builtin_amdgcn_mfma_f32_16x16x32_f16(a, b, c, 0, 0, 0); }
+  __device__ static __forceinline__ int row(int lane, int e) { return 4 * (lane >> 4) + e; }
+  __device__ static __forceinline__ int col(int lane) { return lane & 15; }
+};
+
+template <int F> struct NmLayout {
+  static constexpr int M = F / 4;
+  static constexpr int TS = M + 1;
+  static constexpr int IMG = 16 * M * TS;
+  static constexpr int KCH = 8 * NmShape<F>::KG;
+  static constexpr int ROUND = 4 * KCH;
+  static constexpr int kTiles = 10;
+  static constexpr int kSlots = 3;
+  static constexpr int QUAD = 64 * 4;
+  static constexpr int OPS = 4 * 16 * QUAD;
+  static constexpr int NP = 256 / F;
+  static constexpr int kVec = IMG > OPS ? IMG : OPS;
+  static constexpr size_t lds_floats = (size_t)kVec + 2 * F + NP * F + 64 + 4 * F;
+  __host__ __device__ static constexpr int at(int I, int J, int m, int n) { return ((I * 4 + J) * M + m) * TS + n; }
+};
+
+template <int F, typename T, int BLOCK = 256>
+__device__ __forceinline__ bool nm_cg(const float *img, const float *bvec, float *pv, float *parts, float *red, T *xrow, int cg_steps, int tid) {
+  using L = NmLayout<F>;
+  constexpr int M = L::M, NP = L::NP, JPG = 4 / NP;
+  static_assert(BLOCK >= 256 && BLOCK % 64 == 0, "256 working threads, whole wavefronts beside them");
+  const bool on = BLOCK == 256 || tid < 256;
+  const int r = tid % F, grp = tid / F, lane = tid & 63, wave = tid >> 6;
+  const int I = r / M, m = r % M;
+  int slot = 0;
+  auto matvec = [&]() {
+    if (on) {
+      float s[4] = {0.f, 0.f, 0.f, 0.f};
+#pragma unroll
+      for (int jj = 0; jj < JPG; ++jj) {
+        const int J = grp * JPG + jj;
+        const float *row = img + L::at(I, J, m, 0);
+#pragma unroll
+        for (int n = 0; n < M; n += 4) {
+          const float4 p4 = *reinterpret_cast<const float4 *>(pv + J * M + n);
+          s[0] = fmaf(row[n], p4.x, s[0]), s[1] = fmaf(row[n + 1], p4.y, s[1]);
+          s[2] = fmaf(row[n + 2], p4.z, s[2]), s[3] = fmaf(row[n + 3], p4.w, s[3]);
+        }
+      }
+      parts[grp * F + r] = (s[0] + s[1]) + (s[2] + s[3]);
+    }
+    __syncthreads();
+    float q = parts[r];
+#pragma unroll
+    for (int gq = 1; gq < NP; ++gq) q += parts[gq * F + r];
+    return q;
+  };
+  auto block_sum = [&](float v) {
+    if (on) {
+      v = wave_allsum(grp == 0 ? v : 0.f);
+      if (lane == 0) red[4 * slot + wave] = v;
+    }
+    __syncthreads();
+    const float s = (red[4 * slot] + red[4 * slot + 1]) + (red[4 * slot + 2] + red[4 * slot + 3]);
+    slot = (slot + 1) & 7;
+    return s;
+  };
+  auto finite = [](float v) { return fabsf(v) <= 3.0e38f; };
+  float x = on ? load1(xrow + 4 * m + I) : 0.f;
+  if (grp == 0) pv[r] = x;
+  __syncthreads();
+  float res = bvec[r] - matvec();
+  float p = res;
+  float rsold = block_sum(res * res);
+  if (!finite(rsold)) return true;
+  if (rsold < 1e-20f) return false;
+  for (int it = 0; it < cg_steps; ++it) {
+    if (grp == 0) pv[r] = p;
+    __syncthreads();
+    const float Ap = matvec();
+    const float pAp = block_sum(p * Ap);
+    const float alpha = rsold / pAp;
+    x = fmaf(alpha, p, x);
+    res = fmaf(-alpha, Ap, res);
+    const float rsnew = block_sum(res * res);
+    if (!finite(pAp) || !finite(rsnew) || !finite(alpha)) return true;
+    if (rsnew < 1e-20f) break;
+    p = fmaf(rsnew / rsold, p, res);
+    rsold = rsnew;
+  }
+  if (grp == 0) store1(xrow + 4 * m + I, x);
+  return false;
+}
+
+struct NmFinishArgs {
+  int n_multi = 0;
+  const int32_t *rows = nullptr;
+  const int32_t *row_seg = nullptr;
+  const float *gram_img = nullptr, *partial = nullptr;
+  int *ctl = nullptr;
+  unsigned *fix_rows = nullptr;
+};
+
+constexpr int kNmSegBatch = 8;
+template <int F, int BLOCK, int P, int S>
+__device__ __forceinline__ void nm_sum_partials_shape(const float4 *__restrict__ gram4, const float4 *__restrict__ part4, int s0, int s1,
+                                                      float *img, float *bvec, int tid) {
+  using L = NmLayout<F>;
+  constexpr int NIMG = L::IMG / 4, TOTAL = NIMG + F / 4;
+  constexpr size_t stride = (size_t)(L::IMG + F) / 4;
+  for (int e0 = tid; e0 < TOTAL; e0 += BLOCK * P) {
+    float4 sum[P];
+    int e[P];
+#pragma unroll
+    for (int p = 0; p < P; ++p) {
+      e[p] = min(e0 + p * BLOCK, TOTAL - 1);
+      sum[p] = e[p] < NIMG ? gram4[e[p]] : make_float4(0.f, 0.f, 0.f, 0.f);
+    }
+    for (int s = s0; s < s1; s += S) {
+      float4 v[P][S];
+#pragma unroll
+      for (int q = 0; q < S; ++q)
+#pragma unroll
+        for (int p = 0; p < P; ++p) v[p][q] = part4[(size_t)min(s + q, s1 - 1) * stride + e[p]];
+#pragma unroll
+      for (int q = 0; q < S; ++q) {
+        if (s + q < s1) {
+#pragma unroll
+          for (int p = 0; p < P; ++p) sum[p].x += v[p][q].x, sum[p].y += v[p][q].y, sum[p].z += v[p][q].z, sum[p].w += v[p][q].w;
+        }
+      }
+    }
+#pragma unroll
+    for (int p = 0; p < P; ++p) {
+      const int ep = e0 + p * BLOCK;
+      if (ep < NIMG) reinterpret_cast<float4 *>(img)[ep] = sum[p];
+      else if (ep < TOTAL) reinterpret_cast<float4 *>(bvec)[ep - NIMG] = sum[p];
+    }
+  }
+}
+
+template <int F, typename T, int BLOCK>
+__device__ __forceinline__ void nm_finish_items(const NmFinishArgs &a, T *__restrict__ X, int cg_steps, float *smem) {
+  using L = NmLayout<F>;
+  static_assert(L::IMG % 4 == 0 && F % 4 == 0, "the image and b are moved in 16-byte pieces");
+  float *img = smem, *bvec = img + L::kVec, *pv = bvec + F, *parts = pv + F, *red = parts + L::NP * F;
+  const int tid = threadIdx.x;
+  const float4 *gram4 = reinterpret_cast<const float4 *>(a.gram_img), *part4 = reinterpret_cast<const float4 *>(a.partial);
+  for (int li = blockIdx.x; li < a.n_multi; li += gridDim.x) {
+    const int s0 = a.row_seg[li], s1 = a.row_seg[li + 1];
+    if (s1 - s0 > 4) nm_sum_partials_shape<F, BLOCK, 2, kNmSegBatch>(gram4, part4, s0, s1, img, bvec, tid);
+    else nm_sum_partials_shape<F, BLOCK, 8, 2>(gram4, part4, s0, s1, img, bvec, tid);
+    __syncthreads();
+    const bool bad = nm_cg<F, T, BLOCK>(img, bvec, pv, parts, red, X + (size_t)a.rows[li] * F, cg_steps, tid);
+    if (bad && tid == 0) a.fix_rows[atomicAdd(a.ctl + 2, 1)] = (unsigned)a.rows[li];
+    __syncthreads();
+  }
+}
+
+}
+
+#endif
diff --git a/implicit_amd/csrc/common.h b/implicit_amd/csrc/common.h
--- a/implicit_amd/csrc/common.h
+++ b/implicit_amd/csrc/common.h
@@ -315,10 +315,18 @@
 void gramian_half(const void *Y, long n_rows, int f, float reg, float *out);
 bool cg_native_half(int f);
 void least_squares_cg(const imp_csr *C, imp_matrix *X, const imp_matrix *YtY, const imp_matrix *Y, int cg_steps);
-template <typename T> void least_squares_cg_q(const imp_csr *C, T *X, const T *Y, const float *A0, int f, int cg_steps);
+struct NmTail {
+  LongPlanDev plan{};
+  int n_multi = 0;
+  float *gram_img = nullptr, *partial = nullptr;
+  int *ctl = nullptr;
+  unsigned *fix_rows = nullptr;
+  int capacity = 0;
+};
+template <typename T> void least_squares_cg_q(const imp_csr *C, T *X, const T *Y, const float *A0, int f, int cg_steps, const NmTail &tail);
 void least_squares_cg_w256(const imp_csr *C, float *X, const float *Y, const float *A0, int cg_steps);
-template <typename T>
-void least_squares_cg_nm(const imp_csr *C, T *X, const T *Y, size_t y_rows, const float *A0, int f, int cg_steps);
+template <typename T> NmTail least_squares_cg_nm(const imp_csr *C, T *X, const T *Y, size_t y_rows, const float *A0, int f, int cg_steps);
+template <typename T> void cg_nm_finish(const NmTail &tail, T *X, int f, int cg_steps);
 int64_t least_squares_cholesky(const imp_csr *C, imp_matrix *X, const imp_matrix *YtY, const imp_matrix *Y, double reg);
 int64_t least_squares_subspace(const imp_csr *C, imp_matrix *X, const imp_matrix *YtY, const imp_matrix *Y, double reg, int block_size,
                                int sweeps);
diff --git a/implicit_amd/csrc/containers.hip b/implicit_amd/csrc/containers.hip
--- a/implicit_amd/csrc/containers.hip
+++ b/implicit_amd/csrc/containers.hip
@@ -7,6 +7,7 @@
 #include <thread>
 
 #include "common.h"
+#include "long_tail_route.h"
 
 namespace imp {
 
@@ -626,6 +627,21 @@
   });
 }
 
+int imp_host_long_tail_route(const int32_t *chain_count, const int32_t *wide_count, int32_t n_multi, int32_t capacity, int32_t chained,
+                             int32_t *out) {
+  return guarded_host([&] {
+    if (n_multi < 0 || capacity < 0 || n_multi > capacity)
+      throw std::invalid_argument("host_long_tail_route: 0 <= n_multi <= capacity (the rows of more than one segment are long rows)");
+    for (int k = 0; k < 3; ++k)
+      if (chain_count[k] < 0) throw std::invalid_argument("host_long_tail_route: a class holds no fewer than 0 rows");
+    for (int k = 0; k < 2; ++k)
+      if (wide_count[k] < 0) throw std::invalid_argument("host_long_tail_route: a class holds no fewer than 0 rows");
+    const int32_t chain[3] = {chain_count[0], chain_count[1], chain_count[2]}, wide[2] = {wide_count[0], wide_count[1]};
+    const LongTailRoute r = long_tail_route(chain, wide, n_multi, capacity, chained != 0);
+    out[0] = r.finish, out[1] = r.fixup;
+  });
+}
+
 int imp_matrix_create(size_t rows, size_t cols, const void *host_data, size_t itemsize, imp_matrix **out) {
   return guarded([&] {
     imp_matrix *m = new_matrix(rows, cols, itemsize, host_data == nullptr);
diff --git a/implicit_amd/csrc/long_tail_route.h b/implicit_amd/csrc/long_tail_route.h
--- /dev/null
+++ b/implicit_amd/csrc/long_tail_route.h
@@ -0,0 +1,33 @@
+#ifndef IMPLICIT_AMD_CSRC_LONG_TAIL_ROUTE_H_
+#define IMPLICIT_AMD_CSRC_LONG_TAIL_ROUTE_H_
+
+#include <cstdint>
+
+namespace imp {
+
+struct LongTailRoute {
+  enum Finish : int32_t { kNoFinish = 0, kFinishAlone = 1, kFinishInTeamChain = 2 };
+  enum Fixup : int32_t {
+    kNoFixup = 0,
+    kFixupAheadOfClasses = 1,
+    kFixupBehindTeamChain = 2,
+    kFixupInWideChain = 3
+  };
+  int32_t finish = kNoFinish, fixup = kNoFixup;
+};
+
+inline LongTailRoute long_tail_route(const int32_t (&chain)[3], const int32_t (&wide)[2], int32_t n_multi, int32_t capacity, bool chained) {
+  const bool team_chain = chained && (chain[0] > 0 || chain[1] > 0 || chain[2] > 0);
+  const bool wide_chain = chained && (wide[0] > 0 || wide[1] > 0);
+  LongTailRoute r;
+  if (n_multi > 0) r.finish = team_chain ? LongTailRoute::kFinishInTeamChain : LongTailRoute::kFinishAlone;
+  if (capacity > 0) {
+    if (wide_chain) r.fixup = LongTailRoute::kFixupInWideChain;
+    else r.fixup = r.finish == LongTailRoute::kFinishInTeamChain ? LongTailRoute::kFixupBehindTeamChain : LongTailRoute::kFixupAheadOfClasses;
+  }
+  return r;
+}
+
+}
+
+#endif
diff --git a/implicit_amd/gpu/_hip.py b/implicit_amd/gpu/_hip.py
--- a/implicit_amd/gpu/_hip.py
+++ b/implicit_amd/gpu/_hip.py
@@ -33,6 +33,7 @@
                           ctypes.c_void_p],
     "imp_host_chain_tickets": [ctypes.c_void_p, ctypes.c_void_p, ctypes.c_int32, ctypes.c_void_p, ctypes.c_void_p, ctypes.c_void_p],
     "imp_host_wide_tickets": [ctypes.c_void_p, ctypes.c_void_p, ctypes.c_int32, ctypes.c_void_p, ctypes.c_void_p],
+    "imp_host_long_tail_route": [ctypes.c_void_p, ctypes.c_void_p, ctypes.c_int32, ctypes.c_int32, ctypes.c_int32, ctypes.c_void_p],
     "imp_matrix_create": [ctypes.c_size_t, ctypes.c_size_t, ctypes.c_void_p, ctypes.c_size_t, c_void_pp],
     "imp_matrix_wrap_device": [ctypes.c_size_t, ctypes.c_size_t, ctypes.c_void_p, ctypes.c_size_t, c_void_pp],
     "imp_matrix_row": [ctypes.c_void_p, ctypes.c_size_t, c_void_pp],
diff --git a/implicit_amd/utils.py b/implicit_amd/utils.py
--- a/implicit_amd/utils.py
+++ b/implicit_amd/utils.py
@@ -182,3 +182,15 @@
     base, draws = np.empty((2, 8), np.uint32), np.empty((2, 8), np.uint32)
     check(lib().imp_host_wide_tickets(state.ctypes.data, rows.ctypes.data, int(workgroups), base.ctypes.data, draws.ctypes.data))
     return base, draws
+
+
+def long_tail_route(chain_counts, wide_counts, n_multi, capacity, chained):
+    from .gpu._hip import check, lib
+
+    chain = np.ascontiguousarray(chain_counts, dtype=np.int32)
+    wide = np.ascontiguousarray(wide_counts, dtype=np.int32)
+    assert chain.shape == (3,) and wide.shape == (2,)
+    out = np.zeros(2, np.int32)
+    check(lib().imp_host_long_tail_route(chain.ctypes.data, wide.ctypes.data, int(n_multi), int(capacity), int(bool(chained)),
+                                         out.ctypes.data))
+    return int(out[0]), int(out[1])
diff --git a/include/implicit_hip.h b/include/implicit_hip.h
--- a/include/implicit_hip.h
+++ b/include/implicit_hip.h
@@ -51,6 +51,9 @@
                            uint32_t *draws);
 
 int imp_host_wide_tickets(uint32_t *next, const int32_t *rows, int32_t workgroups, uint32_t *base, uint32_t *draws);
+
+int imp_host_long_tail_route(const int32_t *chain_count, const int32_t *wide_count, int32_t n_multi, int32_t capacity, int32_t chained,
+                             int32_t *out);
 
 int imp_matrix_create(size_t rows, size_t cols, const void *host_data, size_t itemsize, imp_matrix **out);
 int imp_matrix_wrap_device(size_t rows, size_t cols, void *device_ptr, size_t itemsize, imp_matrix **out);
```

Measured after the change: 180.3 million updates/s (median of 6 runs). 1.01x the previous value.
